# tsinghua-fib-lab/PIML

Hardware: AMD Instinct MI355X
Metric: agent-pair force evals/sec + simulated steps/sec, 4096-agent GC scene (higher is better)
Workload: dtype f32

## Files before the change

### include/piml_hip.h

```cpp
#ifndef PIML_HIP_H
#define PIML_HIP_H

#include <stddef.h>
#include <stdint.h>

#ifdef __cplusplus
extern "C" {
#endif

#define PIML_HIP_ABI_VERSION 35
#define PIML_MAX_TOPK 32

int piml_abi_version(void);

const char* piml_error_string(int err);

int piml_heading_fwd(const float* velocity, int C, int T, int N, float* heading, void* stream);

int piml_relfeat_fwd(const float* position, const float* heading, const float* velocity,
                     const float* acceleration, int state_ld, const float* destination,
                     const float* obstacles, int C, int N, int M, int focal_begin,
                     int focal_count, int topk_ped, int topk_obs, float cos_thr_ped,
                     float cos_thr_obs, float dist_thr_ped, float dist_thr_obs,
                     float* ped_feat, float* obs_feat, float* dest_feat, int dest_feat_ld,
// ... 353 lines not shown
                                  size_t rows, float tau, float* out, void* stream);
int piml_pinnsf_epilogue_ksum_bwd(const float* g_out, const float* self_features, size_t rows, float tau, int kp, int ko,
                                  float* g_self, float* g_pred_ped, float* g_pred_obs, void* stream);

int piml_pinnsf_epilogue_agentnorm_fwd(const float* acc_ped, const float* acc_obs, const float* self_features,
                                       int C, int N, float tau, float* out, void* stream);
int piml_pinnsf_epilogue_ksum_agentnorm_fwd(const float* pred_ped, int kp, const float* pred_obs, int ko, const float* self_features,
                                            int C, int N, float tau, float* out, void* stream);
int piml_pinnsf_epilogue_agentnorm_bwd(const float* g_out, const float* self_features, int C, int N, float tau,
                                       float* g_self, void* stream);

int piml_self_features_fwd(const float* dest_feat, int dest_ld, const float* state, const float* desired_speed,
                           size_t rows, float* out, void* stream);
int piml_self_features_bwd(const float* g_self, size_t rows, float* g_dest, float* g_state, float* g_speed,
                           void* stream);

int piml_colsum_blocks(size_t rows, int cols);
int piml_act_bwd_colsum(const float* g, const float* y, size_t rows, int cols, float* g_pre, float* partials,
                        float* db, void* stream);

int piml_sum_leading(const float* parts, int B, size_t n, float* out, void* stream);
int piml_act_bwd_colsum_stage1(const float* g, const float* y, size_t rows, int cols, float* g_pre, float* partials,
                               float* db, void* stream);
int piml_layer_reduce(const float* parts, int B, size_t n, float* out, const float* col_partials, int nb, int cols,
                      float* db, void* stream);

int piml_scale_ksum_fwd(const float* e, const float* bias, size_t agents, int k, int cols, float scale,
                        const unsigned* keep_bits, float* msgs, float* pooled, void* stream);
int piml_ksum_blocks(size_t agents, int cols);
int piml_scale_ksum_bwd(const float* g_pooled, const float* g_msgs, size_t agents, int k, int cols, float scale,
                        const unsigned* keep_bits, float* g_e, float* col_partials, void* stream);

int piml_dropout_keep_bits(unsigned long long* state, long long rows, int cols, float p, int stream_id, unsigned* keep_bits,
                           void* stream);

typedef struct piml_encoder_branch {
    const float* x;
    long long rows;
    int in_dim;
    int k;
    const float *w1, *b1, *w2, *b2, *w3, *b3;
    float scale;
    float *h1, *h2, *msgs;
    const float *g_pooled, *g_msgs;
    float *g2, *g1, *g_x;
    float* partials;
    float* grads;
    float* packed;
    unsigned* relu_mask;
    unsigned* keep_bits;
    unsigned long long* drop_state;
    float drop_p;
    float *sum_a, *sum_b;
} piml_encoder_branch;

int piml_encoder_partial_floats(void);
int piml_encoder_pack_floats(void);
int piml_encoder_pack(const piml_encoder_branch* branches, int nbranches, void* stream);
int piml_encoder_workgroups(const piml_encoder_branch* branches, int nbranches, int* wg_branch0);
int piml_encoder_fwd(const piml_encoder_branch* branches, int nbranches, void* stream);
int piml_encoder_fwd_packed(const piml_encoder_branch* branches, int nbranches, void* stream);
int piml_encoder_bwd(const piml_encoder_branch* branches, int nbranches, void* stream);
int piml_encoder_bwd_acc(const piml_encoder_branch* branches, int nbranches, int accumulate, void* stream);
int piml_encoder_ksum(const float* msgs, long long agents, int k, float* pooled, void* stream);

typedef struct piml_decoder_branch {
    const float* msgs;
    long long agents;
    int k;
    const float *w1, *b1, *w2, *b2, *w3, *b3;
    float *pooled, *h1, *d2;
    float *g_pre2, *g_pre1, *g_pooled;
    float* partials;
    float* grads;
    float* packed;
    float* pred;
    const float* g_pred_rows;
    const float* g_d2;
    const float *fold_w3, *fold_b3;
    float fold_scale;
    float* dw1_out;
} piml_decoder_branch;

int piml_decoder_pack_floats(void);
int piml_decoder_partial_floats(void);
int piml_decoder_workgroups(long long agents);
int piml_decoder_fwd(const piml_decoder_branch* branches, int nbranches, const float* self_features, float tau,
                     float* acc, void* stream);
int piml_decoder_bwd(const piml_decoder_branch* branches, int nbranches, const float* g_pred,
                     const float* self_features, float tau, float* g_self, void* stream);

int piml_rowdecoder_slots(long long rows);
int piml_rowdecoder_fwd(const piml_decoder_branch* branches, int nbranches, void* stream);
int piml_rowdecoder_fwd_packed(const piml_decoder_branch* branches, int nbranches, void* stream);
int piml_rowdecoder_bwd(const piml_decoder_branch* branches, int nbranches, void* stream);
int piml_rowdecoder_bwd_acc(const piml_decoder_branch* branches, int nbranches, int accumulate, void* stream);

typedef struct piml_collision_head {
    const float* msgs;
    long long rows;
    const float *w1, *b1, *w2, *b2;
    float* packed;
    float* out;
    const float *fold_w3, *fold_b3;
    float fold_scale;
} piml_collision_head;

// ... 98 lines not shown
```

### include/piml_hip_tuning.h

```cpp
#ifndef PIML_HIP_TUNING_H
#define PIML_HIP_TUNING_H

#include "piml_hip.h"

#ifdef __cplusplus
extern "C" {
#endif

int piml_timer_create(void** event);
int piml_timer_record(void* event, void* stream);
int piml_timer_elapsed_ms(void* start, void* stop, float* ms);
int piml_timer_destroy(void* event);

int piml_trace_begin(void);
int piml_trace_mark(const char* name, void* stream);
int piml_trace_end(char* names, int names_cap, float* us, int us_cap);

int piml_probe_arith(const float* rx, const float* ry, const float* hx, const float* hy,
                     float* dist, float* cosv, int n, void* stream);

long long piml_encoder_split_tiles(long long tiles);
long long piml_encoder_split_tiles_train(long long tiles);
int piml_encoder_products(int split_bf16);
int piml_rowdecoder_products(int split_bf16);
int piml_encoder_dw2(int layer_split);
int piml_encoder_fused_bwd(int on);
int piml_encoder_sums_bwd(int form);
int piml_encoder_sums_dec_slots(int on);
int piml_pinnsf_streams_init(void);

#ifdef __cplusplus
}
#endif
#endif
```

### piml_amd/_lib.py

```python
import ctypes
import os

import torch

_HERE = os.path.dirname(os.path.abspath(__file__))
LIB_PATH = os.environ.get('PIML_LIB') or os.path.join(_HERE, 'libpiml_hip.so')
ABI_VERSION = 35

_lib = None

_i, _f, _p, _z = ctypes.c_int, ctypes.c_float, ctypes.c_void_p, ctypes.c_size_t
_ll = ctypes.c_longlong
_d = ctypes.c_double


class EncoderBranch(ctypes.Structure):
    _fields_ = [('x', _p), ('rows', _ll), ('in_dim', _i), ('k', _i),
                ('w1', _p), ('b1', _p), ('w2', _p), ('b2', _p), ('w3', _p), ('b3', _p),
                ('scale', _f), ('h1', _p), ('h2', _p), ('msgs', _p), ('g_pooled', _p), ('g_msgs', _p),
                ('g2', _p), ('g1', _p), ('g_x', _p), ('partials', _p), ('grads', _p), ('packed', _p), ('relu_mask', _p),
                ('keep_bits', _p), ('drop_state', _p), ('drop_p', _f), ('sum_a', _p), ('sum_b', _p)]


class DecoderBranch(ctypes.Structure):
    _fields_ = [('msgs', _p), ('agents', _ll), ('k', _i),
                ('w1', _p), ('b1', _p), ('w2', _p), ('b2', _p), ('w3', _p), ('b3', _p),
                ('pooled', _p), ('h1', _p), ('d2', _p), ('g_pre2', _p), ('g_pre1', _p), ('g_pooled', _p),
                ('partials', _p), ('grads', _p), ('packed', _p), ('pred', _p), ('g_pred_rows', _p), ('g_d2', _p),
                ('fold_w3', _p), ('fold_b3', _p), ('fold_scale', _f), ('dw1_out', _p)]


class CollisionHead(ctypes.Structure):
    _fields_ = [('msgs', _p), ('rows', _ll), ('w1', _p), ('b1', _p), ('w2', _p), ('b2', _p), ('packed', _p), ('out', _p),
                ('fold_w3', _p), ('fold_b3', _p), ('fold_scale', _f)]


class Head64(ctypes.Structure):
    _fields_ = [('x', _p), ('rows', _ll), ('w1', _p), ('b1', _p), ('w2', _p), ('b2', _p), ('hidden', _p), ('out', _p),
                ('g_out', _p), ('g_x', _p), ('partials', _p), ('grads', _p)]


class Corrector(ctypes.Structure):
    _fields_ = [('agents', _ll), ('k', _i), ('scale', _f), ('enc', _p), ('keep_bits', _p),
                ('wa', _p), ('ba', _p), ('wb', _p), ('bb', _p), ('wc', _p), ('bc', _p), ('wd', _p), ('bd', _p),
                ('hid', _p), ('score', _p), ('attn', _p), ('pooled', _p), ('chid', _p), ('out', _p),
                ('g_out', _p), ('g_pooled', _p), ('g_score', _p), ('g_chid', _p), ('g_enc', _p),
                ('partials_a', _p), ('partials_b', _p), ('grads', _p)]


class Scenario(ctypes.Structure):
    _fields_ = [('position', _p), ('velocity', _p), ('acceleration', _p), ('destination', _p), ('hist_velocity', _p),
                ('self_features', _p), ('desired_speed', _p), ('mask', _p), ('flag', _p), ('waypoints', _p), ('exit_idx', _p),
                ('spawn_iters', _p), ('position_out', _p), ('velocity_out', _p), ('acceleration_out', _p),
                ('destination_out', _p), ('mask_out', _p), ('spawn_out', _p), ('frame_counter', _p), ('spawned', _p),
                ('dropped', _p), ('entries', _p), ('route_polyline', _p),
                ('hist_width', _i), ('F', _i), ('D', _i), ('E', _i), ('P', _i), ('R', _i), ('capacity', _i), ('T', _i),
                ('n_initial', _i), ('route_max_iters', _i), ('spawn_cap', _i), ('uniform_speed', _i),
                ('dt', _f), ('spawn_offset', _f), ('route_clearance', _f), ('arrival_radius', _f), ('speed_mean', _f),
                ('speed_std', _f), ('speed_min', _f), ('seed', ctypes.c_uint64), ('poisson_thresholds', ctypes.c_uint32 * 8)]


class ScenarioRules(ctypes.Structure):
    _fields_ = [('spawn_law', _i), ('arrival_rule', _i), ('initial_velocity', _i), ('speed_clamp', _i), ('spawn_cap2', _i),
                ('grid', _i), ('length', _f), ('width', _f), ('side_ratio', _f), ('direction_ratio', _f),
                ('poisson_thresholds2', ctypes.c_uint32 * 8), ('square_grid', _f * 32)]


class MlapmLaw(ctypes.Structure):
    _fields_ = [('variant', _i), ('tau', _f), ('A', _f), ('B', _f), ('C', _f), ('D', _f), ('theta_deg', _f), ('radius', _f)]


class WallGrid(ctypes.Structure):
    _fields_ = [('points', _p), ('cell_start', _p), ('n_points', _i), ('gx', _i), ('gy', _i),
                ('x0', _f), ('y0', _f), ('cell', _f), ('cutoff', _f)]
# ... 84 lines not shown
    'piml_pinnsf_epilogue_agentnorm_fwd': [_p, _p, _p, _i, _i, _f, _p, _p],
    'piml_pinnsf_epilogue_ksum_agentnorm_fwd': [_p, _i, _p, _i, _p, _i, _i, _f, _p, _p],
    'piml_pinnsf_epilogue_agentnorm_bwd': [_p, _p, _i, _i, _f, _p, _p],
    'piml_self_features_fwd': [_p, _i, _p, _p, _z, _p, _p],
    'piml_self_features_bwd': [_p, _z, _p, _p, _p, _p],
    'piml_colsum_blocks': [_z, _i],
    'piml_act_bwd_colsum': [_p, _p, _z, _i, _p, _p, _p, _p],
    'piml_sum_leading': [_p, _i, _z, _p, _p],
    'piml_act_bwd_colsum_stage1': [_p, _p, _z, _i, _p, _p, _p, _p],
    'piml_layer_reduce': [_p, _i, _z, _p, _p, _i, _i, _p, _p],
    'piml_scale_ksum_fwd': [_p, _p, _z, _i, _i, _f, _p, _p, _p, _p],
    'piml_ksum_blocks': [_z, _i],
    'piml_scale_ksum_bwd': [_p, _p, _z, _i, _i, _f, _p, _p, _p, _p],
    'piml_dropout_keep_bits': [_p, _ll, _i, _f, _i, _p, _p],
    'piml_timer_create': [ctypes.POINTER(_p)],
    'piml_timer_record': [_p, _p],
    'piml_timer_elapsed_ms': [_p, _p, ctypes.POINTER(_f)],
    'piml_timer_destroy': [_p],
    'piml_trace_begin': [],
    'piml_trace_mark': [ctypes.c_char_p, _p],
    'piml_trace_end': [ctypes.c_char_p, _i, ctypes.POINTER(_f), _i],
    'piml_probe_arith': [_p, _p, _p, _p, _p, _p, _i, _p],
    'piml_encoder_partial_floats': [],
    'piml_encoder_pack_floats': [],
    'piml_encoder_split_tiles': [_ll],
    'piml_encoder_split_tiles_train': [_ll],
    'piml_multi_copy': [ctypes.POINTER(_p), ctypes.POINTER(_p), ctypes.POINTER(_z), _i, _p],
    'piml_rollout_prologue': [_p] * 8 + [_i] * 4 + [_p] * 11 + [_p],
    'piml_rollout_losses_blocks': [_i, _i],
    'piml_rollout_losses': [_p, _p, _ll, _p, _p, _p, _p, _p, _i, _i, _i, _f, _p, _p, _p, _p, _p, _p, _p],
    'piml_rollout_losses_bwd': [_p, _p, _p, _p, _p, _p, _ll, _p, _p],
    'piml_rollout_losses_frames': [_p, _p, _ll, _p, _p, ctypes.POINTER(_p), _i, _p, _i, _i, _i, _f, _f, _f, _p, _p, _p, _p, _p, _p, _p],
    'piml_rollout_losses_frames_bwd': [_p, _p, _p, _p, _f, _f, _p, _p, _p, _ll, _p, _p],
    'piml_collision_pred_loss_blocks': [_ll, _i],
    'piml_collision_pred_loss': [ctypes.POINTER(_p), ctypes.POINTER(_p), _i, _ll, _i, _i, _p, _i, _i, _f, _p, _p, _p, _p, _p],
    'piml_collision_pred_loss_bwd': [_p, _p, _ll, _p, _p],
    'piml_adam_tickets': [],
    'piml_adam_step': [ctypes.POINTER(_p)] * 5 + [ctypes.POINTER(_ll), _i, ctypes.c_double, ctypes.c_double, ctypes.c_double, ctypes.c_double, ctypes.c_double, _p, _p],
    'piml_pointwise_losses_blocks': [_ll, _ll, _i],
    'piml_pointwise_losses': [_p, _p, _ll, _ll, _p, _ll, _f, _p, _i, _p, _p, _p, _p, _p],
    'piml_p2p_alloc': [_z, ctypes.POINTER(_p)],
    'piml_p2p_free': [_p],
    'piml_p2p_export': [_p, _p],
    'piml_p2p_open': [_p, ctypes.POINTER(_p)],
    'piml_p2p_close': [_p],
    'piml_p2p_copy': [_p, _p, _z, _p],
    'piml_allgather_state_p2p': [_p, _z, _i, _i, ctypes.POINTER(_p), ctypes.POINTER(_p), ctypes.c_uint, ctypes.c_uint, _p, _p],
    'piml_encoder_products': [_i],
    'piml_rowdecoder_products': [_i],
    'piml_encoder_dw2': [_i],
    'piml_encoder_fused_bwd': [_i],
    'piml_encoder_sums_bwd': [_i],
    'piml_encoder_sums_dec_slots': [_i],
    'piml_encoder_pack': [ctypes.POINTER(EncoderBranch), _i, _p],
    'piml_encoder_workgroups': [ctypes.POINTER(EncoderBranch), _i, ctypes.POINTER(_i)],
    'piml_encoder_fwd': [ctypes.POINTER(EncoderBranch), _i, _p],
    'piml_encoder_fwd_packed': [ctypes.POINTER(EncoderBranch), _i, _p],
    'piml_encoder_bwd': [ctypes.POINTER(EncoderBranch), _i, _p],
    'piml_encoder_bwd_acc': [ctypes.POINTER(EncoderBranch), _i, _i, _p],
    'piml_encoder_ksum': [_p, _ll, _i, _p, _p],
    'piml_decoder_pack_floats': [],
    'piml_decoder_partial_floats': [],
    'piml_decoder_workgroups': [_ll],
    'piml_decoder_fwd': [ctypes.POINTER(DecoderBranch), _i, _p, _f, _p, _p],
    'piml_decoder_bwd': [ctypes.POINTER(DecoderBranch), _i, _p, _p, _f, _p, _p],
    'piml_rowdecoder_slots': [_ll],
    'piml_rowdecoder_fwd': [ctypes.POINTER(DecoderBranch), _i, _p],
    'piml_rowdecoder_fwd_packed': [ctypes.POINTER(DecoderBranch), _i, _p],
    'piml_rowdecoder_bwd': [ctypes.POINTER(DecoderBranch), _i, _p],
    'piml_rowdecoder_bwd_acc': [ctypes.POINTER(DecoderBranch), _i, _i, _p],
    'piml_collision_head_pack_floats': [],
    'piml_collision_head_fwd': [_p, _ll, _p, _p, _p, _p, _p, _p, _p],
    'piml_head64_partial_floats': [],
    'piml_head64_slots': [_ll],
    'piml_head64_fwd': [ctypes.POINTER(Head64), _p],
    'piml_head64_bwd': [ctypes.POINTER(Head64), _p],
    'piml_head64_bwd_acc': [ctypes.POINTER(Head64), _i, _p],
    'piml_corrector_partial_floats': [_i],
    'piml_corrector_slots': [_i, _ll, _i],
    'piml_corrector_fwd': [ctypes.POINTER(Corrector), _p],
    'piml_corrector_bwd': [ctypes.POINTER(Corrector), _i, _p],
    'piml_pinnsf_pool_h2_ok': [ctypes.POINTER(EncoderBranch), _i],
    'piml_pinnsf_pool_train_ok': [ctypes.POINTER(EncoderBranch), _i],
    'piml_pinnsf_pool_msgs_ok': [ctypes.POINTER(EncoderBranch), _i],
    'piml_pinnsf_streams_init': [],
    'piml_pinnsf_pack_flush': [],
    'piml_pinnsf_slot_sums_flush': [],
    'piml_pinnsf_pack': [ctypes.POINTER(EncoderBranch), ctypes.POINTER(DecoderBranch), _i, ctypes.POINTER(CollisionHead),
                         _i, _p],
    'piml_pinnsf_fwd': [ctypes.POINTER(EncoderBranch), ctypes.POINTER(DecoderBranch), _i, ctypes.POINTER(CollisionHead),
                        _p, _f, _p, _i, _p],
    'piml_pinnsf_bwd': [ctypes.POINTER(EncoderBranch), ctypes.POINTER(DecoderBranch), _i, _p, _p, _f, _p, _i, _p],
    'piml_comm_available': [],
    'piml_comm_unique_id': [_p],
    'piml_comm_init': [ctypes.POINTER(_p), _i, _i, _p],
    'piml_comm_destroy': [_p],
    'piml_allgather_state': [_p, _p, _z, _p, _p],
    'piml_reducescatter_grad': [_p, _p, _p, _z, _p],
    'piml_allreduce_sum': [_p, _p, _z, _p],
    'piml_relfeat_fwd_self': [_p, _p, _p, _p, _i, _p, _p, _p, _i, _i, _i, _i, _i, _i, _i, _f, _f, _f, _f, _p, _p, _p, _p, _p, _p, _p],
    'piml_relfeat_bwd_self': [_p, _p, _p, _p, _p, _p, _i, _p, _i, _i, _i, _i, _i, _i, _p, _p, _p, _p],
    'piml_relfeat_fwd_tick': [_p, _p, _p, _p, _i, _p, _p, _i, _i, _i, _i, _i, _i, _i, _f, _f, _f, _f,
                              _p, _p, _p, _i, _p, _p, _p, _p],
    'piml_relfeat_self_fwd': [_p, _p, _p, _p, _i, _i, _i, _i, _i, _i, _f, _f, _f, _f, _p, _p, _p, _p, _p, _p, _p],
    'piml_relfeat_self_fwd_part': [_i, _p, _p, _p, _p, _i, _i, _i, _i, _i, _i, _f, _f, _f, _f, _p, _p, _p, _p, _p, _p, _p],
    'piml_relfeat_self_bwd': [_p, _p, _p, _p, _p, _p, _p, _i, _i, _i, _i, _i, _p, _p, _p, _p],
# ... 165 lines not shown
```

### piml_amd/csrc/encoder.hip

```cpp
#include <cstdlib>

#include "common.hpp"
#include "encoder.hpp"
#include "pack.hpp"
#include "reduce.hpp"
#include "philox.hpp"
#include "stages.hpp"
#include "../../include/piml_hip.h"

namespace piml {

__device__ __forceinline__ void keep_block_f32(f32x16& a, unsigned word, int h) {
    const unsigned m = word >> (4 * h);
#pragma unroll
    for (int r = 0; r < 16; ++r) a[r] = ((m >> ((r & 3) + 8 * (r >> 2))) & 1u) ? a[r] : 0.f;
}
__device__ __forceinline__ unsigned keep_word(const unsigned* __restrict__ keep, long long row, int blk, bool valid) {
    return valid ? keep[row * 4 + blk] : 0u;
}

__global__ __launch_bounds__(256) void enc_pack_kernel(EncArgs A) {
    const int b = blockIdx.y;
    const piml_encoder_branch J = b ? A.br[1] : A.br[0];
    const int e = blockIdx.x * 256 + threadIdx.x;
    if (e < PACK_FLOATS) J.packed[e] = pack_value(J, e);
}

constexpr int FWD_LDS_FLOATS = 16384 * 2 + 1024 + 384;

__global__ __launch_bounds__(ENC_THREADS) void enc_fwd_kernel(EncArgs A) {
    extern __shared__ __align__(16) float lds[];
    const int tid = threadIdx.x, lane = tid & 63, wave = tid >> 6;
    const int b = (A.nbr > 1 && (int)blockIdx.x >= A.wg_split) ? 1 : 0;
    const piml_encoder_branch J = b ? A.br[1] : A.br[0];
    const int wg0 = b ? A.wg_split : 0;
    const int nwg = b ? (int)gridDim.x - A.wg_split : (A.nbr > 1 ? A.wg_split : (int)gridDim.x);
    const long long R = J.rows;
    const int IN = J.in_dim;
    const long long ntiles = (R + 31) >> 5;
    const long long first = (long long)((int)blockIdx.x - wg0) * ENC_WAVES + wave;
    const long long stride = (long long)nwg * ENC_WAVES;
    if (A.zero)
        for (int e = blockIdx.x * ENC_THREADS + tid; e < A.zero_n; e += gridDim.x * ENC_THREADS) A.zero[e] = 0.f;
    if ((long long)((int)blockIdx.x - wg0) * ENC_WAVES >= ntiles) return;

    const float4* W2f = reinterpret_cast<const float4*>(lds);
    const float4* W3f = reinterpret_cast<const float4*>(lds + 16384);
    const float* W1f = lds + 32768;
    const float* bias = lds + 32768 + 1024;
    stage_linear<PACK_FWD>(lds, J.packed, tid);
    __syncthreads();

    const int j = lane & 31, h = lane >> 5;
    for (long long tile = first; tile < ntiles; tile += stride) {
        const long long row = tile * 32 + j;
        const bool valid = row < R;
        float xb[4];
#pragma unroll
        for (int s = 0; s < 4; ++s) {
            const int c = 2 * s + h;
            xb[s] = (valid && c < IN) ? J.x[row * IN + c] : 0.f;
        }
        f32x16 a1[4], a2[4];
#pragma unroll
        for (int blk = 0; blk < 4; ++blk) {
#pragma unroll
            for (int q = 0; q < 4; ++q) {
                const float4 bq = *reinterpret_cast<const float4*>(bias + feat0(blk, q, h));
                a1[blk][4 * q + 0] = bq.x; a1[blk][4 * q + 1] = bq.y; a1[blk][4 * q + 2] = bq.z; a1[blk][4 * q + 3] = bq.w;
            }
#pragma unroll
            for (int s = 0; s < 4; ++s) a1[blk] = mfma32(W1f[(blk * 4 + s) * 64 + lane], xb[s], a1[blk]);
#pragma unroll
            for (int r = 0; r < 16; ++r) a1[blk][r] = fmaxf(a1[blk][r], 0.f);
        }
        if (J.h1 && valid) {
            float* o = J.h1 + row * EH;
#pragma unroll
// ... 602 lines not shown
struct Reduce2Args { piml_encoder_branch br[2]; int n0[2], n1[2]; int accumulate; };
__global__ __launch_bounds__(256) void enc_reduce2_kernel(Reduce2Args A) {
    const int b = blockIdx.y >> 1, L = blockIdx.y & 1;
    const piml_encoder_branch J = b ? A.br[1] : A.br[0];
    if (L == 0) {
        if ((int)blockIdx.x * 16 < DW2_L0_LANES) sum_slots_16x16(J.partials, J.grads, A.n0[b], DW2_L0_LANES, DW2_L0_SPLIT, 0, DW2_L0_OFF1, A.accumulate != 0);
    } else {
        if ((int)blockIdx.x * 16 < DW2_L1_LANES)
            sum_slots_16x16(J.partials + (size_t)A.n0[b] * (DW2_L0_LANES * 4), J.grads, A.n1[b], DW2_L1_LANES, DW2_L1_SPLIT, DW2_L1_OFF0, DW2_L1_OFF1,
                            A.accumulate != 0);
    }
}

static int split_workgroups(const piml_encoder_branch* br, int nbr, int total, long long unit) {
    if (nbr < 2) return total;
    const double r0 = (double)br[0].rows, r1 = (double)br[1].rows;
    int w = (int)(total * r0 / (r0 + r1) + 0.5);
    if (w < 1) w = 1;
    if (w > total - 1) w = total - 1;
    (void)unit;
    return w;
}

static bool branch_ok(const piml_encoder_branch& b) {
    return b.rows > 0 && b.rows < (1ll << 24) && b.in_dim >= 1 && b.in_dim <= 8 && b.x && b.w1 && b.b1 && b.w2 && b.b2 && b.w3 && b.b3 &&
           b.packed;
}

static int fill_args(EncArgs& A, const piml_encoder_branch* br, int nbr) {
    A.nbr = nbr;
    A.zero = nullptr;
    A.zero_n = 0;
    A.gen_state = nullptr;
    for (int i = 0; i < nbr; ++i) A.br[i] = br[i];
    if (nbr == 1) A.br[1] = br[0];
    A.wg_split = split_workgroups(br, nbr, 256, 1);
    return 256;
}

}

using namespace piml;

PIML_API int piml_encoder_partial_floats(void) { return ENC_PART; }

PIML_API int piml_encoder_workgroups(const piml_encoder_branch* br, int nbr, int* wg_branch0) {
    if (!br || nbr < 1 || nbr > 2) return 0;
    const int total = 256;
    const int w0 = split_workgroups(br, nbr, total, 1);
    if (wg_branch0) *wg_branch0 = w0;
    return total;
}

PIML_API int piml_encoder_pack_floats(void) { return PACK_FLOATS; }

static int enc_check(const piml_encoder_branch* br, int nbr) {
    if (!br || nbr < 1 || nbr > 2) return hipErrorInvalidValue;
    for (int i = 0; i < nbr; ++i)
        if (!branch_ok(br[i])) return hipErrorInvalidValue;
    if (nbr == 2 && (br[0].keep_bits != nullptr) != (br[1].keep_bits != nullptr)) return hipErrorInvalidValue;
    return hipSuccess;
}

static int enc_bwd_check(const piml_encoder_branch* br, int nbr);
static bool enc_bwd_is_fused(const piml_encoder_branch* br, int nbr);


static int enc_set_lds(const void* f, int bytes) {
    return hipFuncSetAttribute(f, hipFuncAttributeMaxDynamicSharedMemorySize, bytes);
}

int piml::enc_stage_pack(const piml_encoder_branch* br, int nbr, hipStream_t s) {
    if (!br || nbr < 1 || nbr > 2) return hipErrorInvalidValue;
    for (int i = 0; i < nbr; ++i) {
        const piml_encoder_branch& b = br[i];
        if (b.in_dim < 1 || b.in_dim > 8 || !b.w1 || !b.b1 || !b.w2 || !b.b2 || !b.w3 || !b.b3 || !b.packed) return hipErrorInvalidValue;
    }
    EncArgs A;
    A.nbr = nbr;
    A.br[0] = br[0];
    A.br[1] = br[nbr - 1];
    A.wg_split = 0;
    A.zero = nullptr;
    A.zero_n = 0;
    A.gen_state = nullptr;
    hipLaunchKernelGGL(enc_pack_kernel, dim3((PACK_FLOATS + 255) / 256, nbr), dim3(256), 0, s, A);
    return hipGetLastError();
}

static long long split_tiles_default() { return getenv("PIML_ENC_SPLIT_TILES") ? atoll(getenv("PIML_ENC_SPLIT_TILES")) : 640; }
static long long split_tiles_train_default() {
    if (getenv("PIML_ENC_SPLIT_TILES_TRAIN")) return atoll(getenv("PIML_ENC_SPLIT_TILES_TRAIN"));
    return getenv("PIML_ENC_SPLIT_TILES") ? atoll(getenv("PIML_ENC_SPLIT_TILES")) : 48;
}
static long long g_split_tiles = split_tiles_default();
static long long g_split_tiles_train = split_tiles_train_default();

PIML_API long long piml_encoder_split_tiles(long long tiles) {
    const long long old = g_split_tiles;
    if (tiles >= 0) g_split_tiles = g_split_tiles_train = tiles;
    else if (tiles == -2) { g_split_tiles = split_tiles_default(); g_split_tiles_train = split_tiles_train_default(); }
    return old;
}
PIML_API long long piml_encoder_split_tiles_train(long long tiles) {
    const long long old = g_split_tiles_train;
    if (tiles >= 0) g_split_tiles_train = tiles;
    return old;
}
static long long split_bound(const piml_encoder_branch* br, int nbr) {
    for (int i = 0; i < nbr; ++i)
        if (!br[i].relu_mask) return g_split_tiles;
    return g_split_tiles_train;
}

static int g_x3 = !(getenv("PIML_ENC_PRODUCTS") && getenv("PIML_ENC_PRODUCTS")[0] == 'f');

PIML_API int piml_encoder_products(int x3) {
    const int old = g_x3;
    if (x3 >= 0) g_x3 = x3 ? 1 : 0;
    return old;
}

static int g_f3 = getenv("PIML_ENC_FUSED_BWD") ? atoi(getenv("PIML_ENC_FUSED_BWD")) != 0 : 1;

PIML_API int piml_encoder_fused_bwd(int on) {
    const int old = g_f3;
    if (on >= 0) g_f3 = on != 0;
    return old;
}

static int g_sums_bwd = getenv("PIML_ENC_SUMS_BWD") && atoi(getenv("PIML_ENC_SUMS_BWD")) == 1 ? 1 : 2;

PIML_API int piml_encoder_sums_bwd(int form) {
    const int old = g_sums_bwd;
    if (form == 1 || form == 2) g_sums_bwd = form;
    return old;
}

bool piml::enc_f32_images_needed() { return !g_x3; }
// ... 262 lines not shown
    if (int e = enc_bwd_check(br, nbr)) return e;
    EncArgs A;
    fill_args(A, br, nbr);
    Reduce2Args R2 = {};
    R2.accumulate = accumulate ? 1 : 0;
    if (defer) {
        ReduceAll R = {};
        R.accumulate = accumulate ? 1 : 0;
        int n = 0, maxl = 0;
        auto add = [&](const float* parts, float* grads, int slots, int lanes, int split, int off0, int off1) {
            R.set[n++] = ReduceSet{parts, grads, slots, lanes, split, off0, off1};
            if (lanes > maxl) maxl = lanes;
        };
        int n0[2] = {0, 0}, n1[2] = {0, 0}, w0 = 0;
        const int total = piml_encoder_workgroups(br, nbr, &w0);
        const bool dw2 = enc_dw2_used(br, nbr, n0, n1);
        for (int i = 0; i < nbr; ++i) {
            if (dw2) {
                add(br[i].partials, br[i].grads, n0[i], DW2_L0_LANES, DW2_L0_SPLIT, 0, DW2_L0_OFF1);
                add(br[i].partials + (size_t)n0[i] * (DW2_L0_LANES * 4), br[i].grads, n1[i], DW2_L1_LANES, DW2_L1_SPLIT, DW2_L1_OFF0, DW2_L1_OFF1);
            } else {
                add(br[i].partials, br[i].grads, nbr == 1 ? total : (i == 0 ? w0 : total - w0), ENC_PART / 4, 0x7fffffff, 0, 0);
            }
        }
        R.nsets = n;
        R.gx = (maxl + 15) / 16;
        return pending_slot_sums_leave(R, s);
    }
    if (enc_dw2_used(br, nbr, R2.n0, R2.n1)) {
        for (int i = 0; i < nbr; ++i) R2.br[i] = br[i];
        hipLaunchKernelGGL(enc_reduce2_kernel, dim3((DW2_L1_LANES + 15) / 16, 2 * nbr), dim3(256), 0, s, R2);
        return hipGetLastError();
    }
    hipLaunchKernelGGL(enc_reduce_kernel, dim3((ENC_PART / 4 + 15) / 16, nbr), dim3(256), 0, s, A, ENC_PART / 4, accumulate ? 1 : 0);
    return hipGetLastError();
}

bool piml::enc_pool_train_ok(const piml_encoder_branch* br, int nbr) {
    static const bool off = getenv("PIML_POOL_TRAIN") && atoi(getenv("PIML_POOL_TRAIN")) == 0;
    if (off || !g_dw2 || g_f3 != 1) return false;
    const long long tiles = pool_tiles(br, nbr, true, [](const piml_encoder_branch& b) { return !b.keep_bits && !b.drop_state; });
    if (tiles < 0 || tiles <= g_split_tiles_train) return false;
    const int total = 256, w0 = split_workgroups(br, nbr, total, 1);
    return nbr == 1 || (w0 >= 2 && total - w0 >= 2);
}

bool piml::enc_pool_msgs_ok(const piml_encoder_branch* br, int nbr) {
    static const bool off = getenv("PIML_POOL_MSGS") && atoi(getenv("PIML_POOL_MSGS")) == 0;
    if (off) return false;
    const long long tiles = pool_tiles(br, nbr, true, [](const piml_encoder_branch& b) { return b.relu_mask != nullptr; });
    return tiles >= 0 && tiles > g_split_tiles_train;
}

int piml::enc_stage_fwd_sum(const piml_encoder_branch* br, int nbr, hipStream_t s, float* zero, long long zero_n) {
    if (int e = enc_check(br, nbr)) return e;
    if (!enc_pool_train_ok(br, nbr)) return hipErrorInvalidValue;
    for (int i = 0; i < nbr; ++i)
        if (!br[i].sum_a || !br[i].sum_b || !br[i].relu_mask) return hipErrorInvalidValue;
    EncArgs A;
    const int total = fill_args(A, br, nbr);
    if (int e = set_zero(A, zero, zero_n)) return e;
    if (int e = x3_ready()) return e;
    enc_x3_launch_fwd_sum(A, total, s);
    return hipGetLastError();
}

int piml::enc_stage_bwd_sum(const piml_encoder_branch* br, int nbr, hipStream_t s, const DecSlotSums* dec, bool* dec_summed) {
    if (dec_summed) *dec_summed = false;
    if (int e = enc_check(br, nbr)) return e;
    if (!enc_pool_train_ok(br, nbr)) return hipErrorInvalidValue;
    for (int i = 0; i < nbr; ++i) {
        const piml_encoder_branch& b = br[i];
        if (!b.g_pooled || b.g_msgs || !b.relu_mask || !b.partials || !b.grads || (b.g_x != nullptr) != (br[0].g_x != nullptr)) return hipErrorInvalidValue;
    }
    EncArgs A;
    const int total = fill_args(A, br, nbr);
    if (int e = x3_ready()) return e;
    static int ready = -1;
    if (ready < 0) { ready = enc_f3_set_attributes(); if (!ready) ready = enc_f5_set_attributes(); }
    if (ready) return ready;
    const int nA[2] = {nbr > 1 ? A.wg_split : total, nbr > 1 ? total - A.wg_split : 0};
    const int zero[2] = {0, 0};
    if (g_sums_bwd == 1 || !enc_f5_launch(A, nA, s, dec)) enc_f3_launch(A, nA, zero, false, s, true);
    else if (dec_summed) *dec_summed = dec && dec->nsets > 0;
    return hipGetLastError();
}

PIML_API int piml_encoder_pack(const piml_encoder_branch* br, int nbr, void* stream) {
    return enc_stage_pack(br, nbr, as_stream(stream));
}

PIML_API int piml_encoder_fwd(const piml_encoder_branch* br, int nbr, void* stream) {
    if (int e = enc_stage_pack(br, nbr, as_stream(stream))) return e;
    return enc_stage_fwd(br, nbr, as_stream(stream));
}

PIML_API int piml_encoder_fwd_packed(const piml_encoder_branch* br, int nbr, void* stream) {
    if (int e = pending_pack_flush(as_stream(stream))) return e;
    return enc_stage_fwd(br, nbr, as_stream(stream));
}

PIML_API int piml_encoder_ksum(const float* msgs, long long agents, int k, float* pooled, void* stream) {
    if (agents == 0) return hipSuccess;
    if (!msgs || !pooled || agents < 0 || k < 0) return hipErrorInvalidValue;
    const long long n = agents * (EH / 4);
    hipLaunchKernelGGL(enc_ksum_kernel, dim3((unsigned)((n + 255) / 256)), dim3(256), 0, as_stream(stream),
                       reinterpret_cast<const float4*>(msgs), agents, k, reinterpret_cast<float4*>(pooled));
    return hipGetLastError();
}

PIML_API int piml_encoder_bwd_acc(const piml_encoder_branch* br, int nbr, int accumulate, void* stream) {
    const bool acc = (accumulate & 1) || (accumulate & PIML_ACCUMULATE), defer = (accumulate & PIML_DEFER_SLOT_SUMS) != 0;
    if (int e = enc_stage_bwd_dx(br, nbr, as_stream(stream))) return e;
    if (int e = enc_stage_bwd_dw(br, nbr, as_stream(stream))) return e;
    return enc_stage_reduce(br, nbr, as_stream(stream), acc, defer);
}

PIML_API int piml_encoder_bwd(const piml_encoder_branch* br, int nbr, void* stream) { return piml_encoder_bwd_acc(br, nbr, 0, stream); }
```

### piml_amd/csrc/encoder.hpp

```cpp
#pragma once
#include <hip/hip_runtime.h>

#include "pack.hpp"
#include "../../include/piml_hip.h"

namespace piml {

typedef float f32x16 __attribute__((ext_vector_type(16)));

constexpr int ENC_THREADS = 512;
constexpr int ENC_WAVES = ENC_THREADS / 64;

struct EncArgs {
    piml_encoder_branch br[2];
    int nbr;
    int wg_split;
    float* zero;
    int zero_n;
    unsigned long long* gen_state;
};

__device__ __forceinline__ f32x16 mfma32(float a, float b, f32x16 c) {
    return __builtin_amdgcn_mfma_f32_32x32x2f32(a, b, c, 0, 0, 0);
}
typedef float f32x4 __attribute__((ext_vector_type(4)));
__device__ __forceinline__ void store4_stream(float* p, float a, float b, float c, float d) {
    *reinterpret_cast<float4*>(p) = make_float4(a, b, c, d);
}

template <int NFLOATS>
__device__ __forceinline__ void stage_linear(float* lds, const float* __restrict__ src, int tid) {
    constexpr int N4 = NFLOATS / 4, ROUNDS = (N4 + ENC_THREADS - 1) / ENC_THREADS;
    static_assert(NFLOATS % 4 == 0, "float4 granularity");
    const float4* s4 = reinterpret_cast<const float4*>(src);
    float4* d4 = reinterpret_cast<float4*>(lds);
    float4 v[ROUNDS];
#pragma unroll
    for (int r = 0; r < ROUNDS; ++r) {
        const int e = r * ENC_THREADS + tid;
        v[r] = s4[(r + 1) * ENC_THREADS <= N4 || e < N4 ? e : 0];
    }
#pragma unroll
    for (int r = 0; r < ROUNDS; ++r) {
        const int e = r * ENC_THREADS + tid;
        if ((r + 1) * ENC_THREADS <= N4 || e < N4) d4[e] = v[r];
    }
}

__device__ __forceinline__ int feat0(int blk, int q, int h) { return 32 * blk + 8 * q + 4 * h; }

int enc_x3_set_attributes();
void enc_x3_launch_fwd_pool(const EncArgs& A, int total, hipStream_t s);
void enc_x3_launch_fwd_sum(const EncArgs& A, int total, hipStream_t s);
void enc_x3_launch_fwd(const EncArgs& A, int total, bool drop, hipStream_t s, bool exch = false);
void enc_x3_launch_fwd_split(const EncArgs& A, int pairs0, int pairs1, bool drop, hipStream_t s);
void enc_x3_launch_bwd_dx_split(const EncArgs& A, int pairs0, int pairs1, bool drop, hipStream_t s);
void enc_x3_launch_bwd_dx(const EncArgs& A, int total, bool mask, bool drop, hipStream_t s);

int enc_dww_set_attributes();
void enc_dww_launch(const EncArgs& A, int grid, bool drop, hipStream_t s);
int enc_dw2_set_attributes();
void enc_dw2_split(int w, int* n0, int* n1);
void enc_dw2_launch(const EncArgs& A, int total, hipStream_t s);

// ... 7 lines not shown
```

### piml_amd/csrc/encoder_bwd5.hip

```cpp
#include "common.hpp"
#include "encoder.hpp"
#include "x3.hpp"

namespace piml {

typedef short f5_s16x4 __attribute__((ext_vector_type(4)));
typedef __attribute__((address_space(3))) f5_s16x4 f5_lds_s16x4;

constexpr int F5_THREADS = 512;
constexpr int F5_IMG = 3 * 128 * 64;
constexpr int F5_M = 0;
constexpr int F5_H = F5_M + 2 * F5_IMG;
constexpr int F5_TROW = 36;
constexpr int F5_TBYTES = 128 * F5_TROW * 4;
constexpr int F5_T = F5_H + 2 * F5_IMG;
constexpr int F5_XS = F5_T + 2 * F5_TBYTES;
constexpr int F5_MK = F5_XS + 3 * 1024;
constexpr int F5_W1 = F5_MK + 2 * 512;
constexpr int F5_GXP = F5_W1 + 4096;
constexpr int F5_GXP_BYTES = 4 * 32 * 16 * 4;
constexpr int F5_TAB = F5_GXP + 2 * F5_GXP_BYTES;
constexpr int F5_KMAX = 16;
constexpr int F5_LDS_BYTES = F5_TAB + F5_KMAX * 2 * 16 * 4;
constexpr int F5_LDS_LAUNCH = F5_LDS_BYTES;
// ... 18 lines not shown
    }
}
__device__ __forceinline__ void f5_dec_sums(const DecSlotSums& D, int wg, int nwg, int t, int nthr) {
    const int total = D.nsets * D.lanes, per = (total + nwg - 1) / nwg;
    const int e1 = min(wg * per + per, total), half = nthr >> 4;
    for (int e = wg * per + (t >> 4); e < e1; e += 2 * half) {
        const bool two = e + half < e1;
        const int ea = e, eb = two ? e + half : e;
        const int sa = ea >= D.lanes ? 1 : 0, sb = eb >= D.lanes ? 1 : 0;
        const float4* const p[2] = {reinterpret_cast<const float4*>(sa ? D.parts[1] : D.parts[0]),
                                    reinterpret_cast<const float4*>(sb ? D.parts[1] : D.parts[0])};
        const int j[2] = {ea - sa * D.lanes, eb - sb * D.lanes};
        float4 s[2];
        slot_chains<2>(p, D.slots, D.lanes, j, t & 15, s);
        const float4 va = s[0], vb = s[1];
        f5_chains_add<1>(s[0], va);
        f5_chains_add<1>(s[1], vb);
        if ((t & 15) == 0) {
            slot_sum_store(reinterpret_cast<float4*>(sa ? D.grads[1] : D.grads[0]) + j[0], s[0], D.accumulate != 0);
            if (two) slot_sum_store(reinterpret_cast<float4*>(sb ? D.grads[1] : D.grads[0]) + j[1], s[1], D.accumulate != 0);
        }
    }
}

#ifdef PIML_F5_STAMPS
__device__ unsigned long long g_f5_stamps[256 * 8 * 16];
#define F5_STAMP(i)                                                        \
    do {                                                                   \
        __builtin_amdgcn_sched_barrier(0);                                 \
        {                                                                  \
            const unsigned long long t_ = __builtin_amdgcn_s_memtime();    \
            st[i] += t_ - tprev;                                           \
            tprev = t_;                                                    \
        }                                                                  \
        __builtin_amdgcn_sched_barrier(0);                                 \
    } while (0)
#else
#define F5_STAMP(i)
#endif

#define F5_BARRIER() asm volatile("s_waitcnt lgkmcnt(0)\n\ts_barrier" ::: "memory")

__device__ __forceinline__ float f5_relu(float x) { return __int_as_float(max(__float_as_int(x), 0)); }
__device__ __forceinline__ constexpr int f5_rho(int r) { return (r & 3) + 8 * (r >> 2); }

#define F5_SLOT(MF, FILL)                        \
    do {                                         \
        MF;                                      \
        __builtin_amdgcn_sched_barrier(0);       \
        FILL;                                    \
        __builtin_amdgcn_sched_barrier(0);       \
    } while (0)

template <bool GX, int INC>
__global__ __launch_bounds__(F5_THREADS) void enc_bwd_sums2_kernel(F5Args F) {
    extern __shared__ __align__(16) unsigned char smem[];
    const int tid = threadIdx.x, lane = tid & 63;
    const int wv = __builtin_amdgcn_readfirstlane(tid >> 6);
    const int crew = wv >> 2, w = wv & 3;
    const int ctid = tid & 255;
    const int n = lane & 31, h = lane >> 5;
    int bx = (int)blockIdx.x, b = 0;
    if (bx >= F.nA[0]) { b = 1; bx -= F.nA[0]; }
    const piml_encoder_branch J = b ? F.A.br[1] : F.A.br[0];
    const int nwg = F.nA[b];
    const unsigned R = (unsigned)J.rows;
    const unsigned IN = __builtin_amdgcn_readfirstlane((unsigned)J.in_dim), K = __builtin_amdgcn_readfirstlane((unsigned)J.k);
    const unsigned kmagic = __builtin_amdgcn_readfirstlane((unsigned)((0x100000000ull + K - 1) / K));
    const int ntiles = (int)((R + 31) >> 5);
    const int nit = bx < ntiles ? (ntiles - bx + nwg - 1) / nwg : 0;
    float* P = J.partials + (size_t)bx * F5_PART1;
    constexpr int NS = INC == 6 ? 3 : 4;

    auto rsrc = [&](const void* base, unsigned bytes) {
        return __builtin_amdgcn_make_buffer_rsrc(const_cast<void*>(base), 0, (int)bytes, 0x00020000);
    };
    constexpr unsigned kOut = 0x80000000u;
    const __amdgpu_buffer_rsrc_t rs_gp = rsrc(J.g_pooled, (R / K) * EH * 4);
    const __amdgpu_buffer_rsrc_t rs_x = rsrc(J.x, R * IN * 4);
    const __amdgpu_buffer_rsrc_t rs_mk = rsrc(J.relu_mask, (unsigned)ntiles * 1024);
    const __amdgpu_buffer_rsrc_t rs_gx = rsrc(J.g_x, GX ? R * IN * 4 : 0u);
    auto ld1 = [&](const __amdgpu_buffer_rsrc_t& rs, unsigned voff, unsigned soff) {
        return (unsigned)__builtin_amdgcn_raw_buffer_load_b32(rs, (int)voff, (int)soff, 0);
    };

#ifdef PIML_F5_STAMPS
    unsigned long long st[16], tprev = __builtin_amdgcn_s_memtime();
#pragma unroll
    for (int i = 0; i < 16; ++i) st[i] = 0;
#endif

    {
        float4* z = reinterpret_cast<float4*>(smem + F5_T);
        constexpr int NZ = (F5_W1 - F5_T) / 16;
#pragma unroll
        for (int i = 0; i < (NZ + F5_THREADS - 1) / F5_THREADS; ++i)
            if (i * F5_THREADS + tid < NZ) z[i * F5_THREADS + tid] = make_float4(0.f, 0.f, 0.f, 0.f);
#pragma unroll
        for (int i = 0; i < 2 * F5_GXP_BYTES / 16 / F5_THREADS; ++i) reinterpret_cast<float4*>(smem + F5_GXP)[i * F5_THREADS + tid] = make_float4(0.f, 0.f, 0.f, 0.f);
        if ((unsigned)tid < K * 32u) {
            const unsigned rem = (unsigned)tid >> 5, hh = ((unsigned)tid >> 4) & 1u, r = (unsigned)tid & 15u;
            reinterpret_cast<unsigned*>(smem + F5_TAB)[tid] = ((rem + 4u * hh + (unsigned)f5_rho((int)r)) / K) * (EH * 4);
        }
        if (tid < 256) reinterpret_cast<float4*>(smem + F5_W1)[tid] = make_float4(0.f, 0.f, 0.f, 0.f);
    }

    if (crew == 0) {
        u32x4 wh[8], wm[8], wl[8];
        {
            const u32x4* imgB = reinterpret_cast<const u32x4*>(J.packed + PACK_F32 + 3 * X3_IMG) + lane;
#pragma unroll
            for (int kb = 0; kb < 8; ++kb) {
                const int fb = w * 8 + kb;
                wh[kb] = imgB[(fb * 2) * 64];
                wm[kb] = imgB[(fb * 2 + 1) * 64];
                wl[kb] = imgB[X3_HM / 4 + fb * 64];
            }
        }
        const float* W1rows = J.packed + PACK_FWD + 32768;
        float w1v[NS];
#pragma unroll
        for (int s = 0; s < NS; ++s) w1v[s] = W1rows[(32 * w + n) * 8 + 2 * s + h];
        const float b1v = J.b1[32 * w + n];

        const int fw = 32 * w + n;
        const int swz_w = (fw >> 1) & 7;
        const int mw_off = F5_M + fw * 64;
        int mr[2];
        {
            const int g16 = lane >> 4, q = (lane >> 2) & 3, pp = lane & 3, hh = g16 >> 1;
            const int chunk = 4 * (g16 & 1) + pp;
#pragma unroll
            for (int half2 = 0; half2 < 2; ++half2)
                mr[half2] = F5_M + (8 * half2 + 4 * hh + q) * 64 + ((chunk ^ (4 * half2 + 2 * hh + (q >> 1))) * 8);
        }
        const int bp = 16 * (w & 1) + (n & 3) + 4 * (n >> 3);
        const int mk_off = F5_MK + ((4 * h + 32 * ((n >> 2) & 1)) * 2 + (w >> 1)) * 4;
        const int t_off = F5_T + fw * (F5_TROW * 4) + (4 * h) * 4;
        const int h_off = F5_H + ((w * 2) * 3 * 64 + lane) * 16;
        const unsigned gbase = (unsigned)(32 * w + n) * 4u;

        float g2[16];
        unsigned m2 = 0, mkv = 0;
        float xa[NS];
        auto req_g = [&](int tile) {
            const unsigned t32 = __builtin_amdgcn_readfirstlane((unsigned)tile * 32u);
            const unsigned a0 = __builtin_amdgcn_readfirstlane(__umulhi(t32, kmagic)), rem = t32 - a0 * K;
            const bool live = tile < ntiles;
            const unsigned gb = live ? gbase + a0 * (EH * 4) : kOut;
            const uint4* tab = reinterpret_cast<const uint4*>(smem + F5_TAB + (rem * 32u + 16u * (unsigned)h) * 4u);
#pragma unroll
            for (int i = 0; i < 4; ++i) {
                const uint4 o = tab[i];
                g2[4 * i + 0] = __uint_as_float(ld1(rs_gp, gb + o.x, 0u));
                g2[4 * i + 1] = __uint_as_float(ld1(rs_gp, gb + o.y, 0u));
                g2[4 * i + 2] = __uint_as_float(ld1(rs_gp, gb + o.z, 0u));
                g2[4 * i + 3] = __uint_as_float(ld1(rs_gp, gb + o.w, 0u));
            }
            m2 = ld1(rs_mk, live ? (unsigned)tile * 1024u + (128u + 2u * (unsigned)lane + (unsigned)(w >> 1)) * 4u : kOut, 0u);
        };
        auto req_x = [&](int tile) {
            const unsigned row = (unsigned)tile * 32u + (unsigned)n;
            const bool valid = (tile < ntiles) & (row < R);
#pragma unroll
            for (int s = 0; s < NS; ++s) {
                const unsigned cx = 2u * s + h;
                xa[s] = __uint_as_float(ld1(rs_x, (valid & (cx < IN)) ? (row * IN + cx) * 4u : kOut, 0u));
            }
            mkv = ld1(rs_mk, tile < ntiles ? (unsigned)tile * 1024u + (unsigned)(ctid & 127) * 4u : kOut, 0u);
        };
        float db1 = 0.f, db2 = 0.f;
        unsigned phi[4], pmid[4], plo[4];
        float sp_ra = 0.f, sp_rb = 0.f;
        auto split_a = [&](float a_, float b_, unsigned& hi) {
            hi = bf16_pair(a_, b_);
            sp_ra = a_ - __uint_as_float(hi << 16);
            sp_rb = b_ - __uint_as_float(hi & 0xffff0000u);
        };
        auto split_b = [&](unsigned& mid, unsigned& lo) {
            mid = bf16_pair(sp_ra, sp_rb);
            lo = bf16_pair(sp_ra - __uint_as_float(mid << 16), sp_rb - __uint_as_float(mid & 0xffff0000u));
        };
        auto g2_step = [&](int j, int pm) {
            const int s = j >> 3, q = j & 7;
            if (q < 2) {
                const unsigned m2w = m2 >> (16 * (w & 1));
#pragma unroll
                for (int r = 8 * s + 4 * q; r < 8 * s + 4 * q + 4; ++r) {
                    const int t = __builtin_amdgcn_sbfe(m2w, r, 1);
                    g2[r] = __uint_as_float(__float_as_uint(g2[r]) & (unsigned)t);
                    db2 += g2[r];
                }
            } else if (q < 6) {
                const int d = q - 2;
                split_a(g2[8 * s + 2 * d], g2[8 * s + 2 * d + 1], phi[d]);
                split_b(pmid[d], plo[d]);
            } else {
                const int g = 2 * s + (q - 6), d = 2 * (g & 1);
                unsigned char* dst = smem + mw_off + pm * F5_IMG + (((2 * g + h) ^ swz_w) * 8);
                *reinterpret_cast<uint2*>(dst) = make_uint2(phi[d], phi[d + 1]);
                *reinterpret_cast<uint2*>(dst + 8192) = make_uint2(pmid[d], pmid[d + 1]);
                *reinterpret_cast<uint2*>(dst + 16384) = make_uint2(plo[d], plo[d + 1]);
            }
        };
        f32x16 hacc;
        auto h1_mma = [&]() {
#pragma unroll
            for (int r = 0; r < 16; ++r) hacc[r] = b1v;
#pragma unroll
            for (int s = 0; s < NS; ++s) hacc = mfma32(xa[s], w1v[s], hacc);
        };
        auto h1_step = [&](int j, int pm) {
            const int s = j / 5, q = j % 5;
            if (q < 4) {
                split_a(f5_relu(hacc[8 * s + 2 * q]), f5_relu(hacc[8 * s + 2 * q + 1]), phi[q]);
                split_b(pmid[q], plo[q]);
            } else {
                u32x4* dst = reinterpret_cast<u32x4*>(smem + h_off + pm * F5_IMG + (s * 3 * 64) * 16);
                dst[0] = (u32x4){phi[0], phi[1], phi[2], phi[3]};
                dst[64] = (u32x4){pmid[0], pmid[1], pmid[2], pmid[3]};
                dst[128] = (u32x4){plo[0], plo[1], plo[2], plo[3]};
            }
        };
        auto stage = [&](int xslot, int pm) {
            if (w < NS) reinterpret_cast<float*>(smem + F5_XS + xslot * 1024)[n * 8 + 2 * w + h] = w == 0 ? xa[0] : (w == 1 ? xa[1] : (w == 2 ? xa[2] : xa[NS - 1]));
            if (ctid < 128) reinterpret_cast<unsigned*>(smem + F5_MK + pm * 512)[ctid] = mkv;
        };
        auto load_b = [&](u32x4 (&o)[3], int kb, int pm) {
#pragma unroll
            for (int p = 0; p < 3; ++p) {
                const f5_s16x4 lo4 = __builtin_amdgcn_ds_read_tr16_b64_v4i16((f5_lds_s16x4*)(smem + mr[0] + pm * F5_IMG + kb * 1024 + p * 8192));
                const f5_s16x4 hi4 = __builtin_amdgcn_ds_read_tr16_b64_v4i16((f5_lds_s16x4*)(smem + mr[1] + pm * F5_IMG + kb * 1024 + p * 8192));
                const uint2 x = __builtin_bit_cast(uint2, lo4), y = __builtin_bit_cast(uint2, hi4);
                o[p] = (u32x4){x.x, x.y, y.x, y.y};
            }
        };

        F5_BARRIER();
        req_g(bx);
        req_x(bx);
#pragma unroll
        for (int j = 0; j < 16; ++j) g2_step(j, 0);
        h1_mma();
#pragma unroll
        for (int j = 0; j < 10; ++j) h1_step(j, 0);
        stage(0, 0);
        req_g(bx + nwg);
        req_x(bx + nwg);
        F5_STAMP(15);
        F5_BARRIER();

        for (int it = 0; it < nit; ++it) {
            const int par = it & 1, tile = bx + it * nwg;
            F5_STAMP(0);
            f32x16 acc;
            u32x4 opa[2][3], ahi[8];
            unsigned mkw[16];
            const unsigned* mk1 = reinterpret_cast<const unsigned*>(smem + mk_off + par * 512);
            auto fill_a = [&](int sl) {
                if (sl < 40 && sl % 5 == 0) {
                    const int kb = sl / 5 + 1;
                    if (kb < 8) load_b(opa[kb & 1], kb, par);
                    return;
                }
                if (sl == 38 || sl == 39) return;
                const int f = sl < 40 ? sl - sl / 5 - 1 : sl - 10;
                (void)it;
                if (f >= 30 && f < 34) {
#pragma unroll
                    for (int i = 4 * (f - 30); i < 4 * (f - 30) + 4; ++i) mkw[i] = mk1[2 * f5_rho(i)];
                }
            };
            load_b(opa[0], 0, par);
            const f32x16 zero16 = {0.f, 0.f, 0.f, 0.f, 0.f, 0.f, 0.f, 0.f, 0.f, 0.f, 0.f, 0.f, 0.f, 0.f, 0.f, 0.f};
#pragma unroll
            for (int kb = 0; kb < 8; ++kb) {
                const u32x4 (&o)[3] = opa[kb & 1];
                ahi[kb] = o[0];
                F5_SLOT(acc = mfma_bf(o[2], wh[kb], kb == 0 ? zero16 : acc), fill_a(kb * 5 + 0));
                F5_SLOT(acc = mfma_bf(o[1], wm[kb], acc), fill_a(kb * 5 + 1));
                F5_SLOT(acc = mfma_bf(o[0], wl[kb], acc), fill_a(kb * 5 + 2));
                F5_SLOT(acc = mfma_bf(o[1], wh[kb], acc), fill_a(kb * 5 + 3));
                F5_SLOT(acc = mfma_bf(o[0], wm[kb], acc), fill_a(kb * 5 + 4));
            }
#pragma unroll
            for (int kb = 0; kb < 8; ++kb) F5_SLOT(acc = mfma_bf(ahi[kb], wh[kb], acc), fill_a(40 + kb));
            F5_STAMP(1);
#pragma unroll
            for (int r = 0; r < 16; ++r) {
                const int t = __builtin_amdgcn_sbfe(mkw[r], bp, 1);
                acc[r] = __uint_as_float(__float_as_uint(acc[r]) & (unsigned)t);
                db1 += acc[r];
            }
            {
                float4* dst = reinterpret_cast<float4*>(smem + t_off + par * F5_TBYTES);
#pragma unroll
                for (int g = 0; g < 4; ++g) dst[2 * g] = make_float4(acc[4 * g], acc[4 * g + 1], acc[4 * g + 2], acc[4 * g + 3]);
            }
            F5_STAMP(2);
            h1_mma();
#pragma unroll
            for (int j = 0; j < 16; ++j) g2_step(j, par ^ 1);
            F5_STAMP(6);
#pragma unroll
            for (int j = 0; j < 10; ++j) h1_step(j, par ^ 1);
            F5_STAMP(7);
            stage((it + 1) % 3, par ^ 1);
            req_g(tile + 2 * nwg);
            req_x(tile + 2 * nwg);
            F5_STAMP(5);
            F5_BARRIER();
        }
        F5_STAMP(3);
        if (F.D.nsets > 0) {
            f5_dec_sums(F.D, (int)blockIdx.x, (int)gridDim.x, ctid, 256);
            F5_STAMP(12);
        }
        F5_BARRIER();
        F5_BARRIER();
        db1 += __shfl_xor(db1, 32, 64);
        db2 += __shfl_xor(db2, 32, 64);
        if (h == 0) {
            P[EH * EH + 1024 + 32 * w + n] = db2;
            P[EH * EH + 1024 + EH + 32 * w + n] = db1;
        }
        for (unsigned cc = IN * 128 + ctid; cc < 1024; cc += 256) P[EH * EH + cc] = 0.f;
        F5_STAMP(11);
    } else {
        f32x16 c[4], sm[4];
#pragma unroll
        for (int jb = 0; jb < 4; ++jb)
#pragma unroll
            for (int r = 0; r < 16; ++r) { c[jb][r] = 0.f; sm[jb][r] = 0.f; }
        float w1acc[INC];
#pragma unroll
        for (int cc = 0; cc < INC; ++cc) w1acc[cc] = 0.f;
        float w1g[8];
        {
            const float* W1r = J.packed + PACK_FWD + 32768;
#pragma unroll
            for (int j = 0; j < 8; ++j) w1g[j] = (lane & 15) < 8 ? W1r[(32 * w + 4 * j + (lane >> 4)) * 8 + (lane & 15)] : 0.f;
        }
        const int fw = 32 * w + n;
        const int swz_w = (fw >> 1) & 7;
        const int mw_off = F5_M + fw * 64;
        const int t_row = F5_T + fw * (F5_TROW * 4) + (4 * h) * 4;
        const int xs_off = F5_XS + (4 * h) * 32;

        auto load_g2 = [&](u32x4 (&g)[3], int s_, int pm) {
#pragma unroll
            for (int p = 0; p < 3; ++p) {
                const uint2 x = *reinterpret_cast<const uint2*>(smem + mw_off + pm * F5_IMG + p * 8192 + (((4 * s_ + h) ^ swz_w) * 8));
                const uint2 y = *reinterpret_cast<const uint2*>(smem + mw_off + pm * F5_IMG + p * 8192 + (((4 * s_ + 2 + h) ^ swz_w) * 8));
                g[p] = (u32x4){x.x, x.y, y.x, y.y};
            }
        };
        auto load_h = [&](u32x4 (&o)[3], int u_, int pm) {
            const int s_ = u_ >> 2, jb_ = u_ & 3;
            const u32x4* hr = reinterpret_cast<const u32x4*>(smem + F5_H + pm * F5_IMG) + lane;
#pragma unroll
            for (int p = 0; p < 3; ++p) o[p] = hr[((jb_ * 2 + s_) * 3 + p) * 64];
        };
        auto gx_store = [&](int tile, int pm) {
            const unsigned grow = (unsigned)tile * 32u + (unsigned)(ctid >> 3), cs = (unsigned)ctid & 7u;
            const float* gp = reinterpret_cast<const float*>(smem + F5_GXP + pm * F5_GXP_BYTES) + (ctid >> 3) * 16 + (ctid & 7);
            const float v = ((gp[0] + gp[512]) + gp[1024]) + gp[1536];
            const bool cok = cs < IN;
            const unsigned off = (grow * IN + cs) * 4u;
            __builtin_amdgcn_raw_buffer_store_b32(__float_as_uint(v), rs_gx, (int)(((tile >= 0) & (tile < ntiles) & (grow < R) & cok) ? off : kOut), 0, 0);
        };
        float g1[16];
        float4 xv[2][4];
        auto g1_load = [&](int half_, int pm) {
            const float4* src = reinterpret_cast<const float4*>(smem + t_row + pm * F5_TBYTES);
#pragma unroll
            for (int g = 2 * half_; g < 2 * half_ + 2; ++g) {
                const float4 v = src[2 * g];
                g1[4 * g] = v.x; g1[4 * g + 1] = v.y; g1[4 * g + 2] = v.z; g1[4 * g + 3] = v.w;
            }
        };
        auto x_load = [&](int k, int xslot) {
            const float4* xr = reinterpret_cast<const float4*>(smem + xs_off + xslot * 1024);
#pragma unroll
            for (int e = 0; e < 2; ++e) {
                xv[k & 1][2 * e] = xr[2 * f5_rho(2 * k + e)];
                if (INC == 8) xv[k & 1][2 * e + 1] = xr[2 * f5_rho(2 * k + e) + 1];
                else {
                    const float2 t2 = *reinterpret_cast<const float2*>(&xr[2 * f5_rho(2 * k + e) + 1]);
                    xv[k & 1][2 * e + 1] = make_float4(t2.x, t2.y, 0.f, 0.f);
                }
            }
        };
        auto x_fma = [&](int k) {
#pragma unroll
            for (int e = 0; e < 2; ++e) {
                const float4 xa4 = xv[k & 1][2 * e], xb4 = xv[k & 1][2 * e + 1];
                const float g = g1[2 * k + e];
                w1acc[0] = __fmaf_rn(g, xa4.x, w1acc[0]); w1acc[1] = __fmaf_rn(g, xa4.y, w1acc[1]);
                w1acc[2] = __fmaf_rn(g, xa4.z, w1acc[2]); w1acc[3] = __fmaf_rn(g, xa4.w, w1acc[3]);
                w1acc[4] = __fmaf_rn(g, xb4.x, w1acc[4]); w1acc[5] = __fmaf_rn(g, xb4.y, w1acc[5]);
                if (INC == 8) { w1acc[INC - 2] = __fmaf_rn(g, xb4.z, w1acc[INC - 2]); w1acc[INC - 1] = __fmaf_rn(g, xb4.w, w1acc[INC - 1]); }
            }
        };
        f32x4 gd[2];
        float ga[8][2];
        const int ga_off = F5_T + (32 * w + (lane >> 4)) * (F5_TROW * 4) + (lane & 15) * 4;
        auto gm_load = [&](int j, int pm) {
#pragma unroll
            for (int r = 0; r < 2; ++r) ga[j][r] = *reinterpret_cast<const float*>(smem + ga_off + pm * F5_TBYTES + j * (4 * F5_TROW * 4) + r * 64);
        };
        auto gxm_step = [&](int f, int pm) {
            if (!GX) return;
            if (f == 0) {
                gd[0] = gd[1] = (f32x4){0.f, 0.f, 0.f, 0.f};
#pragma unroll
                for (int j = 0; j < 8; ++j) gm_load(j, pm);
            } else if (f <= 8) {
                const int j = f - 1;
#pragma unroll
                for (int r = 0; r < 2; ++r) gd[r] = __builtin_amdgcn_mfma_f32_16x16x4f32(ga[j][r], w1g[j], gd[r], 0, 0, 0);
            } else if (f == 9) {
                float* dst = reinterpret_cast<float*>(smem + F5_GXP + (pm ^ 1) * F5_GXP_BYTES) + (w * 32 + 4 * (lane >> 4)) * 16 + (lane & 15);
#pragma unroll
                for (int r = 0; r < 2; ++r)
#pragma unroll
                    for (int i = 0; i < 4; ++i) dst[(16 * r + i) * 16] = gd[r][i];
            }
        };
        auto lag_step = [&](int f, int pm, int xslot) {
            if (f == 0) { g1_load(0, pm); g1_load(1, pm); x_load(0, xslot); }
            else if (f == 1) { x_load(1, xslot); x_fma(0); }
            else if (f < 9) { if (f < 8) x_load(f, xslot); x_fma(f - 1); }
        };

        F5_BARRIER();
        F5_STAMP(15);
        F5_BARRIER();
        for (int it = 0; it < nit; ++it) {
            const int par = it & 1, tile = bx + it * nwg;
            F5_STAMP(0);
            u32x4 g2f[3], opb[2][3];
            const int lpm = par ^ 1, xslot = (it + 2) % 3;
            auto fill_b = [&](int sl) {
                if (sl % 6 == 0) {
                    const int u_ = sl / 6 + 1;
                    if (u_ < 8) load_h(opb[u_ & 1], u_, par);
                    return;
                }
                if (sl == 23) { load_g2(g2f, 1, par); return; }
                const int f = sl - sl / 6 - 1 - (sl > 23);
                if (f == 1) gxm_step(0, lpm);
                else if (f >= 6 && f < 14) gxm_step(f - 5, lpm);
                else if (f == 22) gxm_step(9, lpm);
            };
            if (GX) gx_store(tile - 2 * nwg, par ^ 1);
#pragma unroll
            for (int f = 0; f < 10; ++f) lag_step(f, lpm, xslot);
            F5_STAMP(6);
            F5_STAMP(5);
            load_g2(g2f, 0, par);
            load_h(opb[0], 0, par);
#pragma unroll
            for (int u = 0; u < 8; ++u) {
                const int jb = u & 3;
                const u32x4 (&o)[3] = opb[u & 1];
                F5_SLOT(sm[jb] = mfma_bf(g2f[2], o[0], sm[jb]), fill_b(u * 6 + 0));
                F5_SLOT(sm[jb] = mfma_bf(g2f[1], o[1], sm[jb]), fill_b(u * 6 + 1));
                F5_SLOT(sm[jb] = mfma_bf(g2f[0], o[2], sm[jb]), fill_b(u * 6 + 2));
                F5_SLOT(sm[jb] = mfma_bf(g2f[1], o[0], sm[jb]), fill_b(u * 6 + 3));
                F5_SLOT(sm[jb] = mfma_bf(g2f[0], o[1], sm[jb]), fill_b(u * 6 + 4));
                F5_SLOT(c[jb] = mfma_bf(g2f[0], o[0], c[jb]), fill_b(u * 6 + 5));
            }
            F5_STAMP(1);
            F5_BARRIER();
        }
        F5_STAMP(3);
        {
            const int it = nit, par = it & 1, tile = bx + it * nwg;
            if (GX) gx_store(tile - 2 * nwg, par ^ 1);
#pragma unroll
            for (int f = 0; f < 10; ++f) lag_step(f, par ^ 1, (it + 2) % 3);
#pragma unroll
            for (int f = 0; f < 10; ++f) gxm_step(f, par ^ 1);
            F5_BARRIER();
            if (GX) gx_store(tile - nwg, par);
            F5_BARRIER();
        }
        F5_STAMP(4);
#pragma unroll
        for (int jb = 0; jb < 4; ++jb)
#pragma unroll
            for (int r = 0; r < 16; ++r) P[(size_t)(32 * w + f5_rho(r) + 4 * h) * EH + 32 * jb + n] = c[jb][r] + sm[jb][r];
#pragma unroll
        for (int cc = 0; cc < INC; ++cc) w1acc[cc] += __shfl_xor(w1acc[cc], 32, 64);
        if (h == 0) {
            float* o = P + EH * EH + (size_t)(32 * w + n) * IN;
#pragma unroll
            for (int cc = 0; cc < INC; ++cc)
                if ((unsigned)cc < IN) o[cc] = w1acc[cc];
        }
        F5_STAMP(11);
    }
#ifdef PIML_F5_STAMPS
    if (lane == 0)
        for (int i = 0; i < 16; ++i) g_f5_stamps[(blockIdx.x * 8 + wv) * 16 + i] = st[i];
#endif
}

#ifdef PIML_F5_STAMPS
extern "C" __attribute__((visibility("default"))) int piml_f5_stamps(unsigned long long* out) {
    return (int)hipMemcpyFromSymbol(out, HIP_SYMBOL(g_f5_stamps), sizeof(unsigned long long) * 256 * 8 * 16);
}
#endif

int enc_f5_set_attributes() {
    auto set = [&](const void* f) { return (int)hipFuncSetAttribute(f, hipFuncAttributeMaxDynamicSharedMemorySize, F5_LDS_LAUNCH); };
    if (int e = set(reinterpret_cast<const void*>(enc_bwd_sums2_kernel<false, 6>))) return e;
    if (int e = set(reinterpret_cast<const void*>(enc_bwd_sums2_kernel<true, 6>))) return e;
    if (int e = set(reinterpret_cast<const void*>(enc_bwd_sums2_kernel<false, 8>))) return e;
    return set(reinterpret_cast<const void*>(enc_bwd_sums2_kernel<true, 8>));
}

bool enc_f5_launch(const EncArgs& A, const int* nA, hipStream_t s, const DecSlotSums* D) {
    F5Args F;
    F.A = A;
    F.nA[0] = nA[0]; F.nA[1] = A.nbr > 1 ? nA[1] : 0;
    F.D = D ? *D : DecSlotSums{};
    bool in6 = true;
    for (int i = 0; i < A.nbr; ++i) {
        if (A.br[i].k > F5_KMAX) return false;
        in6 = in6 && A.br[i].in_dim == 6;
    }
    const bool gx = A.br[0].g_x != nullptr;
    const dim3 g((unsigned)(F.nA[0] + F.nA[1])), blk(F5_THREADS);
    if (in6) {
        if (gx) hipLaunchKernelGGL((enc_bwd_sums2_kernel<true, 6>), g, blk, F5_LDS_LAUNCH, s, F);
        else hipLaunchKernelGGL((enc_bwd_sums2_kernel<false, 6>), g, blk, F5_LDS_LAUNCH, s, F);
    } else {
        if (gx) hipLaunchKernelGGL((enc_bwd_sums2_kernel<true, 8>), g, blk, F5_LDS_LAUNCH, s, F);
        else hipLaunchKernelGGL((enc_bwd_sums2_kernel<false, 8>), g, blk, F5_LDS_LAUNCH, s, F);
    }
    return true;
}

}
```

### piml_amd/csrc/encoder_x3.hip

```cpp
#include <cstdlib>

#include "common.hpp"
#include "encoder.hpp"
#include "philox.hpp"
#include "x3.hpp"

namespace piml {

struct Pieces {
    u32x4 hi[8], mid[8], lo[8];
};

__device__ __forceinline__ void split_tile(const f32x16 (&in)[4], Pieces& P) {
#pragma unroll
    for (int kb = 0; kb < 8; ++kb) {
        const f32x16& a = in[kb >> 1];
        const int r = 8 * (kb & 1);
        unsigned hi[4], mid[4], lo[4];
#pragma unroll
        for (int d = 0; d < 4; ++d) split3(a[r + 2 * d], a[r + 2 * d + 1], hi[d], mid[d], lo[d]);
        P.hi[kb] = (u32x4){hi[0], hi[1], hi[2], hi[3]};
        P.mid[kb] = (u32x4){mid[0], mid[1], mid[2], mid[3]};
        P.lo[kb] = (u32x4){lo[0], lo[1], lo[2], lo[3]};
    }
// ... 460 lines not shown
                a[blk][4 * q + 0] = bq.x; a[blk][4 * q + 1] = bq.y; a[blk][4 * q + 2] = bq.z; a[blk][4 * q + 3] = bq.w;
            }
#pragma unroll
            for (int s = 0; s < 4; ++s) a[blk] = mfma32(W1f[(blk * 4 + s) * 64 + lane_t], xb[s], a[blk]);
            const float pre0 = a[blk][0];
#pragma unroll
            for (int r = 0; r < 16; ++r) a[blk][r] = relu1(a[blk][r]);
            if (blk == 0) a[0][0] = __builtin_fmaf(pre0, 0.f, a[0][0]);
        }
        split_tile(a, P);
        load_x(xb, J.x, tile + stride, ntiles, R, IN, lane);
#pragma unroll
        for (int blk = 0; blk < 4; ++blk) {
            f32x16 acc, sm;
            const float bv = bias[128 + 32 * blk + (lane_t & 31)];
#pragma unroll
            for (int r = 0; r < 16; ++r) { sm[r] = 0.f; acc[r] = bv; }
#pragma unroll
            for (int kb = 0; kb < 8; ++kb) {
                const int fb = blk * 8 + kb;
                kblock_x3_t(acc, sm, W2hm[(fb * 2) * 64], W2hm[(fb * 2 + 1) * 64], W2lo[fb * 64], P.hi[kb], P.mid[kb], P.lo[kb]);
            }
#pragma unroll
            for (int r = 0; r < 16; ++r) {
                const float pre = acc[r] + sm[r];
                a[blk][r] = blk == 0 ? __builtin_fmaf(pre, 0.f, relu1(pre)) : relu1(pre);
            }
        }
        pool_rows_k(a, k, tile, agents, lane_t, J.msgs, J.h2);
    }
}


template <bool ROWS>
__device__ __forceinline__ void store_h2_rows(const f32x16 (&a)[4], float* __restrict__ h2, long long tile, long long R, int lane) {
    if (!ROWS) return;
    const int j = lane & 31, h = lane >> 5;
    float* __restrict__ base = h2 + (tile * 32 + 4 * h) * EH + j;
    const long long left = R - tile * 32 - 4 * h;
    if (R - tile * 32 >= 32) {
#pragma unroll
        for (int blk = 0; blk < 4; ++blk)
#pragma unroll
            for (int r = 0; r < 16; ++r) base[((r & 3) + 8 * (r >> 2)) * EH + 32 * blk] = a[blk][r];
    } else {
#pragma unroll
        for (int blk = 0; blk < 4; ++blk)
#pragma unroll
            for (int r = 0; r < 16; ++r)
                if ((r & 3) + 8 * (r >> 2) < left) base[((r & 3) + 8 * (r >> 2)) * EH + 32 * blk] = a[blk][r];
    }
}

__global__ __launch_bounds__(ENC_THREADS) void enc_fwd_sum_x3_kernel(EncArgs A) {
    extern __shared__ __align__(16) float lds[];
    const int tid = threadIdx.x, lane = tid & 63, wave = uniform((int)(threadIdx.x >> 6));
    const int b = (A.nbr > 1 && (int)blockIdx.x >= A.wg_split) ? 1 : 0;
    const piml_encoder_branch J = b ? A.br[1] : A.br[0];
    const int wg0 = b ? A.wg_split : 0;
    const int nwg = b ? (int)gridDim.x - A.wg_split : (A.nbr > 1 ? A.wg_split : (int)gridDim.x);
    const long long R = J.rows;
    const int IN = J.in_dim;
    const long long ntiles = (R + 31) >> 5;
    const long long first = (long long)wave * nwg + ((int)blockIdx.x - wg0);
    const long long stride = (long long)nwg * ENC_WAVES;
    if (A.zero)
        for (int e = blockIdx.x * ENC_THREADS + tid; e < A.zero_n; e += gridDim.x * ENC_THREADS) A.zero[e] = 0.f;
    if ((long long)((int)blockIdx.x - wg0) >= ntiles) return;
    const float* x3 = J.packed + PACK_F32;
    float xb[4];
    ENC_STAMP(0, false);
    load_x(xb, J.x, first, ntiles, R, IN, lane);
    stage_linear<X3_IMG>(lds, x3, tid);
    stage_linear<1024 + 384>(lds + X3_FWD_F32, J.packed + 32768, tid);
    ENC_STAMP(1, true);
    __syncthreads();
    ENC_STAMP(2, false);
    const int k = J.k;
    const long long agents = R / k;
    for (long long tile = first; tile < ntiles; tile += stride) {
        int lane_t = lane;
        asm volatile("" : "+v"(lane_t));
        const u32x4* W2hm = reinterpret_cast<const u32x4*>(lds) + lane_t;
        const u32x4* W2lo = W2hm + X3_HM / 4;
        const float* W1f = lds + X3_FWD_F32;
        const float* bias = W1f + 1024;
        const int h = lane_t >> 5;
        f32x16 a[4];
        Pieces P;
#pragma unroll
        for (int blk = 0; blk < 4; ++blk) {
#pragma unroll
            for (int q = 0; q < 4; ++q) {
                const float4 bq = *reinterpret_cast<const float4*>(bias + feat0(blk, q, h));
                a[blk][4 * q + 0] = bq.x; a[blk][4 * q + 1] = bq.y; a[blk][4 * q + 2] = bq.z; a[blk][4 * q + 3] = bq.w;
            }
#pragma unroll
            for (int s = 0; s < 4; ++s) a[blk] = mfma32(W1f[(blk * 4 + s) * 64 + lane_t], xb[s], a[blk]);
#pragma unroll
            for (int r = 0; r < 16; ++r) a[blk][r] = relu1(a[blk][r]);
        }
        uint2* mrow = reinterpret_cast<uint2*>(J.relu_mask) + (tile * 2) * 64 + lane_t;
        mrow[0] = make_uint2(sign_bits(a[0], a[1]), sign_bits(a[2], a[3]));
        ENC_STAMP(3, false);
        split_tile(a, P);
        ENC_STAMP(4, false);
        load_x(xb, J.x, tile + stride, ntiles, R, IN, lane);
#pragma unroll
        for (int blk = 0; blk < 4; ++blk) {
            f32x16 acc, sm;
            const float bv = bias[128 + 32 * blk + (lane_t & 31)];
#pragma unroll
            for (int r = 0; r < 16; ++r) { sm[r] = 0.f; acc[r] = bv; }
#pragma unroll
            for (int kb = 0; kb < 8; ++kb) {
                const int fb = blk * 8 + kb;
                kblock_x3_t(acc, sm, W2hm[(fb * 2) * 64], W2hm[(fb * 2 + 1) * 64], W2lo[fb * 64], P.hi[kb], P.mid[kb], P.lo[kb]);
            }
#pragma unroll
            for (int r = 0; r < 16; ++r) a[blk][r] = relu1(acc[r] + sm[r]);
        }
        ENC_STAMP(5, false);
        mrow[64] = make_uint2(sign_bits(a[0], a[1]), sign_bits(a[2], a[3]));
        if (J.h2) store_h2_rows<true>(a, J.h2, tile, R, lane_t);
        ENC_STAMP(6, false);
        pool_rows_k(a, k, tile, agents, lane_t, J.sum_a, J.sum_b);
        ENC_STAMP(7, false);
    }
    ENC_STAMP(8, true);
}

constexpr int X3_SPLIT_LDS_BYTES = 2 * 2 * 4 * 3 * 2 * 64 * 16;

template <int DROP>
__global__ __launch_bounds__(512) void enc_fwd_split_x3_kernel(EncArgs A, int pairs0) {
    extern __shared__ __align__(16) float lds[];
    u32x4* exch = reinterpret_cast<u32x4*>(lds);
    const int tid = threadIdx.x, lane = tid & 63, wave = __builtin_amdgcn_readfirstlane(tid >> 6);
    const int b = (int)blockIdx.x >= pairs0 ? 1 : 0;
    const piml_encoder_branch J = b ? A.br[1] : A.br[0];
    const int t = wave >> 2, blk = wave & 3;
    const long long R = J.rows;
    const int IN = J.in_dim;
    const long long tile = ((long long)blockIdx.x - (b ? pairs0 : 0)) * 2 + t;
    const int j = lane & 31, h = lane >> 5;
    const long long row = tile * 32 + j;
    const bool valid = row < R;
    if (A.zero)
        for (int e = blockIdx.x * 512 + tid; e < A.zero_n; e += gridDim.x * 512) A.zero[e] = 0.f;
    const unsigned long long goff = DROP == 2 ? A.gen_state[1] : 0ull;
    const u32x4* W2hm = reinterpret_cast<const u32x4*>(J.packed + PACK_F32) + lane;
    const u32x4* W2lo = W2hm + X3_HM / 4;
    const u32x4* W3hm = reinterpret_cast<const u32x4*>(J.packed + PACK_F32 + X3_IMG) + lane;
    const u32x4* W3lo = W3hm + X3_HM / 4;
    const float* W1g = J.packed + 32768;
    const float* bias = J.packed + 32768 + 1024;
    u32x4 wf[8][3];
#pragma unroll
    for (int kb = 0; kb < 8; ++kb) {
        const int fb = blk * 8 + kb;
        wf[kb][0] = W2hm[(fb * 2) * 64]; wf[kb][1] = W2hm[(fb * 2 + 1) * 64]; wf[kb][2] = W2lo[fb * 64];
    }
    float xb[4], w1[4];
#pragma unroll
    for (int s = 0; s < 4; ++s) {
        const int c = 2 * s + h;
        xb[s] = (valid && c < IN) ? J.x[(valid ? row : 0) * IN + c] : 0.f;
        w1[s] = W1g[(blk * 4 + s) * 64 + lane];
    }
    float4 bq[4], bqn[4];
#pragma unroll
    for (int q = 0; q < 4; ++q) bq[q] = *reinterpret_cast<const float4*>(bias + feat0(blk, q, h));
    f32x16 acc, sm;
    auto init = [&]() {
#pragma unroll
        for (int q = 0; q < 4; ++q) { acc[4 * q] = bq[q].x; acc[4 * q + 1] = bq[q].y; acc[4 * q + 2] = bq[q].z; acc[4 * q + 3] = bq[q].w; }
#pragma unroll
        for (int r = 0; r < 16; ++r) sm[r] = 0.f;
    };
    auto store = [&](float* dst, float sc) {
        if (dst && valid) {
            float* o = dst + row * EH;
#pragma unroll
// ... 421 lines not shown
        }
        __syncthreads();
    }
    if (blk == 0 && J.g_x) {
        float gx[8];
#pragma unroll
        for (int c = 0; c < 8; ++c) gx[c] = 0.f;
#pragma unroll
        for (int bp = 0; bp < 4; ++bp)
#pragma unroll
            for (int q = 0; q < 4; ++q) {
                __builtin_amdgcn_sched_barrier(0);
#pragma unroll
                for (int u = 0; u < 4; ++u) {
                    const int f = feat0(bp, q, h) + u;
                    const float4 wa = W1r[2 * f], wb = W1r[2 * f + 1];
                    const float v = g1x[((t * 4 + bp) * 16 + 4 * q + u) * 64 + lane];
                    gx[0] = __fmaf_rn(wa.x, v, gx[0]); gx[1] = __fmaf_rn(wa.y, v, gx[1]);
                    gx[2] = __fmaf_rn(wa.z, v, gx[2]); gx[3] = __fmaf_rn(wa.w, v, gx[3]);
                    gx[4] = __fmaf_rn(wb.x, v, gx[4]); gx[5] = __fmaf_rn(wb.y, v, gx[5]);
                    gx[6] = __fmaf_rn(wb.z, v, gx[6]); gx[7] = __fmaf_rn(wb.w, v, gx[7]);
                }
            }
#pragma unroll
        for (int c = 0; c < 8; ++c) gx[c] += __shfl_xor(gx[c], 32, 64);
        if (valid) {
            float* o = J.g_x + row * IN + 4 * h;
            const int left = IN - 4 * h;
            const float s0 = h ? gx[4] : gx[0], s1 = h ? gx[5] : gx[1], s2 = h ? gx[6] : gx[2], s3 = h ? gx[7] : gx[3];
            if (left > 0) o[0] = s0;
            if (left > 1) o[1] = s1;
            if (left > 2) o[2] = s2;
            if (left > 3) o[3] = s3;
        }
    }
}


int enc_x3_set_attributes() {
    auto set = [](const void* f, int bytes) { return (int)hipFuncSetAttribute(f, hipFuncAttributeMaxDynamicSharedMemorySize, bytes); };
    if (int e = set(reinterpret_cast<const void*>(enc_bwd_dx_split_x3_kernel<false>), X3_DXS_LDS_BYTES)) return e;
    if (int e = set(reinterpret_cast<const void*>(enc_bwd_dx_split_x3_kernel<true>), X3_DXS_LDS_BYTES)) return e;
    if (int e = set(reinterpret_cast<const void*>(enc_fwd_split_x3_kernel<0>), X3_SPLIT_LDS_BYTES)) return e;
    if (int e = set(reinterpret_cast<const void*>(enc_fwd_split_x3_kernel<1>), X3_SPLIT_LDS_BYTES)) return e;
    if (int e = set(reinterpret_cast<const void*>(enc_fwd_split_x3_kernel<2>), X3_SPLIT_LDS_BYTES)) return e;
    const void* dx[4] = {reinterpret_cast<const void*>(enc_bwd_dx_x3_kernel<false, false>),
                         reinterpret_cast<const void*>(enc_bwd_dx_x3_kernel<true, false>),
                         reinterpret_cast<const void*>(enc_bwd_dx_x3_kernel<false, true>),
                         reinterpret_cast<const void*>(enc_bwd_dx_x3_kernel<true, true>)};
    for (const void* f : dx)
        if (int e = set(f, X3_DX_LDS_BYTES)) return e;
    if (int e = set(reinterpret_cast<const void*>(enc_fwd_pool_x3_kernel), X3_FWD_LDS_BYTES)) return e;
    if (int e = set(reinterpret_cast<const void*>(enc_fwd_sum_x3_kernel), X3_FWD_LDS_BYTES)) return e;
    if (int e = set(reinterpret_cast<const void*>(enc_fwd_x3_kernel<2, true>), X3_FWD_LDS_BYTES)) return e;
    if (int e = set(reinterpret_cast<const void*>(enc_fwd_x3_kernel<1, true>), X3_FWD_LDS_BYTES)) return e;
    if (int e = set(reinterpret_cast<const void*>(enc_fwd_x3_kernel<0, true>), X3_FWD_LDS_BYTES)) return e;
    if (int e = set(reinterpret_cast<const void*>(enc_fwd_x3_kernel<2>), X3_FWD_LDS_BYTES)) return e;
    if (int e = set(reinterpret_cast<const void*>(enc_fwd_x3_kernel<1>), X3_FWD_LDS_BYTES)) return e;
    return set(reinterpret_cast<const void*>(enc_fwd_x3_kernel<0>), X3_FWD_LDS_BYTES);
}

void enc_x3_launch_bwd_dx(const EncArgs& A, int total, bool mask, bool drop, hipStream_t s) {
    const dim3 g(total), b(ENC_THREADS);
    if (mask && drop) hipLaunchKernelGGL((enc_bwd_dx_x3_kernel<true, true>), g, b, X3_DX_LDS_BYTES, s, A);
    else if (mask) hipLaunchKernelGGL((enc_bwd_dx_x3_kernel<true, false>), g, b, X3_DX_LDS_BYTES, s, A);
    else if (drop) hipLaunchKernelGGL((enc_bwd_dx_x3_kernel<false, true>), g, b, X3_DX_LDS_BYTES, s, A);
    else hipLaunchKernelGGL((enc_bwd_dx_x3_kernel<false, false>), g, b, X3_DX_LDS_BYTES, s, A);
}

void enc_x3_launch_bwd_dx_split(const EncArgs& A, int pairs0, int pairs1, bool drop, hipStream_t s) {
    const dim3 g((unsigned)(pairs0 + pairs1));
    if (drop) hipLaunchKernelGGL(enc_bwd_dx_split_x3_kernel<true>, g, dim3(512), X3_DXS_LDS_BYTES, s, A, pairs0);
    else hipLaunchKernelGGL(enc_bwd_dx_split_x3_kernel<false>, g, dim3(512), X3_DXS_LDS_BYTES, s, A, pairs0);
}

void enc_x3_launch_fwd_split(const EncArgs& A, int pairs0, int pairs1, bool drop, hipStream_t s) {
    const dim3 g((unsigned)(pairs0 + pairs1));
    if (drop && A.gen_state) hipLaunchKernelGGL(enc_fwd_split_x3_kernel<2>, g, dim3(512), X3_SPLIT_LDS_BYTES, s, A, pairs0);
    else if (drop) hipLaunchKernelGGL(enc_fwd_split_x3_kernel<1>, g, dim3(512), X3_SPLIT_LDS_BYTES, s, A, pairs0);
    else hipLaunchKernelGGL(enc_fwd_split_x3_kernel<0>, g, dim3(512), X3_SPLIT_LDS_BYTES, s, A, pairs0);
}

void enc_x3_launch_fwd_pool(const EncArgs& A, int total, hipStream_t s) {
    hipLaunchKernelGGL(enc_fwd_pool_x3_kernel, dim3(total), dim3(ENC_THREADS), X3_FWD_LDS_BYTES, s, A);
}

void enc_x3_launch_fwd_sum(const EncArgs& A, int total, hipStream_t s) {
    hipLaunchKernelGGL(enc_fwd_sum_x3_kernel, dim3(total), dim3(ENC_THREADS), X3_FWD_LDS_BYTES, s, A);
}

void enc_x3_launch_fwd(const EncArgs& A, int total, bool drop, hipStream_t s, bool exch) {
    const dim3 g(total), b(ENC_THREADS);
    if (exch) {
        if (drop && A.gen_state) hipLaunchKernelGGL((enc_fwd_x3_kernel<2, true>), g, b, X3_FWD_LDS_BYTES, s, A);
        else if (drop) hipLaunchKernelGGL((enc_fwd_x3_kernel<1, true>), g, b, X3_FWD_LDS_BYTES, s, A);
        else hipLaunchKernelGGL((enc_fwd_x3_kernel<0, true>), g, b, X3_FWD_LDS_BYTES, s, A);
        return;
    }
    if (drop && A.gen_state) hipLaunchKernelGGL(enc_fwd_x3_kernel<2>, g, b, X3_FWD_LDS_BYTES, s, A);
    else if (drop) hipLaunchKernelGGL(enc_fwd_x3_kernel<1>, g, b, X3_FWD_LDS_BYTES, s, A);
    else hipLaunchKernelGGL(enc_fwd_x3_kernel<0>, g, b, X3_FWD_LDS_BYTES, s, A);
}

}

#ifdef PIML_ENC_STAMPS
extern "C" __attribute__((visibility("default"))) int piml_enc_stamps(unsigned long long* out) {
    return (int)hipMemcpyFromSymbol(out, HIP_SYMBOL(piml::g_enc_stamps), sizeof(unsigned long long) * 512 * 16);
}
#endif
```

### piml_amd/csrc/network.hip

```cpp
#include <cstdio>
#include <cstdlib>
#include <mutex>

#include "common.hpp"
#include "pack.hpp"
#include "reduce.hpp"
#include "stages.hpp"
#include "trace.hpp"

namespace piml {

namespace {

struct Side {
    hipStream_t s[2] = {nullptr, nullptr};
    hipEvent_t ev[6] = {};
    bool ok = false;
};

constexpr int kMaxDevices = 64;
Side g_side[kMaxDevices];
std::mutex g_mu;

int side_streams(Side** out) {
// ... 246 lines not shown
PIML_API int piml_pinnsf_pack(const piml_encoder_branch* enc, const piml_decoder_branch* dec, int nbr,
                              const piml_collision_head* head, int flags, void* stream) {
    if (!enc || !dec || nbr < 1 || nbr > 2) return hipErrorInvalidValue;
    PackAll A = {};
    A.nbr = nbr;
    A.has_head = head != nullptr;
    A.skip_f32 = enc_f32_images_needed() ? 0 : 1;
    for (int i = 0; i < nbr; ++i) {
        const piml_encoder_branch& e = enc[i];
        const piml_decoder_branch& d = dec[i];
        if (e.in_dim < 1 || e.in_dim > 8 || !e.w1 || !e.b1 || !e.w2 || !e.b2 || !e.w3 || !e.b3 || !e.packed || !d.w1 || !d.b1 ||
            !d.w2 || !d.b2 || !d.w3 || !d.b3 || !d.packed)
            return hipErrorInvalidValue;
        A.enc[i] = e;
        A.dec[i] = d;
    }
    if (head) {
        if (!head->w1 || !head->b1 || !head->w2 || !head->b2 || !head->packed) return hipErrorInvalidValue;
        A.head = *head;
        if (head->fold_w3) {
            if (!head->fold_b3) return hipErrorInvalidValue;
            A.has_fold = 1;
        }
    }
    for (int i = 0; i < nbr; ++i)
        if (dec[i].fold_w3) {
            if (!dec[i].fold_b3) return hipErrorInvalidValue;
            A.has_fold = 1;
        }
    if (flags & PIML_DEFER_PACK) return pending_pack_leave(A, as_stream(stream));
    return launch_pack(A, as_stream(stream));
}

PIML_API int piml_pinnsf_pack_flush(void) { return pending_pack_flush(nullptr); }

static int reduce_all(const piml_encoder_branch* enc, const piml_decoder_branch* dec, int nbr, hipStream_t s, bool accumulate, bool defer = false,
                      bool sums = false, bool defer_unfold = false, bool dec_summed = false) {
    ReduceAll R = {};
    R.accumulate = accumulate ? 1 : 0;
    R.defer_unfold = defer_unfold ? 1 : 0;
    R.dec_upstream = dec_summed ? 1 : 0;
    int w0 = 0, n = 0, maxl = 0;
    const int total = piml_encoder_workgroups(enc, nbr, &w0);
    const int dslots = piml_decoder_workgroups(dec[0].agents);
    int n0[2] = {0, 0}, n1[2] = {0, 0};
    const bool dw2 = !sums && enc_dw2_used(enc, nbr, n0, n1);
    auto add = [&](const float* parts, float* grads, int slots, int lanes, int split, int off0, int off1) {
        R.set[n++] = ReduceSet{parts, grads, slots, lanes, split, off0, off1};
        if (lanes > maxl) maxl = lanes;
    };
    for (int i = 0; i < nbr; ++i) {
        if (sums) {
            add(enc[i].partials, enc[i].grads, nbr == 1 ? total : (i == 0 ? w0 : total - w0), DW2_L1_LANES, DW2_L1_SPLIT, DW2_L1_OFF0, DW2_L1_OFF1);
            R.unf[i] = UnfoldSet{dec[i].grads, dec[i].w1, enc[i].w3, enc[i].b3, dec[i].fold_scale, enc[i].k, dec[i].dw1_out, enc[i].grads};
            R.nunf = nbr;
        } else if (dw2) {
            add(enc[i].partials, enc[i].grads, n0[i], DW2_L0_LANES, DW2_L0_SPLIT, 0, DW2_L0_OFF1);
            add(enc[i].partials + (size_t)n0[i] * (DW2_L0_LANES * 4), enc[i].grads, n1[i], DW2_L1_LANES, DW2_L1_SPLIT, DW2_L1_OFF0, DW2_L1_OFF1);
        } else {
            add(enc[i].partials, enc[i].grads, nbr == 1 ? total : (i == 0 ? w0 : total - w0), ENC_PART / 4, 0x7fffffff, 0, 0);
        }
    }
    if (!dec_summed)
        for (int i = 0; i < nbr; ++i) add(dec[i].partials, dec[i].grads, dslots, DEC_PART / 4, 0x7fffffff, 0, 0);
    R.nsets = n;
    R.gx = (maxl + 15) / 16;
    if (defer) return pending_slot_sums_leave(R, s);
    UnfoldTail t;
    if (int e = launch_slot_sums(unfold_begin(R, s, &t), s)) return e;
    trace_mark("pinnsf_reduce", s);
    return unfold_end(t);
}

static int g_dec_slots_enc = !(getenv("PIML_ENC_DEC_SLOTS") && atoi(getenv("PIML_ENC_DEC_SLOTS")) == 0);

PIML_API int piml_encoder_sums_dec_slots(int on) {
    const int old = g_dec_slots_enc;
    if (on >= 0) g_dec_slots_enc = on ? 1 : 0;
    return old;
}

PIML_API int piml_pinnsf_slot_sums_flush(void) { return pending_slot_sums_flush(); }

PIML_API int piml_pinnsf_pool_h2_ok(const piml_encoder_branch* enc, int nbr) { return enc_pool_h2_ok(enc, nbr) ? 1 : 0; }
PIML_API int piml_pinnsf_pool_train_ok(const piml_encoder_branch* enc, int nbr) { return enc_pool_train_ok(enc, nbr) ? 1 : 0; }
PIML_API int piml_pinnsf_pool_msgs_ok(const piml_encoder_branch* enc, int nbr) { return enc_pool_msgs_ok(enc, nbr) ? 1 : 0; }

PIML_API int piml_pinnsf_fwd(const piml_encoder_branch* enc, const piml_decoder_branch* dec, int nbr,
                             const piml_collision_head* head, const float* self_features, float tau, float* acc,
                             int flags, void* stream) {
    hipStream_t m = as_stream(stream);
    const bool pack = !(flags & PIML_PACKED_VALID);
    PIML_TRY(pending_pack_flush(m));
    if (flags & PIML_POOL_TRAIN) {
        if ((flags & (PIML_FORK | PIML_POOL_H2)) || !enc_pool_train_ok(enc, nbr)) return hipErrorInvalidValue;
        for (int i = 0; i < nbr; ++i)
            if (dec[i].pooled != enc[i].sum_a || dec[i].msgs != enc[i].sum_b) return hipErrorInvalidValue;
        if (pack) PIML_TRY(piml_pinnsf_pack(enc, dec, nbr, head, 0, stream));
        PIML_TRY(enc_stage_fwd_sum(enc, nbr, m, nbr > 1 ? acc : nullptr, nbr > 1 ? dec[0].agents * 2 : 0));
        trace_mark("enc_fwd_sum", m);
        PIML_TRY(dec_stage_fwd_sum(dec, nbr, head, self_features, tau, acc, m));
        trace_mark("dec_fwd_head_sum", m);
        return hipSuccess;
    }
    if (flags & PIML_POOL_MSGS) {
        if ((flags & (PIML_FORK | PIML_POOL_H2)) || !enc_pool_msgs_ok(enc, nbr)) return hipErrorInvalidValue;
        for (int i = 0; i < nbr; ++i)
            if (dec[i].pooled != enc[i].sum_a || dec[i].msgs != enc[i].sum_b) return hipErrorInvalidValue;
        if (head && head->rows > 0 && head->msgs != enc[0].msgs) return hipErrorInvalidValue;
        if (pack) PIML_TRY(piml_pinnsf_pack(enc, dec, nbr, head, 0, stream));
        PIML_TRY(enc_stage_fwd(enc, nbr, m, nbr > 1 ? acc : nullptr, nbr > 1 ? dec[0].agents * 2 : 0, true));
        trace_mark("enc_fwd", m);
        PIML_TRY(dec_stage_fwd_sum(dec, nbr, head, self_features, tau, acc, m, false));
        trace_mark("dec_fwd_head_sum", m);
        return hipSuccess;
    }
    if (flags & PIML_POOL_H2) {
        if ((flags & PIML_FORK) || head || !enc_pool_h2_ok(enc, nbr)) return hipErrorInvalidValue;
        if (pack) PIML_TRY(piml_pinnsf_pack(enc, dec, nbr, nullptr, 0, stream));
        PIML_TRY(enc_stage_fwd_pool(enc, nbr, m, nbr > 1 ? acc : nullptr, nbr > 1 ? dec[0].agents * 2 : 0));
        trace_mark("enc_fwd", m);
        PIML_TRY(dec_stage_fwd_ph2(dec, nbr, self_features, tau, acc, m));
        trace_mark("dec_fwd_head", m);
        return hipSuccess;
    }
    if (!(flags & PIML_FORK)) {
        if (pack) PIML_TRY(piml_pinnsf_pack(enc, dec, nbr, head, 0, stream));
        PIML_TRY(enc_stage_fwd(enc, nbr, m, nbr > 1 ? acc : nullptr, nbr > 1 ? dec[0].agents * 2 : 0));
        trace_mark("enc_fwd", m);
        PIML_TRY(dec_stage_fwd_fused(dec, nbr, head, self_features, tau, acc, m));
        trace_mark("dec_fwd_head", m);
// ... 77 lines not shown
```

### piml_amd/csrc/pack.hpp

```cpp
#pragma once
#include <hip/hip_runtime.h>

#include "../../include/piml_hip.h"

namespace piml {

constexpr int EH = 128;
constexpr int DH = 128;
constexpr int DD = 64;
constexpr int ENC_PART = 2 * EH * EH + EH * 8 + 3 * EH;
constexpr int DEC_PART = DD * DH + DD * DD + 2 * DD + DD + DD + 8;

constexpr int PACK_FWD = 16384 * 2 + 1024 + 384;
constexpr int PACK_DX = 16384 * 2 + 1024;
constexpr int PACK_F32 = PACK_FWD + PACK_DX;

constexpr int X3_HM = 32 * 2 * 64 * 4;
constexpr int X3_LO = 32 * 64 * 4;
constexpr int X3_IMG = X3_HM + X3_LO;
constexpr int PACK_X3 = 4 * X3_IMG;
constexpr int PACK_FLOATS = PACK_F32 + PACK_X3;

typedef float f32x2_t __attribute__((ext_vector_type(2)));
typedef __bf16 bf16x2_t __attribute__((ext_vector_type(2)));

__device__ __forceinline__ unsigned bf16_pair(float a, float b) {
    return __builtin_bit_cast(unsigned, __builtin_convertvector((f32x2_t){a, b}, bf16x2_t));
}
__device__ __forceinline__ void split3(float a, float b, unsigned& hi, unsigned& mid, unsigned& lo) {
    hi = bf16_pair(a, b);
    const float ra = a - __uint_as_float(hi << 16), rb = b - __uint_as_float(hi & 0xffff0000u);
    mid = bf16_pair(ra, rb);
    lo = bf16_pair(ra - __uint_as_float(mid << 16), rb - __uint_as_float(mid & 0xffff0000u));
}

__device__ __forceinline__ unsigned pack_bits_x3(const piml_encoder_branch& J, int e) {
    const int img = e / X3_IMG, g = e - img * X3_IMG;
    const bool tr = img >= 2;
    const float* W = (img == 0 || img == 3) ? J.w2 : J.w3;
    const int d = g & 3, lane = (g >> 2) & 63;
    int p, fb;
    if (g < X3_HM) { p = (g >> 8) & 1; fb = g >> 9; }
    else { p = 2; fb = (g - X3_HM) >> 8; }
    const int blk = fb >> 3, kb = fb & 7, i = 32 * blk + (lane & 31);
    const int c = 16 * kb + 8 * (d >> 1) + 4 * (lane >> 5) + 2 * (d & 1);
    const float a = tr ? W[(size_t)c * EH + i] : W[(size_t)i * EH + c];
    const float b = tr ? W[(size_t)(c + 1) * EH + i] : W[(size_t)i * EH + c + 1];
    unsigned hi, mid, lo;
    split3(a, b, hi, mid, lo);
    return p == 0 ? hi : (p == 1 ? mid : lo);
}

__device__ __forceinline__ float pack_value(const piml_encoder_branch& J, int e) {
    const int IN = J.in_dim;
    if (e >= PACK_F32) return __uint_as_float(pack_bits_x3(J, e - PACK_F32));
    if (e < 32768 || (e >= PACK_FWD && e < PACK_FWD + 32768)) {
        const bool tr = e >= PACK_FWD;
        const int f = tr ? e - PACK_FWD : e;
        const float* W = (f < 16384) == tr ? J.w3 : J.w2;
        const int g = f & 16383, u = g & 3, lane = (g >> 2) & 63, q = (g >> 8) & 3, bp = (g >> 10) & 3, blk = g >> 12;
        const int i = lane & 31, c = 32 * bp + 8 * q + 4 * (lane >> 5) + u;
        return tr ? W[(size_t)c * EH + 32 * blk + i] : W[(size_t)(32 * blk + i) * EH + c];
    }
    if (e < 32768 + 1024) {
        const int g = e - 32768, l = g & 63, sidx = (g >> 6) & 3, blk = g >> 8;
        const int c = 2 * sidx + (l >> 5);
        return c < IN ? J.w1[(size_t)(32 * blk + (l & 31)) * IN + c] : 0.f;
    }
    if (e < PACK_FWD) {
        const int g = e - 32768 - 1024;
        return g < 128 ? J.b1[g] : (g < 256 ? J.b2[g - 128] : J.b3[g - 256]);
    }
    {
        const int g = e - PACK_FWD - 32768, f = g >> 3, c = g & 7;
// ... 189 lines not shown
```

### piml_amd/csrc/reduce.hpp

```cpp
#pragma once
#include <hip/hip_runtime.h>

#include "pack.hpp"

namespace piml {

struct ReduceSet {
    const float* parts;
    float* grads;
    int slots, lanes, split, off0, off1;
};
struct UnfoldSet {
    const float* dgrads;
    const float *w1, *w3, *b3;
    float scale;
    int k;
    float* dw1_out;
    float* egrads;
};
constexpr int REDUCE_SETS = 8;
struct ReduceAll {
    ReduceSet set[REDUCE_SETS];
    int nsets;
    int accumulate;
    int gx;
    UnfoldSet unf[2];
    int nunf;
    int defer_unfold;
    int dec_upstream;
    int unf_blocks;
};
constexpr int kUnfoldBlocks = 64 + 64 + 1;

struct UnfoldTail {
    ReduceAll R;
    hipStream_t stream = nullptr;
    bool go = false;
};
ReduceAll unfold_begin(const ReduceAll& R, hipStream_t s, UnfoldTail* t);
int unfold_end(const UnfoldTail& t);

__device__ __forceinline__ void unfold_block(const ReduceAll& R, int bid) {
    const int y = bid / kUnfoldBlocks, x = bid - y * kUnfoldBlocks, tid = (int)threadIdx.x;
    const UnfoldSet U = R.unf[y];
    const float* __restrict__ G = U.dgrads;
    const float* __restrict__ gb = U.dgrads + DD * DH + DD * DD + 2 * DD;
    const double sc = (double)U.scale;
    if (x < 64) {
        __shared__ float g[DH];
        __shared__ double part[256];
        if (tid < DH) g[tid] = G[(size_t)x * DH + tid];
        __syncthreads();
        const int m = tid & 127, half = tid >> 7;
        const float4* wr = reinterpret_cast<const float4*>(U.w3 + (size_t)m * EH + 64 * half);
        double a = 0.0;
#pragma unroll 8
        for (int q = 0; q < 16; ++q) {
            const float4 wv = wr[q];
            const float* gq = g + 64 * half + 4 * q;
            a += (double)gq[0] * wv.x + (double)gq[1] * wv.y + (double)gq[2] * wv.z + (double)gq[3] * wv.w;
        }
        part[tid] = a;
        __syncthreads();
        if (tid < DH)
            U.dw1_out[(size_t)x * DH + tid] = (float)(sc * ((part[tid] + part[tid + 128]) + (double)U.k * (double)gb[x] * (double)U.b3[tid]));
    } else if (x < 128) {
        const int m = __builtin_amdgcn_readfirstlane(2 * (x - 64) + (tid >> 7)), j = tid & 127;
        double a = 0.0;
        for (int i0 = 0; i0 < DD; i0 += 8) {
            float wv[8], gv[8];
#pragma unroll
            for (int u = 0; u < 8; ++u) { wv[u] = U.w1[(size_t)(i0 + u) * DH + m]; gv[u] = G[(size_t)(i0 + u) * DH + j]; }
#pragma unroll
            for (int u = 0; u < 8; ++u) a += (double)wv[u] * (double)gv[u];
        }
        U.egrads[(size_t)m * EH + j] = (float)(sc * a);
    } else if (tid < EH) {
        double a = 0.0;
        for (int i0 = 0; i0 < DD; i0 += 8) {
            float wv[8], gv[8];
#pragma unroll
            for (int u = 0; u < 8; ++u) { wv[u] = U.w1[(size_t)(i0 + u) * DH + tid]; gv[u] = gb[i0 + u]; }
#pragma unroll
            for (int u = 0; u < 8; ++u) a += (double)wv[u] * (double)gv[u];
        }
        U.egrads[2 * EH * EH + 8 * EH + tid] = (float)(sc * (double)U.k * a);
    }
}
static_assert(2 * EH * EH + 8 * EH >= (DW2_L1_OFF0 + DW2_L1_SPLIT) * 4 && 2 * EH * EH + 9 * EH <= DW2_L1_OFF1 * 4 && EH * EH <= DW2_L1_OFF0 * 4,
              "the unfold's dW3 / db3 fields lie outside the encoder layer-1 set's targets");

__device__ __forceinline__ void reduce_block(const ReduceAll& A, int bid) {
    const int y = bid / A.gx, x = bid - y * A.gx;
    const ReduceSet S = A.set[y];
    if (x * 16 < S.lanes) sum_slots_16x16_at(x, S.parts, S.grads, S.slots, S.lanes, S.split, S.off0, S.off1, A.accumulate != 0);
}
__device__ __forceinline__ void reduce_launch_block(const ReduceAll& A, int bid) {
    if (bid < A.unf_blocks) unfold_block(A, bid);
    else reduce_block(A, bid - A.unf_blocks);
}
__host__ __device__ inline int reduce_launch_blocks(const ReduceAll& A) { return A.unf_blocks + A.gx * A.nsets; }

struct PackAll {
    piml_encoder_branch enc[2];
    piml_decoder_branch dec[2];
    piml_collision_head head;
    int nbr, has_head;
    int has_fold;
    int skip_f32;
};
constexpr int ENC_LIVE_X3 = PACK_FLOATS - 2 * 32768;
__host__ __device__ inline int enc_set_elems(const PackAll& A) { return A.skip_f32 ? ENC_LIVE_X3 : PACK_FLOATS; }
__host__ __device__ inline int pack_elems_total(const PackAll& A) {
    return A.nbr * (enc_set_elems(A) + DEC_PACK_PLAIN) + (A.has_head ? HEAD_PACK_PLAIN : 0);
}

__device__ __forceinline__ void pack_flat(const PackAll& A, int t) {
    const int ne = enc_set_elems(A);
    for (int y = 0; y < A.nbr; ++y) {
        if (t < ne) {
            int e = t;
            if (A.skip_f32) e = t < PACK_FWD - 32768 ? t + 32768 : t + 2 * 32768;
            const piml_encoder_branch& J = A.enc[y];
            J.packed[e] = pack_value(J, e);
            return;
        }
        t -= ne;
    }
    for (int y = 0; y < A.nbr; ++y) {
        if (t < DEC_PACK_PLAIN) {
            const piml_decoder_branch& J = A.dec[y];
            J.packed[t] = dec_pack_value(J, t);
            return;
        }
        t -= DEC_PACK_PLAIN;
    }
    if (A.has_head && t < HEAD_PACK_PLAIN) A.head.packed[t] = head_pack_value(A.head, t);
}
__host__ __device__ inline int fold_sets(const PackAll& A) { return A.has_fold ? A.nbr + (A.has_head ? 1 : 0) : 0; }
__host__ __device__ inline int fold_groups_per_block(int threads) { return threads >= 512 ? threads / 512 : 1; }
__host__ __device__ inline int fold_blocks(const PackAll& A, int threads) {
    const int g = fold_groups_per_block(threads);
    return (fold_sets(A) * FOLD_GROUPS + g - 1) / g;
}
template <int CH>
__device__ __forceinline__ void fold_block(const PackAll& A, int fb, int threads, double* red) {
    const int wave = (int)threadIdx.x >> 6, lane = (int)threadIdx.x & 63;
    const int grp = fb * ((threads >> 6) / CH) + wave / CH, chunk = wave % CH;
    const int f = grp / FOLD_GROUPS, r = grp - f * FOLD_GROUPS, i = r / 3, hc = r - 3 * i;
    const bool live = f < fold_sets(A);
    const bool is_head = f >= A.nbr;
    const piml_decoder_branch& J = A.dec[is_head ? 0 : f];
    const float* w1 = is_head ? A.head.w1 : J.w1;
    const float* w3 = is_head ? A.head.fold_w3 : J.fold_w3;
    const float* b3 = is_head ? A.head.fold_b3 : J.fold_b3;
    const bool have = live && w3 != nullptr;
    double part = 0.0;
    if (have && (hc < 2 || lane == 0))
        part = fold_partial<CH>(w1 + (size_t)i * DH, hc < 2 ? w3 + 64 * hc + lane : b3, hc < 2 ? EH : 1, chunk);
    red[threadIdx.x] = part;
    __syncthreads();
    if (have && chunk == 0) {
        double sum = 0.0;
#pragma unroll
        for (int c = 0; c < CH; ++c) sum += red[threadIdx.x + 64 * c];
        if (is_head) head_fold_store(A.head, i, hc, lane, sum);
        else dec_fold_store(J, i, hc, lane, sum);
    }
}
constexpr int kPackPerThread = 4;
struct PackWork {
    PackAll A;
    int first_block;
};
__host__ __device__ inline int pack_plain_blocks(const PackAll& A, int threads) {
    return (pack_elems_total(A) + threads * kPackPerThread - 1) / (threads * kPackPerThread);
}
__host__ __device__ inline int pack_blocks_total(const PackAll& A, int threads) { return pack_plain_blocks(A, threads) + fold_blocks(A, threads); }
__device__ __forceinline__ void pack_block(const PackAll& A, int bid, int threads, double* red) {
    const int plain = pack_plain_blocks(A, threads);
    if (bid < plain) {
        const int total = pack_elems_total(A);
#pragma unroll
        for (int j = 0; j < kPackPerThread; ++j) {
            const int t = (bid * kPackPerThread + j) * threads + (int)threadIdx.x;
            if (t < total) pack_flat(A, t);
        }
    } else if (threads >= 512) {
        fold_block<8>(A, bid - plain, threads, red);
    } else {
        fold_block<4>(A, bid - plain, threads, red);
    }
}
int launch_pack(const PackAll& A, hipStream_t s);
int pending_pack_leave(const PackAll& A, hipStream_t s);
bool pending_pack_take(hipStream_t s, PackAll* out);
int pending_pack_flush(hipStream_t consumer);

int launch_slot_sums(const ReduceAll& R, hipStream_t s);
int pending_slot_sums_leave(const ReduceAll& R, hipStream_t s);
bool pending_slot_sums_take(hipStream_t s, ReduceAll* out);
int pending_slot_sums_flush();
bool pending_slot_sums_write(const float* grads);

}
```

### piml_amd/ops.py

```python
import collections
import ctypes
import math

import torch

from . import _lib

MAX_TOPK = 32
import contextlib
import functools
import os as _os
DETERMINISTIC_BWD = _os.environ.get('PIML_DETERMINISTIC_BWD', '0') == '1'


@functools.lru_cache(maxsize=None)
def cos_threshold(angle_deg):
    return float(torch.tensor(math.cos(3.14 * angle_deg / 180), dtype=torch.float32))


def _gpu_f32(name, t):
    if not isinstance(t, torch.Tensor) or not t.is_cuda:
        raise _lib.PimlHipError(f'{name}: expected a GPU tensor (piml_amd has no CPU path), got '
                                f'{getattr(t, "device", type(t))}')
    if t.dtype != torch.float32:
        raise TypeError(f'{name}: expected float32, got {t.dtype}')
    return t.contiguous()


def _stream():
    return torch.cuda.current_stream().cuda_stream


def _ptr(t):
    return None if t is None or t.numel() == 0 else t.data_ptr()


def heading_direction(velocity):
    v = _gpu_f32('velocity', velocity)
    if v.dim() < 3:
        raise ValueError('velocity must be (*c, t, N, 2)')
    T, N = v.shape[-3], v.shape[-2]
    C = v.numel() // max(T * N * 2, 1)
    out = torch.empty_like(v)
    with torch.cuda.device(v.device):
        _lib.check(_lib.lib().piml_heading_fwd(_ptr(v), C, T, N, _ptr(out), _stream()), 'piml_heading_fwd')
    return out


RelGeom = collections.namedtuple('RelGeom', 'kp ko cos_p cos_o dthr_p dthr_o')


def _rel_geom(topk_ped, sight_angle_ped, dist_threshold_ped, topk_obs, sight_angle_obs, dist_threshold_obs):
    if topk_ped > MAX_TOPK or topk_obs > MAX_TOPK:
        raise ValueError(f'topk must be <= {MAX_TOPK}')
    return RelGeom(int(topk_ped), int(topk_obs), cos_threshold(sight_angle_ped), cos_threshold(sight_angle_obs),
                   float(dist_threshold_ped), float(dist_threshold_obs))


_FEAT_DTYPES = (torch.float32,) * 3 + (torch.int32,) * 2


def _feat_shapes(lead, n, kpe, koe, width):
    return (*lead, n, kpe, 6), (*lead, n, koe, 6), (*lead, n, width), (*lead, n, kpe), (*lead, n, koe)


def _alloc_feats(lead, n, kpe, koe, width, device):
    return tuple(torch.empty(s, device=device, dtype=dt) for s, dt in zip(_feat_shapes(lead, n, kpe, koe, width), _FEAT_DTYPES))


def _fresh_zeros(shape, device):
    return torch.zeros(shape, device=device, dtype=torch.float32)


def _dense(grads, shapes, device, zeros):
    return [zeros(s, device) if g is None else _gpu_f32('grad', g) for g, s in zip(grads, shapes)]


def _separate_state(position, velocity, acceleration, destination):
    p, v, a, d = [_gpu_f32(n, x) for n, x in (('position', position), ('velocity', velocity),
                                              ('acceleration', acceleration), ('destination', destination))]
    if not (p.shape == v.shape == a.shape == d.shape) or p.shape[-1] != 2 or p.dim() < 2:
        raise ValueError(f'position/velocity/acceleration/destination must share a (..., N, 2) shape, got '
                         f'{tuple(p.shape)} {tuple(v.shape)} {tuple(a.shape)} {tuple(d.shape)}')
    N = p.shape[-2]
    return p, v, a, d, N, tuple(p.shape[:-2]), p.numel() // max(N * 2, 1)


def _packed_state(state, destination_rows, focal_count, flat=False):
    s = _gpu_f32('state', state)
    d_rows = _gpu_f32('destination_rows', destination_rows)
    if s.shape[-1] != 6 or (s.dim() != 2 if flat else s.dim() < 2):
        raise ValueError(f'state must be {"(N, 6)" if flat else "(..., N, 6)"}, got {tuple(s.shape)}')
    N = s.shape[-2]
    lead = tuple(s.shape[:-2])
    if tuple(d_rows.shape) != (*lead, focal_count, 2):
        raise ValueError(f'destination_rows must be {(*lead, focal_count, 2)}, got {tuple(d_rows.shape)}')
    return s, d_rows, N, lead, s.numel() // max(N * 6, 1)


def _focal_speed(desired_speed, focal_count):
    w = _gpu_f32('desired_speed', desired_speed)
    if w.numel() != focal_count:
        raise ValueError('destination_rows (n, 2) and desired_speed (n, 1) expected for the focal rows')
    return w


def _launch_relfeat_fwd(p_ptr, v_ptr, a_ptr, ld, hd, dest_rows, o, lead, C, N, f0, fcnt, geo, device,
                        outs=None, dest_ld=2, tick=None):
    M = o.shape[0]
    kpe, koe = min(geo.kp, N), min(geo.ko, M)
    if outs is None:
        outs = _alloc_feats(lead, fcnt, kpe, koe, 2, device)
    else:
        for t, shp, dt in zip(outs, _feat_shapes(lead, fcnt, kpe, koe, dest_ld), _FEAT_DTYPES):
            if tuple(t.shape) != shp or t.dtype != dt or not t.is_contiguous() or t.device != device:
                raise ValueError(f'output buffer mismatch: expected {shp} {dt}, got {tuple(t.shape)} {t.dtype}')
    ped_feat, obs_feat, dest_feat, ped_idx, obs_idx = outs
    args = (p_ptr, _ptr(hd), v_ptr, a_ptr, ld, _ptr(dest_rows), _ptr(o), C, N, M, f0, fcnt, *geo,
            _ptr(ped_feat), _ptr(obs_feat), _ptr(dest_feat), dest_ld, _ptr(ped_idx), _ptr(obs_idx))
    with torch.cuda.device(device):
# ... 24 lines not shown
        with torch.cuda.device(device):
            _lib.check(_lib.lib().piml_relfeat_bwd_det(
                _ptr(g_ped), _ptr(g_obs), _ptr(g_dest), _ptr(ped_idx), _ptr(obs_idx), _ptr(sorted_keys), _ptr(order),
                p_ptr, ld, _ptr(dest_rows), C, N, f0, fcnt, kpe, koe, int(seeded), _ptr(g_state), _ptr(g_dest_rows),
                _stream()), 'piml_relfeat_bwd_det')
        return g_state, g_dest_rows
    with torch.cuda.device(device):
        _lib.check(_lib.lib().piml_relfeat_bwd(
            _ptr(g_ped), _ptr(g_obs), _ptr(g_dest), _ptr(ped_idx), _ptr(obs_idx), p_ptr, ld,
            _ptr(dest_rows), C, N, f0, fcnt, kpe, koe, _ptr(g_state), _ptr(g_dest_rows), _stream()),
            'piml_relfeat_bwd')
    return g_state, g_dest_rows


def _relfeat_self_fwd(p, v, a, d, o, v0, lead, C, N, geo, g_state):
    M = o.shape[0]
    outs = _alloc_feats(lead, N, min(geo.kp, N), min(geo.ko, M), 7, p.device)
    with torch.cuda.device(p.device):
        _lib.check(_lib.lib().piml_relfeat_fwd_self(
            _ptr(p), None, _ptr(v), _ptr(a), 2, _ptr(d), _ptr(o), _ptr(v0), C, N, M, 0, N, *geo,
            *[_ptr(x) for x in outs], _ptr(g_state), _stream()), 'piml_relfeat_fwd_self')
    return outs


def _relfeat_self_bwd(grads, pi, oi, p, d, lead, C, N, g_state, g_speed, zeros):
    kpe, koe = pi.shape[-1], oi.shape[-1]
    g_ped, g_obs, g_self = _dense(grads, _feat_shapes(lead, N, kpe, koe, 7), p.device, zeros)
    if g_state is None:
        g_state = _fresh_zeros((*lead, N, 6), p.device)
    g_dest = torch.empty(*lead, N, 2, device=p.device, dtype=torch.float32)
    with torch.cuda.device(p.device):
        _lib.check(_lib.lib().piml_relfeat_bwd_self(
            _ptr(g_ped), _ptr(g_obs), _ptr(g_self), _ptr(pi), _ptr(oi), _ptr(p), 2, _ptr(d), C, N, 0, N, kpe, koe,
            _ptr(g_state), _ptr(g_dest), _ptr(g_speed), _stream()), 'piml_relfeat_bwd_self')
    return g_state, g_dest


class _RelativeFeatures(torch.autograd.Function):

    @staticmethod
    def forward(ctx, position, velocity, acceleration, destination, obstacles, heading, focal_begin, focal_count, geo):
        p, v, a, d, N, lead, C = _separate_state(position, velocity, acceleration, destination)
        o = _gpu_f32('obstacles', obstacles).reshape(-1, 2)
        if focal_count is None:
            focal_begin, focal_count = 0, N
        hd = None if heading is None else _gpu_f32('heading', heading)
        d_rows = d if focal_count == N else d[..., focal_begin:focal_begin + focal_count, :].contiguous()
        out = _launch_relfeat_fwd(_ptr(p), _ptr(v), _ptr(a), 2, hd, d_rows, o, lead, C, N, focal_begin,
                                  focal_count, geo, p.device)
        ctx.save_for_backward(out[3], out[4], p, d_rows)
        ctx.geom = (C, N, focal_begin, focal_count, out[3].shape[-1], out[4].shape[-1], lead)
        ctx.mark_non_differentiable(out[3], out[4])
        ctx.set_materialize_grads(False)
        return out

    @staticmethod
    def backward(ctx, g_ped, g_obs, g_dest, _gi, _go):
        if g_ped is None and g_obs is None and g_dest is None:
            return (None,) * 9
        ped_idx, obs_idx, p, d_rows = ctx.saved_tensors
        C, N, f0, fcnt, kpe, koe, lead = ctx.geom
        g_state, g_d_rows = _launch_relfeat_bwd(ctx.geom, g_ped, g_obs, g_dest, ped_idx, obs_idx,
                                                _ptr(p), 2, d_rows, p.device)
        if fcnt == N:
            g_destination = g_d_rows
        else:
            g_destination = torch.zeros(*lead, N, 2, device=p.device, dtype=torch.float32)
            g_destination[..., f0:f0 + fcnt, :] = g_d_rows
        return (g_state[..., 0:2], g_state[..., 2:4], g_state[..., 4:6], g_destination) + (None,) * 5


class _RelativeFeaturesSelf(torch.autograd.Function):

    @staticmethod
    def forward(ctx, position, velocity, acceleration, destination, obstacles, desired_speed, geo):
        p, v, a, d, N, lead, C = _separate_state(position, velocity, acceleration, destination)
        o = _gpu_f32('obstacles', obstacles).reshape(-1, 2)
        v0 = _gpu_f32('desired_speed', desired_speed)
        if v0.numel() != C * N:
            raise ValueError(f'desired_speed must hold one value per agent, got {tuple(v0.shape)}')
        outs = _relfeat_self_fwd(p, v, a, d, o, v0, lead, C, N, geo, None)
        ctx.save_for_backward(outs[3], outs[4], p, d)
        ctx.geom = (C, N, lead, tuple(desired_speed.shape))
        ctx.mark_non_differentiable(outs[3], outs[4])
        ctx.set_materialize_grads(False)
        return outs

    @staticmethod
    def backward(ctx, g_ped, g_obs, g_self, _gi, _go):
        if g_ped is None and g_obs is None and g_self is None:
            return (None,) * 7
        pi, oi, p, d = ctx.saved_tensors
        C, N, lead, speed_shape = ctx.geom
        g_speed = torch.empty(speed_shape, device=p.device, dtype=torch.float32) if ctx.needs_input_grad[5] else None
        g_state, g_dest = _relfeat_self_bwd((g_ped, g_obs, g_self), pi, oi, p, d, lead, C, N, None, g_speed, _fresh_zeros)
        return (g_state[..., 0:2], g_state[..., 2:4], g_state[..., 4:6], g_dest, None, g_speed, None)


class _RelativeFeaturesPacked(torch.autograd.Function):

    @staticmethod
    def forward(ctx, state, destination_rows, obstacles, focal_begin, focal_count, geo):
        s, d_rows, N, lead, C = _packed_state(state, destination_rows, focal_count)
        o = _gpu_f32('obstacles', obstacles).reshape(-1, 2)
        base = s.data_ptr()
        out = _launch_relfeat_fwd(base, base + 8, base + 16, 6, None, d_rows, o, lead, C, N, focal_begin,
                                  focal_count, geo, s.device)
        ctx.save_for_backward(out[3], out[4], s, d_rows)
        ctx.geom = (C, N, focal_begin, focal_count, out[3].shape[-1], out[4].shape[-1], lead)
        ctx.mark_non_differentiable(out[3], out[4])
        ctx.set_materialize_grads(False)
        return out

    @staticmethod
    def backward(ctx, g_ped, g_obs, g_dest, _gi, _go):
        if g_ped is None and g_obs is None and g_dest is None:
            return (None,) * 6
        ped_idx, obs_idx, s, d_rows = ctx.saved_tensors
        g_state, g_d_rows = _launch_relfeat_bwd(ctx.geom, g_ped, g_obs, g_dest, ped_idx, obs_idx,
                                                s.data_ptr(), 6, d_rows, s.device)
        return (g_state, g_d_rows) + (None,) * 4


class _RelativeFeaturesPackedSelf(torch.autograd.Function):

    @staticmethod
    def forward(ctx, state, destination_rows, obstacles, desired_speed, focal_begin, focal_count, geo, local=None):
        s, d_rows, N, _, _ = _packed_state(state, destination_rows, focal_count, flat=True)
        o = _gpu_f32('obstacles', obstacles).reshape(-1, 2)
        w = _focal_speed(desired_speed, focal_count)
        M = o.shape[0]
        kpe, koe = min(geo.kp, N), min(geo.ko, M)
        need_grad = any(ctx.needs_input_grad[:4]) and not DETERMINISTIC_BWD
        if local is None:
            outs = _alloc_feats((), focal_count, kpe, koe, 7, s.device)
            ctx.g_state = torch.empty(N, 6, device=s.device, dtype=torch.float32) if need_grad else None
            with torch.cuda.device(s.device):
                _lib.check(_lib.lib().piml_relfeat_self_fwd(
                    _ptr(s), _ptr(d_rows), _ptr(o), _ptr(w), N, M, focal_begin, focal_count, *geo,
                    *[_ptr(x) for x in outs], _ptr(ctx.g_state), _stream()), 'piml_relfeat_self_fwd')
        else:
            if local.geom != (s.data_ptr(), N, M, focal_begin, focal_count, geo):
                raise ValueError('relative_features_packed_self: `local` was made for another state buffer / geometry')
            outs = (local.ped_feat, local.obs_feat, local.self_features, local.ped_idx, local.obs_idx)
            ctx.g_state = local.g_state if need_grad else None
            local.g_state = None
            with torch.cuda.device(s.device):
                _lib.check(_lib.lib().piml_relfeat_self_fwd_part(
                    2, _ptr(s), None, None, None, N, M, focal_begin, focal_count, *geo,
                    _ptr(outs[0]), None, None, _ptr(outs[3]), None, None, _stream()),
                    'piml_relfeat_self_fwd_part(REMOTE)')
        ctx.save_for_backward(outs[3], outs[4], s, d_rows)
        ctx.geom = (1, N, focal_begin, focal_count, kpe, koe, ())
        ctx.speed_shape = tuple(desired_speed.shape)
        ctx.mark_non_differentiable(outs[3], outs[4])
        ctx.set_materialize_grads(False)
        return outs

    @staticmethod
    def backward(ctx, g_ped, g_obs, g_self, _gi, _go):
        if g_ped is None and g_obs is None and g_self is None:
            return (None,) * 8
        ped_idx, obs_idx, s, d_rows = ctx.saved_tensors
        _, N, f0, fcnt, kpe, koe, _ = ctx.geom
        opt = dict(device=s.device, dtype=torch.float32)
        if DETERMINISTIC_BWD:
            g_dest, g_speed = None, None
            if g_self is None:
                g_state = torch.zeros(N, 6, **opt)
            else:
                g_self = g_self.contiguous()
                g_state = torch.empty(N, 6, **opt) if fcnt == N else torch.zeros(N, 6, **opt)
                g_dest = torch.empty(fcnt, 2, **opt)
                g_speed = torch.empty(ctx.speed_shape, **opt) if ctx.needs_input_grad[3] else None
                with torch.cuda.device(s.device):
                    _lib.check(_lib.lib().piml_self_features_bwd(_ptr(g_self), fcnt, _ptr(g_dest),
                                                                 g_state.data_ptr() + 24 * f0, _ptr(g_speed),
                                                                 _stream()), 'piml_self_features_bwd')
            g_state, g_d_rows = _launch_relfeat_bwd(ctx.geom, g_ped, g_obs, g_dest, ped_idx, obs_idx, s.data_ptr(), 6,
                                                    d_rows, s.device, g_state=g_state)
            return (g_state, g_d_rows, None, g_speed) + (None,) * 4
        g_ped, g_obs, g_self = _dense((g_ped, g_obs, g_self), _feat_shapes((), fcnt, kpe, koe, 7), s.device, _fresh_zeros)
        g_state, ctx.g_state = ctx.g_state, None
        if g_state is None:
            g_state = torch.zeros(N, 6, **opt)
        g_d_rows = torch.empty(fcnt, 2, **opt)
        g_speed = torch.empty(ctx.speed_shape, **opt) if ctx.needs_input_grad[3] else None
        with torch.cuda.device(s.device):
            _lib.check(_lib.lib().piml_relfeat_self_bwd(
                _ptr(g_ped), _ptr(g_obs), _ptr(g_self), _ptr(ped_idx), _ptr(obs_idx), _ptr(s), _ptr(d_rows), N, f0, fcnt,
                kpe, koe, _ptr(g_state), _ptr(g_d_rows), _ptr(g_speed), _stream()), 'piml_relfeat_self_bwd')
        return (g_state, g_d_rows, None, g_speed) + (None,) * 4


class LocalFeatures:

    def __init__(self):
        self.ped_feat = self.obs_feat = self.self_features = self.ped_idx = self.obs_idx = self.g_state = None
        self.geom = None


def relative_features_local_part(state, destination_rows, obstacles, desired_speed, focal_begin, focal_count,
                                 topk_ped=6, sight_angle_ped=90, dist_threshold_ped=4,
                                 topk_obs=10, sight_angle_obs=90, dist_threshold_obs=4, want_grad=True):
    geo = _rel_geom(topk_ped, sight_angle_ped, dist_threshold_ped, topk_obs, sight_angle_obs, dist_threshold_obs)
    focal_begin, focal_count = int(focal_begin), int(focal_count)
    s, d_rows, N, _, _ = _packed_state(state.detach(), destination_rows.detach(), focal_count, flat=True)
    o = _gpu_f32('obstacles', obstacles.detach()).reshape(-1, 2)
    w = _focal_speed(desired_speed.detach(), focal_count)
# ... 1443 lines not shown


class _CollisionCorrection(torch.autograd.Function):
    @staticmethod
    def forward(ctx, predictions, ped_features, velocity, thr, dt):
        P = _gpu_f32('predictions', predictions)
        F = _gpu_f32('ped_features', ped_features)
        V = _gpu_f32('velocity', velocity)
        k, stride = F.shape[-2], F.shape[-1]
        rows = P.numel() // 2
        out = torch.empty_like(P)
        with torch.cuda.device(P.device):
            _lib.check(_lib.lib().piml_collision_correction_fwd(_ptr(P), _ptr(F), _ptr(V), rows, k, stride, float(thr),
                                                                float(dt), _ptr(out), _stream()),
                       'piml_collision_correction_fwd')
        ctx.save_for_backward(P, F, V)
        ctx.cfg = (rows, k, stride, float(thr), float(dt))
        ctx.set_materialize_grads(False)
        return out

    @staticmethod
    @torch.autograd.function.once_differentiable
    def backward(ctx, g):
        if g is None:
            return (None,) * 5
        P, F, V = ctx.saved_tensors
        rows, k, stride, thr, dt = ctx.cfg
        need = ctx.needs_input_grad
        gP = torch.empty_like(P) if need[0] else None
        gF = torch.empty_like(F) if need[1] else None
        gV = torch.empty_like(V) if need[2] else None
        with torch.cuda.device(P.device):
            _lib.check(_lib.lib().piml_collision_correction_bwd(_ptr(g.contiguous()), _ptr(P), _ptr(F), _ptr(V), rows, k,
                                                                stride, thr, dt, _ptr(gP), _ptr(gF), _ptr(gV),
                                                                _stream()), 'piml_collision_correction_bwd')
        return gP, gF, gV, None, None


def collision_post_correction(predictions, ped_features, velocity, collision_threshold=0.5, time_unit=0.08):
    if predictions.shape[-1] != 2 or velocity.shape != predictions.shape or ped_features.dim() != predictions.dim() + 1 \
            or ped_features.shape[:-2] != predictions.shape[:-1] or ped_features.shape[-1] < 4:
        raise ValueError('collision_post_correction: predictions / velocity (..., N, 2) and ped_features '
                         '(..., N, k, >= 4) expected')
    return _CollisionCorrection.apply(predictions, ped_features, velocity, collision_threshold, time_unit)


ENCODER_HIDDEN = 128
RELU_MASK = _os.environ.get('PIML_RELU_MASK', '1') != '0'
ENCODER_MAX_IN = 8


def _enc_branch_struct(x2, k, scale, wb, msgs, h1=None, h2=None, g_pooled=None, g_msgs=None, g2=None, g1=None,
                       g_x=None, partials=None, packed=None, grads=None, keep_bits=None, draw_p=None, relu_mask=None,
                       sum_a=None, sum_b=None):
    B = _lib.EncoderBranch()
    B.sum_a, B.sum_b = _ptr(sum_a), _ptr(sum_b)
    B.keep_bits = _ptr(keep_bits)
    if draw_p is not None:
        B.drop_state, B.drop_p = dropout_state(x2.device).data_ptr(), float(draw_p)
    B.x, B.rows, B.in_dim, B.k = x2.data_ptr(), x2.shape[0], x2.shape[1], int(k)
    B.w1, B.b1, B.w2, B.b2, B.w3, B.b3 = [t.data_ptr() for t in wb]
    B.scale = float(scale)
    B.h1, B.h2, B.msgs = _ptr(h1), _ptr(h2), _ptr(msgs)
    B.g_pooled, B.g_msgs, B.g2, B.g1, B.g_x, B.partials = [_ptr(t) for t in (g_pooled, g_msgs, g2, g1, g_x, partials)]
    B.packed, B.grads = _ptr(packed), _ptr(grads)
    R = x2.shape[0]
    B.relu_mask = (h2.data_ptr() + R * h2.shape[1] * 4) if (RELU_MASK and h2 is not None and h2.shape[0] >= R + 2 * ((R + 31) // 32)) else None
    if relu_mask is not None:
        B.relu_mask = relu_mask.data_ptr()
    return B


H1_RECOMPUTE = _os.environ.get('PIML_H1_RECOMPUTE', '1') != '0'


def _h1_needed(rows_per_branch, alone=True):
    if not (H1_RECOMPUTE and RELU_MASK):
        return True
    L = _lib.lib()
    per_branch = [(r + 31) // 32 for r in rows_per_branch]
    tiles = min(per_branch)
    if not (L.piml_encoder_products(-1) == 1 and L.piml_encoder_dw2(-1) == 1 and tiles > L.piml_encoder_split_tiles_train(-1)):
        return True
    arr = (_lib.EncoderBranch * len(rows_per_branch))()
    for b, r in enumerate(rows_per_branch):
        arr[b].rows = r
    w0 = ctypes.c_int(0)
    total = L.piml_encoder_workgroups(arr, len(rows_per_branch), ctypes.byref(w0))
    w = [total] if len(rows_per_branch) == 1 else [w0.value, total - w0.value]
    return min(w) < 2


def _h2_buffer(R, opt):
    return torch.empty(R + 2 * ((R + 31) // 32), ENCODER_HIDDEN, **opt)


class _FusedEncoders(torch.autograd.Function):

    @staticmethod
    def forward(ctx, nbr, scales, want_pooled, need_grad, keeps, packs, *tensors):
        L = _lib.lib()
        xs = [tensors[7 * b] for b in range(nbr)]
        wbs = [[_gpu_f32('encoder weight', t.detach()) for t in tensors[7 * b + 1:7 * b + 7]] for b in range(nbr)]
        dev = xs[0].device
        x2s, msgs, h1s, h2s, ks = [], [], [], [], []
        opt = dict(device=dev, dtype=torch.float32)
        for b in range(nbr):
            x = _gpu_f32('encoder input', xs[b])
            x2 = x.reshape(-1, x.shape[-1])
# ... 332 lines not shown
    if not ok:
        ok = all(getattr(p, 'grad', None) is None and id(p) not in _DEFER_SEEN and not getattr(p, '_backward_hooks', None)
                 and not getattr(p, '_post_accumulate_grad_hooks', None) for p in params)
        if ok:
            _DEFER_SEEN.update(id(p) for p in params)
    if ok:
        _DEFER_DEVS.add(dev)
    else:
        _flush_deferred_sums()
    return ok


class _FusedPinnsf(torch.autograd.Function):
    PER = 13
    FIRST = 10
    SELF = 9

    @staticmethod
    def forward(ctx, need_grad, nbr, scales, tau, fold_epilogue, packs, nhead, keeps, sums, self_features, *tensors):
        L = _lib.lib()
        PER = _FusedPinnsf.PER
        xs = [tensors[PER * b] for b in range(nbr)]
        ewb = [[_gpu_f32('encoder weight', t.detach()) for t in tensors[PER * b + 1:PER * b + 7]] for b in range(nbr)]
        dwb = [[_gpu_f32('decoder weight', t.detach()) for t in tensors[PER * b + 7:PER * b + 13]] for b in range(nbr)]
        hwb = [_gpu_f32('head weight', t.detach()) for t in tensors[PER * nbr:PER * nbr + 4]] if nhead else None
        dev = xs[0].device
        opt = dict(device=dev, dtype=torch.float32)
        H = ENCODER_HIDDEN
        lead = tuple(xs[0].shape[:-2])
        agents = 1
        for d in lead:
            agents *= d
        sf = _gpu_f32('self_features', self_features).reshape(agents, 7) if fold_epilogue else None
        x2s, ks, msgs, h1s, h2s = [], [], [], [], []
        msum = False
        for b in range(nbr):
            x = _gpu_f32('encoder input', xs[b])
            if tuple(x.shape[:-2]) != lead:
                raise ValueError('fused_pinnsf: both branches must share the leading (..., N) shape')
            x2s.append(x.reshape(-1, x.shape[-1]))
            ks.append(x.shape[-2])
        if sums:
            probe = (_lib.EncoderBranch * nbr)()
            for b in range(nbr):
                probe[b].rows, probe[b].in_dim, probe[b].k = x2s[b].shape[0], x2s[b].shape[1], ks[b]
            wanted = sums
            sums = bool(L.piml_pinnsf_pool_train_ok(probe, nbr)) and not FORK_NETWORK and \
                (packs is None or packs.fold == tuple(float(sc) for sc in scales)) and all(k is None for k in keeps)
            if wanted and not sums and need_grad and not FORK_NETWORK and RELU_MASK and POOL_MSGS:
                for b in range(nbr):
                    probe[b].relu_mask = 1
                msum = bool(L.piml_pinnsf_pool_msgs_ok(probe, nbr))
        ctx.sums = sums
        sum_a, sum_b, masks = [None] * nbr, [None] * nbr, [None] * nbr
        for b in range(nbr):
            R = x2s[b].shape[0]
            h1s.append(None)
            if msum:
                msgs.append(torch.empty(R, H, **opt) if (nhead and b == 0) else None)
                sum_a[b], sum_b[b] = torch.empty(agents, H, **opt), torch.empty(agents, H, **opt)
                h2s.append(_h2_buffer(R, opt))
            elif sums:
                msgs.append(None)
                sum_a[b], sum_b[b] = torch.empty(agents, H, **opt), torch.empty(agents, H, **opt)
                masks[b] = torch.empty(2 * ((R + 31) // 32), H, **opt)
                h2s.append(torch.empty(R, H, **opt) if (nhead and b == 0) else None)
            else:
                msgs.append(torch.empty(R, H, **opt))
                h2s.append(_h2_buffer(R, opt) if need_grad else None)
        if not sums and need_grad and _h1_needed([x2.shape[0] for x2 in x2s], alone=False):
            h1s = [torch.empty(x2.shape[0], H, **opt) for x2 in x2s]
        flags = (_lib.FORK if FORK_NETWORK else 0) | (_lib.POOL_TRAIN if sums else 0) | (_lib.POOL_MSGS if msum else 0)
        if packs is not None:
            if packs.sig != _weights_sig(ewb, dwb, hwb):
                raise ValueError('fused_pinnsf: `packs` were filled from other weight tensors, or the weights were modified in '
                                 'place since (optimizer step / load_state_dict inside a packed_weights() block): pinnsf_prepack first')
            epack, dpack, hpack = packs.epack, packs.dpack, packs.hpack
            flags |= _lib.PACKED_VALID
        else:
            epack = torch.empty(nbr, L.piml_encoder_pack_floats(), **opt)
            dpack = torch.empty(nbr, L.piml_decoder_pack_floats(), **opt)
            hpack = torch.empty(L.piml_collision_head_pack_floats(), **opt) if nhead else None
        keeps, draws = zip(*[_resolve_keep(keeps[b], x2s[b].shape[0], H, dev) for b in range(nbr)])
        earr = (_lib.EncoderBranch * nbr)(*[_enc_branch_struct(x2s[b], ks[b], scales[b], ewb[b], msgs[b], h1s[b], h2s[b],
                                                               packed=epack[b], keep_bits=keeps[b], draw_p=draws[b],
                                                               relu_mask=masks[b], sum_a=sum_a[b], sum_b=sum_b[b])
                                            for b in range(nbr)])
        pooled = sum_a if (sums or msum) else [torch.empty(agents, H, **opt) for _ in range(nbr)]
        dh1 = [torch.empty(agents, 64, **opt) if need_grad else None for _ in range(nbr)]
        dd2 = [torch.empty(agents, 64, **opt) if need_grad else None for _ in range(nbr)]
        folds = [(ewb[b][4], ewb[b][5], scales[b]) if sums else None for b in range(nbr)]
        darr = (_lib.DecoderBranch * nbr)(*[_dec_branch_struct(sum_b[b] if (sums or msum) else msgs[b], agents, ks[b], dwb[b], dpack[b], pooled[b],
                                                               dh1[b], dd2[b], fold=folds[b]) for b in range(nbr)])
        acc = torch.empty(agents, 2, **opt)
        head, coll = None, None
        if nhead:
            coll = torch.empty(x2s[0].shape[0], **opt)
            head = _lib.CollisionHead()
            head.msgs, head.rows = (h2s[0] if sums else msgs[0]).data_ptr(), x2s[0].shape[0]
            head.w1, head.b1, head.w2, head.b2 = [t.data_ptr() for t in hwb]
            head.packed, head.out = hpack.data_ptr(), coll.data_ptr()
            if sums:
                head.fold_w3, head.fold_b3, head.fold_scale = ewb[0][4].data_ptr(), ewb[0][5].data_ptr(), float(scales[0])
        with torch.cuda.device(dev):
            _lib.check(L.piml_pinnsf_fwd(earr, darr, nbr, ctypes.byref(head) if head is not None else None, _ptr(sf),
                                         float(tau), _ptr(acc), flags, _stream()), 'piml_pinnsf_fwd')
        if need_grad:
            saved_msgs = sum_b if sums else ([msgs[b] if msgs[b] is not None else sum_b[b] for b in range(nbr)] if msum else msgs)
            ctx.save_for_backward(*x2s, *h1s, *(masks if sums else h2s), *saved_msgs, *pooled, *dh1, *dd2,
                                  *[w for wb in ewb for w in wb],
                                  *[w for wb in dwb for w in wb], epack, dpack, *([sf] if sf is not None else []),
                                  *(hwb if nhead else []))
        ctx.meta = (nbr, tuple(scales), float(tau), bool(fold_epilogue), tuple(ks), [tuple(x.shape) for x in xs],
                    tuple(self_features.shape), agents, need_grad, int(nhead))
        ctx.keeps = keeps
        ctx.sink = ParamGradSink._active if need_grad else None
        ctx.params = tensors if need_grad else None
        ctx.set_materialize_grads(False)
        out = (acc.view(*lead, 2), *[None if (sums or msum) else msgs[b].view(*lead, ks[b], H) for b in range(nbr)])
        if nhead:
            out = out + (coll.view(*lead, ks[0]),)
        return out

    @staticmethod
    @torch.autograd.function.once_differentiable
    def backward(ctx, g_acc, *g_rest):
        nbr, scales, tau, fold, ks, xshapes, sf_shape, agents, need_grad, nhead = ctx.meta
        PER, FIRST = _FusedPinnsf.PER, _FusedPinnsf.FIRST
        nin = FIRST + PER * nbr + 4 * nhead
        grads = [None] * nin
        g_msgs = list(g_rest[:nbr])
        g_coll = g_rest[nbr] if nhead else None
        if not need_grad or (g_acc is None and g_coll is None and all(g is None for g in g_msgs)):
            return tuple(grads)
        L = _lib.lib()
        sv = list(ctx.saved_tensors)
        take = lambda n: [sv.pop(0) for _ in range(n)]
        x2s, h1s, h2s, msgs, pooled, dh1, dd2 = [take(nbr) for _ in range(7)]
        ewb = [take(6) for _ in range(nbr)]
# ... 80 lines not shown
                    dW1, dW2 = flat[:64 * H].view(64, H), flat[64 * H:64 * H + 4096].view(64, 64)
                    dW3 = flat[64 * H + 4096:64 * H + 4096 + 128].view(2, 64)
                    rest = flat[64 * H + 4096 + 128:]
                    for jx, t in enumerate((dW1, rest[:64], dW2, rest[64:128], dW3, rest[128:130])):
                        if need[jx]:
                            if sink is not None:
                                sink.give(ctx.params[o + jx - FIRST], t)
                            else:
                                grads[o + jx] = t
            else:
                if h1s[live[0]] is None and _h1_needed([x2s[b].shape[0] for b in live], alone=False):
                    raise _lib.PimlHipError(
                        'fused_pinnsf: a backward pass through the messages of a subset of the branches only needs the '
                        'layer-1 activations, which the forward did not store; run it with PIML_H1_RECOMPUTE=0')
                _lib.check(L.piml_encoder_bwd(earr, len(live), _stream()), 'piml_encoder_bwd')
            for i, b in enumerate(live):
                flat = flats[i]
                in_dim = x2s[b].shape[1]
                o = FIRST + PER * b
                need = ctx.needs_input_grad[o:o + 7]
                if need[0]:
                    grads[o] = keep[i][3].view(xshapes[b])
                dW3, dW2 = flat[:H * H].view(H, H), flat[H * H:2 * H * H].view(H, H)
                dW1 = flat[2 * H * H:2 * H * H + H * in_dim].view(H, in_dim)
                db3, db2, db1 = flat[2 * H * H + 8 * H:].view(3, H)
                for jx, t in zip(range(1, 7), (dW1, db1, dW2, db2, dW3, db3)):
                    if need[jx]:
                        if sink is not None:
                            sink.give(ctx.params[o + jx - FIRST], t)
                        else:
                            grads[o + jx] = t
        return tuple(grads)


def _backward_sums(ctx, g_acc, g_coll, grads, x2s, masks, pooled, dh1, dd2, ewb, dwb, epack, dpack, sf):
    nbr, scales, tau, fold, ks, xshapes, sf_shape, agents, need_grad, nhead = ctx.meta
    PER, FIRST = _FusedPinnsf.PER, _FusedPinnsf.FIRST
    if g_coll is not None:
        raise _lib.PimlHipError('fused_pinnsf(sums=True): the collision head\'s output received a gradient; this form serves callers '
                                'that train on predictions[0] only (model.messages_wanted = True selects the message path)')
    if g_acc is None:
        return tuple(grads)
    L = _lib.lib()
    dev = x2s[0].device
    opt = dict(device=dev, dtype=torch.float32)
    H = ENCODER_HIDDEN
    with torch.cuda.device(dev):
        part1 = H * H + 1024 + 2 * H
        g_pooled = [torch.empty(agents, H, **opt) for _ in range(nbr)]
        gxs = [torch.empty(x2s[b].shape, **opt) if ctx.needs_input_grad[FIRST + PER * b] else None for b in range(nbr)]
        if len({g is None for g in gxs}) > 1:
            gxs = [g if g is not None else torch.empty(x2s[b].shape, **opt) for b, g in enumerate(gxs)]
        earr = (_lib.EncoderBranch * nbr)(*[_enc_branch_struct(x2s[b], ks[b], scales[b], ewb[b], None, None, None, g_pooled[b], None,
                                                               None, None, gxs[b], packed=epack[b], relu_mask=masks[b])
                                            for b in range(nbr)])
        w0 = ctypes.c_int(0)
        total = L.piml_encoder_workgroups(earr, nbr, ctypes.byref(w0))
        slots = [w0.value, total - w0.value] if nbr == 2 else [total]
        parts = [torch.empty(n, part1, **opt) for n in slots]
        sink = ParamGradSink.current(ctx.sink)
        flags = _lib.POOL_TRAIN
        flats = dflats = dw1 = None
        if sink is not None:
            ids = lambda lo, hi: tuple(id(t) for t in ctx.params[lo:hi])
            flats, acc_e = sink.take([ids(PER * b + 1, PER * b + 7) for b in range(nbr)], L.piml_encoder_partial_floats(), opt)
            dflats, acc_d = sink.take([ids(PER * b + 7, PER * b + 13) for b in range(nbr)], L.piml_decoder_partial_floats(), opt, mode='fold')
            dw1, _ = sink.take([ids(PER * b + 7, PER * b + 13) for b in range(nbr)], 64 * H, opt, mode='fold')
            if acc_e != acc_d:
                raise _lib.PimlHipError('fused_pinnsf(sums=True): the encoders and decoders of one network went through different numbers '
                                        'of backward passes inside ParamGradSink.step()')
            if acc_e:
                flags |= _lib.ACCUMULATE
            flags |= _lib.DEFER_UNFOLD
        else:
            flats = [torch.empty(L.piml_encoder_partial_floats(), **opt) for _ in range(nbr)]
        for b in range(nbr):
            earr[b].partials, earr[b].grads = parts[b].data_ptr(), flats[b].data_ptr()
        ga = _gpu_f32('g_acc', g_acc).reshape(agents, 2)
        want_self = fold and ctx.needs_input_grad[_FusedPinnsf.SELF]
        g_self = torch.empty(agents, 7, **opt) if want_self else None
        nwg = L.piml_decoder_workgroups(agents)
        dparts = [torch.empty(nwg, L.piml_decoder_partial_floats(), **opt) for _ in range(nbr)]
        if sink is None:
            dflats = [torch.empty(L.piml_decoder_partial_floats(), **opt) for _ in range(nbr)]
            dw1 = [torch.empty(64 * H, **opt) for _ in range(nbr)]
        keep, dstructs = [], []
        for b in range(nbr):
            gp2, gp1 = torch.empty(agents, 64, **opt), torch.empty(agents, 64, **opt)
            keep += [gp2, gp1]
            dstructs.append(_dec_branch_struct(pooled[b], agents, ks[b], dwb[b], dpack[b], pooled[b], dh1[b], dd2[b], gp2, gp1,
                                               g_pooled[b], dparts[b], dflats[b], fold=(ewb[b][4], ewb[b][5], scales[b]), dw1_out=dw1[b]))
        darr = (_lib.DecoderBranch * nbr)(*dstructs)
        if _defer_slot_sums([ctx.params[PER * b + jx] for b in range(nbr) for jx in range(1, 13)], sink, dev):
            flags |= _lib.DEFER_SLOT_SUMS
            _defer_keep(parts, dparts, dflats, flats, dw1)
        _lib.check(L.piml_pinnsf_bwd(earr, darr, nbr, _ptr(ga), _ptr(sf), float(tau), _ptr(g_self), flags, _stream()), 'piml_pinnsf_bwd')
        if want_self:
            grads[_FusedPinnsf.SELF] = g_self.view(sf_shape)
        for b in range(nbr):
            flat = dflats[b]
            o = FIRST + PER * b + 7
            need = ctx.needs_input_grad[o:o + 6]
            dW2 = flat[64 * H:64 * H + 4096].view(64, 64)
            dW3 = flat[64 * H + 4096:64 * H + 4096 + 128].view(2, 64)
            rest = flat[64 * H + 4096 + 128:]
            for jx, t in enumerate((dw1[b].view(64, H), rest[:64], dW2, rest[64:128], dW3, rest[128:130])):
                if need[jx]:
                    if sink is not None:
                        sink.give(ctx.params[o + jx - FIRST], t)
                    else:
                        grads[o + jx] = t
            flat = flats[b]
            in_dim = x2s[b].shape[1]
            o = FIRST + PER * b
            need = ctx.needs_input_grad[o:o + 7]
            if need[0]:
                grads[o] = gxs[b].view(xshapes[b])
            dW3, dW2 = flat[:H * H].view(H, H), flat[H * H:2 * H * H].view(H, H)
            dW1 = flat[2 * H * H:2 * H * H + H * in_dim].view(H, in_dim)
            db3, db2, db1 = flat[2 * H * H + 8 * H:].view(3, H)
            for jx, t in zip(range(1, 7), (dW1, db1, dW2, db2, dW3, db3)):
                if need[jx]:
                    if sink is not None:
                        sink.give(ctx.params[o + jx - FIRST], t)
                    else:
                        grads[o + jx] = t
    return tuple(grads)


_FusedPinnsf._backward_sums = staticmethod(_backward_sums)


def fused_pinnsf(branches, self_features, tau, fold_epilogue=True, head=None, packs=None, sums=False):
    if not 1 <= len(branches) <= 2:
        raise ValueError('fused_pinnsf: one or two branches')
    flat = []
    for br in branches:
        x, e, d, p = br['x'], br['encoder'], br['decoder'], br['predictor']
        if not x.is_cuda:
            raise _lib.PimlHipError('fused_pinnsf: expected GPU tensors (piml_amd has no CPU path)')
        H = ENCODER_HIDDEN
        ok = (x.dim() >= 3 and 1 <= x.shape[-1] <= ENCODER_MAX_IN and x.numel() > 0 and
              [tuple(t.shape) for t in e] == [(H, x.shape[-1]), (H,), (H, H), (H,), (H, H), (H,)] and
              [tuple(t.shape) for t in d] == [(64, H), (64,), (64, 64), (64,)] and
              [tuple(t.shape) for t in p] == [(2, 64), (2,)])
        if not ok:
            raise ValueError('fused_pinnsf: unsupported geometry (encoder in<=8 -> 128 x3, decoder 128 -> 64 -> 64, '
                             'predictor 64 -> 2)')
# ... 395 lines not shown
```

Baseline: 229.4 billion.

## Compact obstacle-encoder rows to agents with neighbors, handling empty agents in closed form

Builds a per-call plan that splits agents into those with valid obstacle neighbors and those without. The encoder backward then processes tiles only for the non-empty agents, gathering rows through the plan. Agents with no neighbors take a precomputed zero-input activation row (relu(b1), relu(W2·relu(b1)+b2)) and contribute to bias and weight gradients in closed form. This avoids running the MLP backward on padding rows, at the cost of extra plan bookkeeping, indirect loads, a Python-side cache of neighbor indices keyed by data pointer, and several new constraints on when the path is enabled.

```diff
diff --git a/include/piml_hip.h b/include/piml_hip.h
--- a/include/piml_hip.h
+++ b/include/piml_hip.h
@@ -429,7 +429,13 @@
     unsigned long long* drop_state;
     float drop_p;
     float *sum_a, *sum_b;
+    const int* nbr_idx;
+    int* plan;
 } piml_encoder_branch;
+#define PIML_COMPACT_MAX_AGENTS 16384
+#define PIML_COMPACT_PLAN_INTS(agents) (16 + 2 * (((agents) + 3) / 4 * 4))
+#define PIML_COMPACT_TILES(agents, k) (((agents) + 32 / (k) - 1) / (32 / (k)))
+#define PIML_COMPACT_SLOTS 256
 
 int piml_encoder_partial_floats(void);
 int piml_encoder_pack_floats(void);
diff --git a/include/piml_hip_tuning.h b/include/piml_hip_tuning.h
--- a/include/piml_hip_tuning.h
+++ b/include/piml_hip_tuning.h
@@ -27,6 +27,7 @@
 int piml_encoder_fused_bwd(int on);
 int piml_encoder_sums_bwd(int form);
 int piml_encoder_sums_dec_slots(int on);
+int piml_encoder_compact_rows(int on);
 int piml_pinnsf_streams_init(void);
 
 #ifdef __cplusplus
diff --git a/piml_amd/_lib.py b/piml_amd/_lib.py
--- a/piml_amd/_lib.py
+++ b/piml_amd/_lib.py
@@ -6,6 +6,8 @@
 _HERE = os.path.dirname(os.path.abspath(__file__))
 LIB_PATH = os.environ.get('PIML_LIB') or os.path.join(_HERE, 'libpiml_hip.so')
 ABI_VERSION = 35
+COMPACT_MAX_AGENTS = 16384
+COMPACT_SLOTS = 256
 
 _lib = None
 
@@ -19,7 +21,8 @@
                 ('w1', _p), ('b1', _p), ('w2', _p), ('b2', _p), ('w3', _p), ('b3', _p),
                 ('scale', _f), ('h1', _p), ('h2', _p), ('msgs', _p), ('g_pooled', _p), ('g_msgs', _p),
                 ('g2', _p), ('g1', _p), ('g_x', _p), ('partials', _p), ('grads', _p), ('packed', _p), ('relu_mask', _p),
-                ('keep_bits', _p), ('drop_state', _p), ('drop_p', _f), ('sum_a', _p), ('sum_b', _p)]
+                ('keep_bits', _p), ('drop_state', _p), ('drop_p', _f), ('sum_a', _p), ('sum_b', _p),
+                ('nbr_idx', _p), ('plan', _p)]
 
 
 class DecoderBranch(ctypes.Structure):
@@ -210,6 +213,7 @@
     'piml_encoder_fused_bwd': [_i],
     'piml_encoder_sums_bwd': [_i],
     'piml_encoder_sums_dec_slots': [_i],
+    'piml_encoder_compact_rows': [_i],
     'piml_encoder_pack': [ctypes.POINTER(EncoderBranch), _i, _p],
     'piml_encoder_workgroups': [ctypes.POINTER(EncoderBranch), _i, ctypes.POINTER(_i)],
     'piml_encoder_fwd': [ctypes.POINTER(EncoderBranch), _i, _p],
diff --git a/piml_amd/csrc/encoder.hip b/piml_amd/csrc/encoder.hip
--- a/piml_amd/csrc/encoder.hip
+++ b/piml_amd/csrc/encoder.hip
@@ -24,6 +24,13 @@
     const piml_encoder_branch J = b ? A.br[1] : A.br[0];
     const int e = blockIdx.x * 256 + threadIdx.x;
     if (e < PACK_FLOATS) J.packed[e] = pack_value(J, e);
+    else if (e < PACK_FLOATS + EH) J.packed[e] = fmaxf(J.b1[e - PACK_FLOATS], 0.f);
+    else if (e < PACK_TOTAL) {
+        const int j = e - PACK_FLOATS - EH;
+        double sum = 0.0;
+        for (int q = 0; q < EH; ++q) sum += (double)J.w2[(size_t)j * EH + q] * (double)fmaxf(J.b1[q], 0.f);
+        J.packed[e] = fmaxf((float)((double)J.b2[j] + sum), 0.f);
+    }
 }
 
 constexpr int FWD_LDS_FLOATS = 16384 * 2 + 1024 + 384;
@@ -732,7 +739,7 @@
     return total;
 }
 
-PIML_API int piml_encoder_pack_floats(void) { return PACK_FLOATS; }
+PIML_API int piml_encoder_pack_floats(void) { return PACK_TOTAL; }
 
 static int enc_check(const piml_encoder_branch* br, int nbr) {
     if (!br || nbr < 1 || nbr > 2) return hipErrorInvalidValue;
@@ -764,7 +771,7 @@
     A.zero = nullptr;
     A.zero_n = 0;
     A.gen_state = nullptr;
-    hipLaunchKernelGGL(enc_pack_kernel, dim3((PACK_FLOATS + 255) / 256, nbr), dim3(256), 0, s, A);
+    hipLaunchKernelGGL(enc_pack_kernel, dim3((PACK_TOTAL + 255) / 256, nbr), dim3(256), 0, s, A);
     return hipGetLastError();
 }
 
@@ -1133,9 +1140,22 @@
     return tiles >= 0 && tiles > g_split_tiles_train;
 }
 
+static int enc_compact_asked(const piml_encoder_branch* br, int nbr, bool fwd) {
+    bool any = false;
+    for (int i = 0; i < nbr; ++i) any = any || br[i].plan || br[i].nbr_idx;
+    if (!any) return 0;
+    if (nbr != 2 || br[0].plan || br[0].nbr_idx || !br[1].plan || (fwd && !br[1].nbr_idx)) return -1;
+    const piml_encoder_branch& b = br[1];
+    if ((b.k != 2 && b.k != 6 && b.k != 10) || br[0].k < 1 || br[0].k > 16 || b.rows % b.k || b.rows / b.k > PIML_COMPACT_MAX_AGENTS ||
+        b.in_dim != 6 || br[0].in_dim != 6 || b.h2 || g_sums_bwd == 1)
+        return -1;
+    return 1;
+}
+
 int piml::enc_stage_fwd_sum(const piml_encoder_branch* br, int nbr, hipStream_t s, float* zero, long long zero_n) {
     if (int e = enc_check(br, nbr)) return e;
     if (!enc_pool_train_ok(br, nbr)) return hipErrorInvalidValue;
+    if (enc_compact_asked(br, nbr, true) < 0) return hipErrorInvalidValue;
     for (int i = 0; i < nbr; ++i)
         if (!br[i].sum_a || !br[i].sum_b || !br[i].relu_mask) return hipErrorInvalidValue;
     EncArgs A;
@@ -1154,14 +1174,22 @@
         const piml_encoder_branch& b = br[i];
         if (!b.g_pooled || b.g_msgs || !b.relu_mask || !b.partials || !b.grads || (b.g_x != nullptr) != (br[0].g_x != nullptr)) return hipErrorInvalidValue;
     }
+    const int compact = enc_compact_asked(br, nbr, false);
+    if (compact < 0) return hipErrorInvalidValue;
     EncArgs A;
     const int total = fill_args(A, br, nbr);
+    if (compact && total != PIML_COMPACT_SLOTS) return hipErrorInvalidValue;
     if (int e = x3_ready()) return e;
     static int ready = -1;
     if (ready < 0) { ready = enc_f3_set_attributes(); if (!ready) ready = enc_f5_set_attributes(); }
     if (ready) return ready;
     const int nA[2] = {nbr > 1 ? A.wg_split : total, nbr > 1 ? total - A.wg_split : 0};
     const int zero[2] = {0, 0};
+    if (compact) {
+        if (!enc_f5_launch(A, nA, s, dec)) return hipErrorInvalidValue;
+        if (dec_summed) *dec_summed = dec && dec->nsets > 0;
+        return hipGetLastError();
+    }
     if (g_sums_bwd == 1 || !enc_f5_launch(A, nA, s, dec)) enc_f3_launch(A, nA, zero, false, s, true);
     else if (dec_summed) *dec_summed = dec && dec->nsets > 0;
     return hipGetLastError();
diff --git a/piml_amd/csrc/encoder.hpp b/piml_amd/csrc/encoder.hpp
--- a/piml_amd/csrc/encoder.hpp
+++ b/piml_amd/csrc/encoder.hpp
@@ -10,6 +10,7 @@
 
 constexpr int ENC_THREADS = 512;
 constexpr int ENC_WAVES = ENC_THREADS / 64;
+constexpr int CP_LISTS = 16;
 
 struct EncArgs {
     piml_encoder_branch br[2];
diff --git a/piml_amd/csrc/encoder_bwd5.hip b/piml_amd/csrc/encoder_bwd5.hip
--- a/piml_amd/csrc/encoder_bwd5.hip
+++ b/piml_amd/csrc/encoder_bwd5.hip
@@ -94,8 +94,9 @@
         __builtin_amdgcn_sched_barrier(0);       \
     } while (0)
 
-template <bool GX, int INC>
-__global__ __launch_bounds__(F5_THREADS) void enc_bwd_sums2_kernel(F5Args F) {
+template <bool GX, int INC, int CPM>
+__device__ __forceinline__ void enc_bwd_sums2_body(const F5Args& F) {
+    constexpr bool CP = CPM != 0;
     extern __shared__ __align__(16) unsigned char smem[];
     const int tid = threadIdx.x, lane = tid & 63;
     const int wv = __builtin_amdgcn_readfirstlane(tid >> 6);
@@ -103,13 +104,22 @@
     const int ctid = tid & 255;
     const int n = lane & 31, h = lane >> 5;
     int bx = (int)blockIdx.x, b = 0;
-    if (bx >= F.nA[0]) { b = 1; bx -= F.nA[0]; }
+    const int* __restrict__ plan = CP ? F.A.br[1].plan : nullptr;
+    int nA0 = F.nA[0], nA1 = F.nA[1], nne = 0, nemp = 0, ctiles = 0;
+    if (CP) {
+        nne = __builtin_amdgcn_readfirstlane(plan[0]); nemp = __builtin_amdgcn_readfirstlane(plan[1]);
+        ctiles = __builtin_amdgcn_readfirstlane(plan[2]);
+        nA0 = __builtin_amdgcn_readfirstlane(plan[3]); nA1 = __builtin_amdgcn_readfirstlane(plan[4]);
+    }
+    if (CPM == 2 || (CPM == 0 && bx >= nA0)) { b = 1; bx -= nA0; }
     const piml_encoder_branch J = b ? F.A.br[1] : F.A.br[0];
-    const int nwg = F.nA[b];
+    const int nwg = b ? nA1 : nA0;
+    constexpr bool cp = CPM == 2;
+    const bool cpe = cp && nemp > 0;
     const unsigned R = (unsigned)J.rows;
     const unsigned IN = __builtin_amdgcn_readfirstlane((unsigned)J.in_dim), K = __builtin_amdgcn_readfirstlane((unsigned)J.k);
     const unsigned kmagic = __builtin_amdgcn_readfirstlane((unsigned)((0x100000000ull + K - 1) / K));
-    const int ntiles = (int)((R + 31) >> 5);
+    const int ntiles = cp ? ctiles : (int)((R + 31) >> 5);
     const int nit = bx < ntiles ? (ntiles - bx + nwg - 1) / nwg : 0;
     float* P = J.partials + (size_t)bx * F5_PART1;
     constexpr int NS = INC == 6 ? 3 : 4;
@@ -122,6 +132,8 @@
     const __amdgpu_buffer_rsrc_t rs_x = rsrc(J.x, R * IN * 4);
     const __amdgpu_buffer_rsrc_t rs_mk = rsrc(J.relu_mask, (unsigned)ntiles * 1024);
     const __amdgpu_buffer_rsrc_t rs_gx = rsrc(J.g_x, GX ? R * IN * 4 : 0u);
+    const unsigned cS = CP ? 32u / K : 1u;
+    const __amdgpu_buffer_rsrc_t rs_pl = rsrc(CP ? plan + CP_LISTS : nullptr, CP ? (unsigned)nne * 4u : 0u);
     auto ld1 = [&](const __amdgpu_buffer_rsrc_t& rs, unsigned voff, unsigned soff) {
         return (unsigned)__builtin_amdgcn_raw_buffer_load_b32(rs, (int)voff, (int)soff, 0);
     };
@@ -185,7 +197,25 @@
         float g2[16];
         unsigned m2 = 0, mkv = 0;
         float xa[NS];
+        const unsigned slot_n = CP ? (unsigned)n / K : 0u, kn = (unsigned)n - slot_n * K;
+        int av = -1;
+        auto plan_req = [&](int tile) {
+            const unsigned idx = cS * (unsigned)tile + slot_n;
+            const bool ok = (tile < ntiles) & (slot_n < cS) & (idx < (unsigned)nne);
+            const unsigned v = ld1(rs_pl, ok ? idx * 4u : kOut, 0u);
+            av = ok ? (int)v : -1;
+        };
         auto req_g = [&](int tile) {
+            if (CP && cp) {
+#pragma unroll
+                for (int r = 0; r < 16; ++r) {
+                    const int sa = __builtin_amdgcn_readlane(av, f5_rho(r)), sb = __builtin_amdgcn_readlane(av, f5_rho(r) + 4);
+                    const int a_ = h ? sb : sa;
+                    g2[r] = __uint_as_float(ld1(rs_gp, a_ >= 0 ? gbase + (unsigned)a_ * (EH * 4) : kOut, 0u));
+                }
+                m2 = ld1(rs_mk, tile < ntiles ? (unsigned)tile * 1024u + (128u + 2u * (unsigned)lane + (unsigned)(w >> 1)) * 4u : kOut, 0u);
+                return;
+            }
             const unsigned t32 = __builtin_amdgcn_readfirstlane((unsigned)tile * 32u);
             const unsigned a0 = __builtin_amdgcn_readfirstlane(__umulhi(t32, kmagic)), rem = t32 - a0 * K;
             const bool live = tile < ntiles;
@@ -202,14 +232,15 @@
             m2 = ld1(rs_mk, live ? (unsigned)tile * 1024u + (128u + 2u * (unsigned)lane + (unsigned)(w >> 1)) * 4u : kOut, 0u);
         };
         auto req_x = [&](int tile) {
-            const unsigned row = (unsigned)tile * 32u + (unsigned)n;
-            const bool valid = (tile < ntiles) & (row < R);
+            const unsigned row = (CP && cp) ? (unsigned)av * K + kn : (unsigned)tile * 32u + (unsigned)n;
+            const bool valid = (CP && cp) ? av >= 0 : (tile < ntiles) & (row < R);
 #pragma unroll
             for (int s = 0; s < NS; ++s) {
                 const unsigned cx = 2u * s + h;
                 xa[s] = __uint_as_float(ld1(rs_x, (valid & (cx < IN)) ? (row * IN + cx) * 4u : kOut, 0u));
             }
             mkv = ld1(rs_mk, tile < ntiles ? (unsigned)tile * 1024u + (unsigned)(ctid & 127) * 4u : kOut, 0u);
+            if (CP && cp) plan_req(tile + nwg);
         };
         float db1 = 0.f, db2 = 0.f;
         unsigned phi[4], pmid[4], plo[4];
@@ -279,6 +310,7 @@
         };
 
         F5_BARRIER();
+        if (CP && cp) plan_req(bx);
         req_g(bx);
         req_x(bx);
 #pragma unroll
@@ -358,6 +390,24 @@
             f5_dec_sums(F.D, (int)blockIdx.x, (int)gridDim.x, ctid, 256);
             F5_STAMP(12);
         }
+        if (CP && cpe) {
+            const float* sv = reinterpret_cast<const float*>(smem + F5_W1);
+            const float* __restrict__ wc = J.w2 + (size_t)(64 * h) * EH + 32 * w + n;
+            float pacc = 0.f;
+#pragma unroll 1
+            for (int q0 = 0; q0 < 64; q0 += 16) {
+                float w2c[16];
+#pragma unroll
+                for (int q = 0; q < 16; ++q) w2c[q] = wc[(size_t)(q0 + q) * EH];
+#pragma unroll
+                for (int q = 0; q < 16; ++q) pacc = __fmaf_rn(w2c[q], sv[64 * h + q0 + q], pacc);
+            }
+            pacc += __shfl_xor(pacc, 32, 64);
+            if (h == 0) {
+                db1 += J.packed[PACK_ZROW + 32 * w + n] > 0.f ? pacc : 0.f;
+                db2 += sv[32 * w + n];
+            }
+        }
         F5_BARRIER();
         F5_BARRIER();
         db1 += __shfl_xor(db1, 32, 64);
@@ -403,13 +453,23 @@
 #pragma unroll
             for (int p = 0; p < 3; ++p) o[p] = hr[((jb_ * 2 + s_) * 3 + p) * 64];
         };
+        const unsigned slot_m = CP ? (unsigned)(ctid >> 3) / K : 0u, km = (unsigned)(ctid >> 3) - slot_m * K;
+        int bav = -1;
         auto gx_store = [&](int tile, int pm) {
-            const unsigned grow = (unsigned)tile * 32u + (unsigned)(ctid >> 3), cs = (unsigned)ctid & 7u;
+            const unsigned grow = (CP && cp) ? (unsigned)bav * K + km : (unsigned)tile * 32u + (unsigned)(ctid >> 3), cs = (unsigned)ctid & 7u;
             const float* gp = reinterpret_cast<const float*>(smem + F5_GXP + pm * F5_GXP_BYTES) + (ctid >> 3) * 16 + (ctid & 7);
             const float v = ((gp[0] + gp[512]) + gp[1024]) + gp[1536];
             const bool cok = cs < IN;
             const unsigned off = (grow * IN + cs) * 4u;
-            __builtin_amdgcn_raw_buffer_store_b32(__float_as_uint(v), rs_gx, (int)(((tile >= 0) & (tile < ntiles) & (grow < R) & cok) ? off : kOut), 0, 0);
+            const bool rok = (CP && cp) ? bav >= 0 : (tile >= 0) & (tile < ntiles) & (grow < R);
+            __builtin_amdgcn_raw_buffer_store_b32(__float_as_uint(v), rs_gx, (int)((rok & cok) ? off : kOut), 0, 0);
+            if (CP && cp) {
+                const int nt = tile + nwg;
+                const unsigned idx = cS * (unsigned)nt + slot_m;
+                const bool ok = (nt >= 0) & (nt < ntiles) & (slot_m < cS) & (idx < (unsigned)nne);
+                const unsigned pv = ld1(rs_pl, ok ? idx * 4u : kOut, 0u);
+                bav = ok ? (int)pv : -1;
+            }
         };
         float g1[16];
         float4 xv[2][4];
@@ -476,8 +536,34 @@
         };
 
         F5_BARRIER();
+        if (CP && cpe) {
+            const int* __restrict__ eo = plan + CP_LISTS + (((int)(R / K) + 3) & ~3);
+            const float* __restrict__ gp = J.g_pooled + 32 * w + n;
+            float sacc = 0.f;
+            for (int e0 = bx + h * nwg; e0 < nemp; e0 += 16 * nwg) {
+                int ai[8];
+                float gv[8];
+#pragma unroll
+                for (int u = 0; u < 8; ++u) ai[u] = eo[min(e0 + 2 * u * nwg, nemp - 1)];
+#pragma unroll
+                for (int u = 0; u < 8; ++u) gv[u] = gp[(size_t)ai[u] * EH];
+#pragma unroll
+                for (int u = 0; u < 8; ++u) sacc += e0 + 2 * u * nwg < nemp ? gv[u] : 0.f;
+            }
+            sacc += __shfl_xor(sacc, 32, 64);
+            if (h == 0) reinterpret_cast<float*>(smem + F5_W1)[32 * w + n] = J.packed[PACK_ZROW + EH + 32 * w + n] > 0.f ? (float)K * sacc : 0.f;
+        }
         F5_STAMP(15);
         F5_BARRIER();
+        if (CP && cpe) {
+            const float* sv = reinterpret_cast<const float*>(smem + F5_W1) + 32 * w + 4 * h;
+#pragma unroll
+            for (int jb = 0; jb < 4; ++jb) {
+                const float h1v = J.packed[PACK_ZROW + 32 * jb + n];
+#pragma unroll
+                for (int r = 0; r < 16; ++r) c[jb][r] = sv[f5_rho(r)] * h1v;
+            }
+        }
         for (int it = 0; it < nit; ++it) {
             const int par = it & 1, tile = bx + it * nwg;
             F5_STAMP(0);
@@ -548,6 +634,13 @@
         for (int i = 0; i < 16; ++i) g_f5_stamps[(blockIdx.x * 8 + wv) * 16 + i] = st[i];
 #endif
 }
+template <bool GX, int INC>
+__global__ __launch_bounds__(F5_THREADS) void enc_bwd_sums2_kernel(F5Args F) { enc_bwd_sums2_body<GX, INC, 0>(F); }
+template <bool GX>
+__global__ __launch_bounds__(F5_THREADS) void enc_bwd_sums2_cp_kernel(F5Args F) {
+    if ((int)blockIdx.x < __builtin_amdgcn_readfirstlane(F.A.br[1].plan[3])) enc_bwd_sums2_body<GX, 6, 1>(F);
+    else enc_bwd_sums2_body<GX, 6, 2>(F);
+}
 
 #ifdef PIML_F5_STAMPS
 extern "C" __attribute__((visibility("default"))) int piml_f5_stamps(unsigned long long* out) {
@@ -560,6 +653,8 @@
     if (int e = set(reinterpret_cast<const void*>(enc_bwd_sums2_kernel<false, 6>))) return e;
     if (int e = set(reinterpret_cast<const void*>(enc_bwd_sums2_kernel<true, 6>))) return e;
     if (int e = set(reinterpret_cast<const void*>(enc_bwd_sums2_kernel<false, 8>))) return e;
+    if (int e = set(reinterpret_cast<const void*>(enc_bwd_sums2_cp_kernel<false>))) return e;
+    if (int e = set(reinterpret_cast<const void*>(enc_bwd_sums2_cp_kernel<true>))) return e;
     return set(reinterpret_cast<const void*>(enc_bwd_sums2_kernel<true, 8>));
 }
 
@@ -575,7 +670,10 @@
     }
     const bool gx = A.br[0].g_x != nullptr;
     const dim3 g((unsigned)(F.nA[0] + F.nA[1])), blk(F5_THREADS);
-    if (in6) {
+    if (A.nbr > 1 && A.br[1].plan) {
+        if (gx) hipLaunchKernelGGL((enc_bwd_sums2_cp_kernel<true>), g, blk, F5_LDS_LAUNCH, s, F);
+        else hipLaunchKernelGGL((enc_bwd_sums2_cp_kernel<false>), g, blk, F5_LDS_LAUNCH, s, F);
+    } else if (in6) {
         if (gx) hipLaunchKernelGGL((enc_bwd_sums2_kernel<true, 6>), g, blk, F5_LDS_LAUNCH, s, F);
         else hipLaunchKernelGGL((enc_bwd_sums2_kernel<false, 6>), g, blk, F5_LDS_LAUNCH, s, F);
     } else {
diff --git a/piml_amd/csrc/encoder_x3.hip b/piml_amd/csrc/encoder_x3.hip
--- a/piml_amd/csrc/encoder_x3.hip
+++ b/piml_amd/csrc/encoder_x3.hip
@@ -536,7 +536,67 @@
     }
 }
 
-__global__ __launch_bounds__(ENC_THREADS) void enc_fwd_sum_x3_kernel(EncArgs A) {
+constexpr int CP_LDS_CNT = X3_IMG;
+constexpr int CP_LDS_LIST = X3_IMG + 1024;
+constexpr int CP_ROUNDS0 = 8;
+static_assert((CP_LDS_LIST - X3_IMG) * 4 + PIML_COMPACT_MAX_AGENTS * 2 <= (X3_FWD_F32 - X3_IMG) * 4, "the lists fit W3's region");
+static_assert(PIML_COMPACT_MAX_AGENTS <= 65536 && PIML_COMPACT_MAX_AGENTS <= 32 * ENC_THREADS, "u16 entries, a 32-bit flag word per thread");
+
+__device__ __forceinline__ bool cp_straddles(int agent, int k) { return ((agent * k) >> 5) != ((agent * k + k - 1) >> 5); }
+
+__device__ __forceinline__ unsigned cp_split_cost(int w0, int tiles0, int tiles1, int nemp) {
+    const int w1 = PIML_COMPACT_SLOTS - w0;
+    const unsigned c0 = (unsigned)((tiles0 + w0 - 1) / w0) * 6000u;
+    const unsigned c1 = (unsigned)((tiles1 + w1 - 1) / w1) * 6000u + (nemp > 0 ? 2500u + 40u * (unsigned)((nemp + w1 - 1) / w1) : 0u);
+    return min(c0 > c1 ? c0 : c1, (1u << 23) - 1u);
+}
+
+template <int K>
+__device__ __forceinline__ void pool_rows_c(const f32x16 (&a)[4], int tile, int nne, const unsigned short* list, int lane,
+                                            float* __restrict__ sum_a, float* __restrict__ sum_b) {
+    constexpr int S = 32 / K;
+    const int i = lane & 31;
+    const bool h = lane >= 32;
+    float tot[4][S];
+#pragma unroll
+    for (int blk = 0; blk < 4; ++blk) {
+        float sum[S];
+#pragma unroll
+        for (int s = 0; s < S; ++s) sum[s] = 0.f;
+#pragma unroll
+        for (int r = 0; r < 16; ++r) {
+            const int m0 = (r & 3) + 8 * (r >> 2), s0 = m0 / K, s1 = (m0 + 4) / K;
+            if (s0 == s1) {
+                if (s0 < S) sum[s0] += a[blk][r];
+            } else {
+                if (s0 < S) sum[s0] += h ? 0.f : a[blk][r];
+                if (s1 < S) sum[s1] += h ? a[blk][r] : 0.f;
+            }
+        }
+#pragma unroll
+        for (int s = 0; s < S; ++s) tot[blk][s] = add_halves(sum[s]);
+    }
+    const int left = nne - S * tile;
+    if (!h) {
+#pragma unroll
+        for (int s = 0; s < S; ++s) {
+            if (s < left) {
+                const int ag = list[S * tile + s];
+                float* __restrict__ dst = sum_a + (size_t)ag * EH + i;
+#pragma unroll
+                for (int blk = 0; blk < 4; ++blk) dst[32 * blk] = tot[blk][s];
+                if (cp_straddles(ag, K)) {
+                    float* __restrict__ zb = sum_b + (size_t)ag * EH + i;
+#pragma unroll
+                    for (int blk = 0; blk < 4; ++blk) zb[32 * blk] = 0.f;
+                }
+            }
+        }
+    }
+}
+
+template <bool CP>
+__device__ __forceinline__ void enc_fwd_sum_body(const EncArgs& A) {
     extern __shared__ __align__(16) float lds[];
     const int tid = threadIdx.x, lane = tid & 63, wave = uniform((int)(threadIdx.x >> 6));
     const int b = (A.nbr > 1 && (int)blockIdx.x >= A.wg_split) ? 1 : 0;
@@ -545,23 +605,113 @@
     const int nwg = b ? (int)gridDim.x - A.wg_split : (A.nbr > 1 ? A.wg_split : (int)gridDim.x);
     const long long R = J.rows;
     const int IN = J.in_dim;
-    const long long ntiles = (R + 31) >> 5;
+    const bool cp = CP && b == 1;
+    long long ntiles = (R + 31) >> 5;
     const long long first = (long long)wave * nwg + ((int)blockIdx.x - wg0);
     const long long stride = (long long)nwg * ENC_WAVES;
     if (A.zero)
         for (int e = blockIdx.x * ENC_THREADS + tid; e < A.zero_n; e += gridDim.x * ENC_THREADS) A.zero[e] = 0.f;
-    if ((long long)((int)blockIdx.x - wg0) >= ntiles) return;
+    if (!cp && (long long)((int)blockIdx.x - wg0) >= ntiles) return;
     const float* x3 = J.packed + PACK_F32;
     float xb[4];
     ENC_STAMP(0, false);
-    load_x(xb, J.x, first, ntiles, R, IN, lane);
+    const int k = J.k;
+    const int agents = CP ? (int)(R / k) : 0;
+    int iv[CP_ROUNDS0];
+    if (cp) {
+#pragma unroll
+        for (int i = 0; i < CP_ROUNDS0; ++i) {
+            const int a = i * ENC_THREADS + tid;
+            iv[i] = a < agents ? J.nbr_idx[(size_t)a * k] : -1;
+        }
+    } else {
+        load_x(xb, J.x, first, ntiles, R, IN, lane);
+    }
     stage_linear<X3_IMG>(lds, x3, tid);
     stage_linear<1024 + 384>(lds + X3_FWD_F32, J.packed + 32768, tid);
     ENC_STAMP(1, true);
-    __syncthreads();
+    int nne = 0, nemp = 0, S = 1, slot_n = 0, kn = 0;
+    bool rowlive = false;
+    const unsigned short* list = reinterpret_cast<const unsigned short*>(lds + CP_LDS_LIST);
+    if (cp) {
+        int* cnt = reinterpret_cast<int*>(lds + CP_LDS_CNT);
+        unsigned short* lw = reinterpret_cast<unsigned short*>(lds + CP_LDS_LIST);
+        const int rounds = (agents + ENC_THREADS - 1) / ENC_THREADS;
+        unsigned flags = 0;
+#pragma unroll
+        for (int i = 0; i < CP_ROUNDS0; ++i) flags |= (iv[i] >= 0 ? 1u : 0u) << i;
+        for (int i = CP_ROUNDS0; i < rounds; ++i) {
+            const int a = i * ENC_THREADS + tid;
+            const int v = a < agents ? J.nbr_idx[(size_t)a * k] : -1;
+            flags |= (v >= 0 ? 1u : 0u) << i;
+        }
+        for (int i = 0; i < rounds; ++i) {
+            const unsigned long long bal = __ballot((flags >> i) & 1u);
+            if (lane == 0) cnt[i * ENC_WAVES + wave] = __popcll(bal);
+        }
+        __syncthreads();
+        if (wave == 0) {
+            int v[4], tot = 0;
+#pragma unroll
+            for (int u = 0; u < 4; ++u) { v[u] = 4 * lane + u < rounds * ENC_WAVES ? cnt[4 * lane + u] : 0; tot += v[u]; }
+            int inc = tot;
+#pragma unroll
+            for (int d = 1; d < 64; d <<= 1) {
+                const int o = __shfl_up(inc, d, 64);
+                if (lane >= d) inc += o;
+            }
+            int ex = inc - tot;
+#pragma unroll
+            for (int u = 0; u < 4; ++u) { cnt[4 * lane + u] = ex; ex += v[u]; }
+            if (lane == 63) cnt[256] = inc;
+        }
+        __syncthreads();
+        nne = uniform(cnt[256]);
+        nemp = agents - nne;
+        for (int i = 0; i < rounds; ++i) {
+            const int a = i * ENC_THREADS + tid;
+            const unsigned bit = (flags >> i) & 1u;
+            const unsigned long long bal = __ballot(bit);
+            const int pos = cnt[i * ENC_WAVES + wave] + __popcll(bal & ((1ull << lane) - 1ull));
+            if (a < agents) lw[bit ? pos : agents - 1 - (a - pos)] = (unsigned short)a;
+        }
+        S = 32 / k;
+        ntiles = (nne + S - 1) / S;
+        const int n = lane & 31;
+        slot_n = n / k; kn = n - slot_n * k; rowlive = slot_n < S;
+        if ((int)blockIdx.x == wg0) {
+            if (tid == 0) cnt[257] = 0x7fffffff;
+        }
+        __syncthreads();
+        if ((int)blockIdx.x == wg0) {
+            const int tiles0 = (int)((A.br[0].rows + 31) >> 5);
+            if (tid >= 2 && tid <= PIML_COMPACT_SLOTS - 2)
+                atomicMin(reinterpret_cast<unsigned*>(cnt + 257), cp_split_cost(tid, tiles0, (int)ntiles, nemp) * 256u + (unsigned)tid);
+            const int apad = (agents + 3) & ~3;
+            for (int c = tid; c < nne; c += ENC_THREADS) J.plan[CP_LISTS + c] = list[c];
+            for (int e = tid; e < nemp; e += ENC_THREADS) J.plan[CP_LISTS + apad + e] = list[agents - 1 - e];
+            __syncthreads();
+            if (tid == 0) {
+                const int w0 = cnt[257] & 255;
+                J.plan[0] = nne; J.plan[1] = nemp; J.plan[2] = (int)ntiles; J.plan[3] = w0; J.plan[4] = PIML_COMPACT_SLOTS - w0;
+            }
+        }
+    } else {
+        __syncthreads();
+    }
     ENC_STAMP(2, false);
-    const int k = J.k;
-    const long long agents = R / k;
+    auto load_xc = [&](long long tile) {
+        const int idx = S * (int)tile + slot_n;
+        const bool ok = tile < ntiles && rowlive && idx < nne;
+        const long long row = ok ? (long long)list[idx] * k + kn : 0;
+#pragma unroll
+        for (int s = 0; s < 4; ++s) {
+            const int c = 2 * s + (lane >> 5);
+            xb[s] = (ok && c < IN) ? J.x[row * IN + c] : 0.f;
+        }
+    };
+    if (cp) load_xc(first);
+    const long long agents_d = R / k;
     for (long long tile = first; tile < ntiles; tile += stride) {
         int lane_t = lane;
         asm volatile("" : "+v"(lane_t));
@@ -589,7 +739,8 @@
         ENC_STAMP(3, false);
         split_tile(a, P);
         ENC_STAMP(4, false);
-        load_x(xb, J.x, tile + stride, ntiles, R, IN, lane);
+        if (cp) load_xc(tile + stride);
+        else load_x(xb, J.x, tile + stride, ntiles, R, IN, lane);
 #pragma unroll
         for (int blk = 0; blk < 4; ++blk) {
             f32x16 acc, sm;
@@ -608,11 +759,32 @@
         mrow[64] = make_uint2(sign_bits(a[0], a[1]), sign_bits(a[2], a[3]));
         if (J.h2) store_h2_rows<true>(a, J.h2, tile, R, lane_t);
         ENC_STAMP(6, false);
-        pool_rows_k(a, k, tile, agents, lane_t, J.sum_a, J.sum_b);
+        if (cp) {
+            if (k == 10) pool_rows_c<10>(a, (int)tile, nne, list, lane_t, J.sum_a, J.sum_b);
+            else if (k == 6) pool_rows_c<6>(a, (int)tile, nne, list, lane_t, J.sum_a, J.sum_b);
+            else pool_rows_c<2>(a, (int)tile, nne, list, lane_t, J.sum_a, J.sum_b);
+        } else {
+            pool_rows_k(a, k, tile, agents_d, lane_t, J.sum_a, J.sum_b);
+        }
         ENC_STAMP(7, false);
     }
+    if (cp && nemp > 0) {
+        const int nwav = nwg * ENC_WAVES, idle = nwav - (int)ntiles;
+        const int q = idle > 0 ? (int)first - (int)ntiles : (int)first, share = idle > 0 ? idle : nwav;
+        if (q >= 0) {
+            const float2 hc = reinterpret_cast<const float2*>(J.packed + PACK_ZROW + EH)[lane];
+            const float2 v = make_float2((float)k * hc.x, (float)k * hc.y);
+            for (int e = q; e < nemp; e += share) {
+                const int ag = list[agents - 1 - e];
+                reinterpret_cast<float2*>(J.sum_a + (size_t)ag * EH)[lane] = v;
+                if (cp_straddles(ag, k)) reinterpret_cast<float2*>(J.sum_b + (size_t)ag * EH)[lane] = make_float2(0.f, 0.f);
+            }
+        }
+    }
     ENC_STAMP(8, true);
 }
+__global__ __launch_bounds__(ENC_THREADS) void enc_fwd_sum_x3_kernel(EncArgs A) { enc_fwd_sum_body<false>(A); }
+__global__ __launch_bounds__(ENC_THREADS) void enc_fwd_sum_x3_cp_kernel(EncArgs A) { enc_fwd_sum_body<true>(A); }
 
 constexpr int X3_SPLIT_LDS_BYTES = 2 * 2 * 4 * 3 * 2 * 64 * 16;
 
@@ -1140,6 +1312,7 @@
         if (int e = set(f, X3_DX_LDS_BYTES)) return e;
     if (int e = set(reinterpret_cast<const void*>(enc_fwd_pool_x3_kernel), X3_FWD_LDS_BYTES)) return e;
     if (int e = set(reinterpret_cast<const void*>(enc_fwd_sum_x3_kernel), X3_FWD_LDS_BYTES)) return e;
+    if (int e = set(reinterpret_cast<const void*>(enc_fwd_sum_x3_cp_kernel), X3_FWD_LDS_BYTES)) return e;
     if (int e = set(reinterpret_cast<const void*>(enc_fwd_x3_kernel<2, true>), X3_FWD_LDS_BYTES)) return e;
     if (int e = set(reinterpret_cast<const void*>(enc_fwd_x3_kernel<1, true>), X3_FWD_LDS_BYTES)) return e;
     if (int e = set(reinterpret_cast<const void*>(enc_fwd_x3_kernel<0, true>), X3_FWD_LDS_BYTES)) return e;
@@ -1174,7 +1347,8 @@
 }
 
 void enc_x3_launch_fwd_sum(const EncArgs& A, int total, hipStream_t s) {
-    hipLaunchKernelGGL(enc_fwd_sum_x3_kernel, dim3(total), dim3(ENC_THREADS), X3_FWD_LDS_BYTES, s, A);
+    if (A.nbr > 1 && A.br[1].plan) hipLaunchKernelGGL(enc_fwd_sum_x3_cp_kernel, dim3(total), dim3(ENC_THREADS), X3_FWD_LDS_BYTES, s, A);
+    else hipLaunchKernelGGL(enc_fwd_sum_x3_kernel, dim3(total), dim3(ENC_THREADS), X3_FWD_LDS_BYTES, s, A);
 }
 
 void enc_x3_launch_fwd(const EncArgs& A, int total, bool drop, hipStream_t s, bool exch) {
diff --git a/piml_amd/csrc/network.hip b/piml_amd/csrc/network.hip
--- a/piml_amd/csrc/network.hip
+++ b/piml_amd/csrc/network.hip
@@ -322,6 +322,7 @@
     for (int i = 0; i < nbr; ++i) {
         if (sums) {
             add(enc[i].partials, enc[i].grads, nbr == 1 ? total : (i == 0 ? w0 : total - w0), DW2_L1_LANES, DW2_L1_SPLIT, DW2_L1_OFF0, DW2_L1_OFF1);
+            if (nbr == 2 && enc[1].plan) R.set[n - 1].dev_slots = enc[1].plan + 3 + i;
             R.unf[i] = UnfoldSet{dec[i].grads, dec[i].w1, enc[i].w3, enc[i].b3, dec[i].fold_scale, enc[i].k, dec[i].dw1_out, enc[i].grads};
             R.nunf = nbr;
         } else if (dw2) {
@@ -347,6 +348,14 @@
 PIML_API int piml_encoder_sums_dec_slots(int on) {
     const int old = g_dec_slots_enc;
     if (on >= 0) g_dec_slots_enc = on ? 1 : 0;
+    return old;
+}
+
+static int g_compact_rows = !(getenv("PIML_ENC_COMPACT") && atoi(getenv("PIML_ENC_COMPACT")) == 0);
+
+PIML_API int piml_encoder_compact_rows(int on) {
+    const int old = g_compact_rows;
+    if (on >= 0) g_compact_rows = on ? 1 : 0;
     return old;
 }
 
diff --git a/piml_amd/csrc/pack.hpp b/piml_amd/csrc/pack.hpp
--- a/piml_amd/csrc/pack.hpp
+++ b/piml_amd/csrc/pack.hpp
@@ -20,6 +20,8 @@
 constexpr int X3_IMG = X3_HM + X3_LO;
 constexpr int PACK_X3 = 4 * X3_IMG;
 constexpr int PACK_FLOATS = PACK_F32 + PACK_X3;
+constexpr int PACK_ZROW = PACK_FLOATS;
+constexpr int PACK_TOTAL = PACK_FLOATS + 2 * EH;
 
 typedef float f32x2_t __attribute__((ext_vector_type(2)));
 typedef __bf16 bf16x2_t __attribute__((ext_vector_type(2)));
diff --git a/piml_amd/csrc/reduce.hpp b/piml_amd/csrc/reduce.hpp
--- a/piml_amd/csrc/reduce.hpp
+++ b/piml_amd/csrc/reduce.hpp
@@ -9,6 +9,7 @@
     const float* parts;
     float* grads;
     int slots, lanes, split, off0, off1;
+    const int* dev_slots;
 };
 struct UnfoldSet {
     const float* dgrads;
@@ -93,7 +94,7 @@
 __device__ __forceinline__ void reduce_block(const ReduceAll& A, int bid) {
     const int y = bid / A.gx, x = bid - y * A.gx;
     const ReduceSet S = A.set[y];
-    if (x * 16 < S.lanes) sum_slots_16x16_at(x, S.parts, S.grads, S.slots, S.lanes, S.split, S.off0, S.off1, A.accumulate != 0);
+    if (x * 16 < S.lanes) sum_slots_16x16_at(x, S.parts, S.grads, S.dev_slots ? *S.dev_slots : S.slots, S.lanes, S.split, S.off0, S.off1, A.accumulate != 0);
 }
 __device__ __forceinline__ void reduce_launch_block(const ReduceAll& A, int bid) {
     if (bid < A.unf_blocks) unfold_block(A, bid);
@@ -176,7 +177,32 @@
 __host__ __device__ inline int pack_plain_blocks(const PackAll& A, int threads) {
     return (pack_elems_total(A) + threads * kPackPerThread - 1) / (threads * kPackPerThread);
 }
-__host__ __device__ inline int pack_blocks_total(const PackAll& A, int threads) { return pack_plain_blocks(A, threads) + fold_blocks(A, threads); }
+__device__ __forceinline__ void zrow_block(const PackAll& A, int y, int threads, double* red) {
+    const piml_encoder_branch& J = A.enc[y];
+    const int t = (int)threadIdx.x, parts = threads >= 512 ? 4 : 2, per = EH / parts;
+    double part = 0.0;
+    if (t < parts * EH) {
+        const int j = t & (EH - 1), p = t >> 7;
+        const float* __restrict__ wr = J.w2 + (size_t)j * EH + p * per;
+        const float* __restrict__ br = J.b1 + p * per;
+        for (int q0 = 0; q0 < per; q0 += 16) {
+            float wv[16], bv[16];
+#pragma unroll
+            for (int u = 0; u < 16; ++u) { wv[u] = wr[q0 + u]; bv[u] = br[q0 + u]; }
+#pragma unroll
+            for (int u = 0; u < 16; ++u) part += (double)wv[u] * (double)fmaxf(bv[u], 0.f);
+        }
+    }
+    red[t] = part;
+    __syncthreads();
+    if (t < EH) {
+        double sum = 0.0;
+        for (int p = 0; p < parts; ++p) sum += red[t + p * EH];
+        J.packed[PACK_ZROW + t] = fmaxf(J.b1[t], 0.f);
+        J.packed[PACK_ZROW + EH + t] = fmaxf((float)((double)J.b2[t] + sum), 0.f);
+    }
+}
+__host__ __device__ inline int pack_blocks_total(const PackAll& A, int threads) { return pack_plain_blocks(A, threads) + fold_blocks(A, threads) + A.nbr; }
 __device__ __forceinline__ void pack_block(const PackAll& A, int bid, int threads, double* red) {
     const int plain = pack_plain_blocks(A, threads);
     if (bid < plain) {
@@ -186,6 +212,8 @@
             const int t = (bid * kPackPerThread + j) * threads + (int)threadIdx.x;
             if (t < total) pack_flat(A, t);
         }
+    } else if (bid >= plain + fold_blocks(A, threads)) {
+        zrow_block(A, bid - plain - fold_blocks(A, threads), threads, red);
     } else if (threads >= 512) {
         fold_block<8>(A, bid - plain, threads, red);
     } else {
diff --git a/piml_amd/ops.py b/piml_amd/ops.py
--- a/piml_amd/ops.py
+++ b/piml_amd/ops.py
@@ -1,4 +1,5 @@
 import collections
+import weakref
 import ctypes
 import math
 
@@ -66,6 +67,37 @@
 
 def _alloc_feats(lead, n, kpe, koe, width, device):
     return tuple(torch.empty(s, device=device, dtype=dt) for s, dt in zip(_feat_shapes(lead, n, kpe, koe, width), _FEAT_DTYPES))
+
+
+_NBR_IDX = collections.OrderedDict()
+_NBR_IDX_MAX = 8
+
+
+def _note_nbr_idx(feat, idx):
+    if feat is None or idx is None or feat.numel() == 0:
+        return
+    key = feat.data_ptr()
+    _NBR_IDX.pop(key, None)
+    for dead in [k for k, (ref, _, _) in _NBR_IDX.items() if ref() is None]:
+        del _NBR_IDX[dead]
+    while len(_NBR_IDX) >= _NBR_IDX_MAX:
+        _NBR_IDX.popitem(last=False)
+    _NBR_IDX[key] = (weakref.ref(feat), idx, (feat._version, idx._version))
+
+
+def _nbr_idx_of(x):
+    hit = _NBR_IDX.get(x.data_ptr())
+    if hit is None:
+        return None
+    feat, idx, version = hit[0](), hit[1], hit[2]
+    if feat is None:
+        del _NBR_IDX[x.data_ptr()]
+        return None
+    if feat._version != version[0] or x._version != version[0] or idx._version != version[1] or feat.data_ptr() != x.data_ptr() or tuple(feat.shape) != tuple(x.shape) or \
+            not x.is_contiguous() or tuple(idx.shape) != tuple(x.shape[:-1]) or idx.dtype != torch.int32 or not idx.is_contiguous() or \
+            idx.device != x.device:
+        return None
+    return idx
 
 
 def _fresh_zeros(shape, device):
@@ -196,6 +228,7 @@
         ctx.geom = (C, N, focal_begin, focal_count, out[3].shape[-1], out[4].shape[-1], lead)
         ctx.mark_non_differentiable(out[3], out[4])
         ctx.set_materialize_grads(False)
+        _note_nbr_idx(out[1], out[4])
         return out
 
     @staticmethod
@@ -228,6 +261,7 @@
         ctx.geom = (C, N, lead, tuple(desired_speed.shape))
         ctx.mark_non_differentiable(outs[3], outs[4])
         ctx.set_materialize_grads(False)
+        _note_nbr_idx(outs[1], outs[4])
         return outs
 
     @staticmethod
@@ -254,6 +288,7 @@
         ctx.geom = (C, N, focal_begin, focal_count, out[3].shape[-1], out[4].shape[-1], lead)
         ctx.mark_non_differentiable(out[3], out[4])
         ctx.set_materialize_grads(False)
+        _note_nbr_idx(out[1], out[4])
         return out
 
     @staticmethod
@@ -299,6 +334,7 @@
         ctx.speed_shape = tuple(desired_speed.shape)
         ctx.mark_non_differentiable(outs[3], outs[4])
         ctx.set_materialize_grads(False)
+        _note_nbr_idx(outs[1], outs[4])
         return outs
 
     @staticmethod
@@ -1848,9 +1884,10 @@
 
 def _enc_branch_struct(x2, k, scale, wb, msgs, h1=None, h2=None, g_pooled=None, g_msgs=None, g2=None, g1=None,
                        g_x=None, partials=None, packed=None, grads=None, keep_bits=None, draw_p=None, relu_mask=None,
-                       sum_a=None, sum_b=None):
+                       sum_a=None, sum_b=None, nbr_idx=None, plan=None):
     B = _lib.EncoderBranch()
     B.sum_a, B.sum_b = _ptr(sum_a), _ptr(sum_b)
+    B.nbr_idx, B.plan = _ptr(nbr_idx), _ptr(plan)
     B.keep_bits = _ptr(keep_bits)
     if draw_p is not None:
         B.drop_state, B.drop_p = dropout_state(x2.device).data_ptr(), float(draw_p)
@@ -2289,6 +2326,13 @@
                     probe[b].relu_mask = 1
                 msum = bool(L.piml_pinnsf_pool_msgs_ok(probe, nbr))
         ctx.sums = sums
+        nidx, plan = None, None
+        if sums and nbr == 2 and ks[1] in (2, 6, 10) and x2s[0].shape[1] == 6 and x2s[1].shape[1] == 6 and \
+                agents <= _lib.COMPACT_MAX_AGENTS and L.piml_encoder_compact_rows(-1) and L.piml_encoder_sums_bwd(-1) == 2:
+            nidx = _nbr_idx_of(xs[1]) if xs[1].data_ptr() == x2s[1].data_ptr() else None
+            if nidx is not None:
+                plan = torch.empty(16 + 2 * ((agents + 3) // 4 * 4), device=dev, dtype=torch.int32)
+        ctx.plan = plan
         sum_a, sum_b, masks = [None] * nbr, [None] * nbr, [None] * nbr
         for b in range(nbr):
             R = x2s[b].shape[0]
@@ -2300,7 +2344,10 @@
             elif sums:
                 msgs.append(None)
                 sum_a[b], sum_b[b] = torch.empty(agents, H, **opt), torch.empty(agents, H, **opt)
-                masks[b] = torch.empty(2 * ((R + 31) // 32), H, **opt)
+                tiles = (R + 31) // 32
+                if plan is not None and b == 1:
+                    tiles = max(tiles, -(-agents // (32 // ks[b])))
+                masks[b] = torch.empty(2 * tiles, H, **opt)
                 h2s.append(torch.empty(R, H, **opt) if (nhead and b == 0) else None)
             else:
                 msgs.append(torch.empty(R, H, **opt))
@@ -2321,7 +2368,8 @@
         keeps, draws = zip(*[_resolve_keep(keeps[b], x2s[b].shape[0], H, dev) for b in range(nbr)])
         earr = (_lib.EncoderBranch * nbr)(*[_enc_branch_struct(x2s[b], ks[b], scales[b], ewb[b], msgs[b], h1s[b], h2s[b],
                                                                packed=epack[b], keep_bits=keeps[b], draw_p=draws[b],
-                                                               relu_mask=masks[b], sum_a=sum_a[b], sum_b=sum_b[b])
+                                                               relu_mask=masks[b], sum_a=sum_a[b], sum_b=sum_b[b],
+                                                               nbr_idx=nidx if b == 1 else None, plan=plan if b == 1 else None)
                                             for b in range(nbr)])
         pooled = sum_a if (sums or msum) else [torch.empty(agents, H, **opt) for _ in range(nbr)]
         dh1 = [torch.empty(agents, 64, **opt) if need_grad else None for _ in range(nbr)]
@@ -2508,11 +2556,14 @@
         if len({g is None for g in gxs}) > 1:
             gxs = [g if g is not None else torch.empty(x2s[b].shape, **opt) for b, g in enumerate(gxs)]
         earr = (_lib.EncoderBranch * nbr)(*[_enc_branch_struct(x2s[b], ks[b], scales[b], ewb[b], None, None, None, g_pooled[b], None,
-                                                               None, None, gxs[b], packed=epack[b], relu_mask=masks[b])
+                                                               None, None, gxs[b], packed=epack[b], relu_mask=masks[b],
+                                                               plan=ctx.plan if b == 1 else None)
                                             for b in range(nbr)])
         w0 = ctypes.c_int(0)
         total = L.piml_encoder_workgroups(earr, nbr, ctypes.byref(w0))
         slots = [w0.value, total - w0.value] if nbr == 2 else [total]
+        if ctx.plan is not None:
+            slots = [_lib.COMPACT_SLOTS] * nbr
         parts = [torch.empty(n, part1, **opt) for n in slots]
         sink = ParamGradSink.current(ctx.sink)
         flags = _lib.POOL_TRAIN
@@ -2549,7 +2600,7 @@
         darr = (_lib.DecoderBranch * nbr)(*dstructs)
         if _defer_slot_sums([ctx.params[PER * b + jx] for b in range(nbr) for jx in range(1, 13)], sink, dev):
             flags |= _lib.DEFER_SLOT_SUMS
-            _defer_keep(parts, dparts, dflats, flats, dw1)
+            _defer_keep(parts, dparts, dflats, flats, dw1, ctx.plan)
         _lib.check(L.piml_pinnsf_bwd(earr, darr, nbr, _ptr(ga), _ptr(sf), float(tau), _ptr(g_self), flags, _stream()), 'piml_pinnsf_bwd')
         if want_self:
             grads[_FusedPinnsf.SELF] = g_self.view(sf_shape)
```

After: 240.6 billion (median of 6 runs). 4.9% higher.
